# Rorisis/Co-Occ

Measured on AMD Instinct MI355X. Metric: samples/sec (6-cam frame + sweep -> occ+render), 200x200x16 grid, higher is better.
Workload: dtype f32 (split-f16 products, fp32 accumulate)

## Files before the change

co_occ_amd/_lib.py:

```python
import ctypes
import os
import threading
import time

import torch

_HERE = os.path.dirname(os.path.abspath(__file__))
LIB_PATH = os.path.join(_HERE, "libcoocc_hip.so")

c_int, c_float, c_void_p, c_size_t, c_int64 = (ctypes.c_int, ctypes.c_float, ctypes.c_void_p,
                                               ctypes.c_size_t, ctypes.c_int64)


class ConvDesc(ctypes.Structure):
    _fields_ = [(n, c_void_p) for n in ("in_", "w", "out", "scale", "bias", "res", "gather", "out_rows", "ws")] + \
               [("ws_floats", c_int64)] + \
               [(n, c_int) for n in ("M", "Cin", "Cout", "taps", "in_stride", "out_stride", "res_stride",
                                     "B", "Xi", "Yi", "Zi", "Xo", "Yo", "Zo", "ksize", "stride", "pad",
                                     "relu", "res_mode", "splitk", "tile_hint", "kx", "ky", "kz", "px", "py", "pz",
                                     "wgroup_rows", "mfma_dtype")] + [("alpha", ctypes.c_float), ("M_dev", c_void_p), ("gather_stride", c_int), ("out16", c_void_p), ("out16_stride", c_int), ("out_h2", c_int),
                                                                   ("out_h2_twin", c_void_p), ("tile_sem", c_void_p), ("tile_sem_ints", c_int),
                                                                  ("alpha_dev", c_void_p), ("sx", c_int), ("sy", c_int), ("sz", c_int)]


class SearchDesc(ctypes.Structure):
    _fields_ = [("cat4", c_void_p), ("pts", c_void_p), ("pts_rows", c_int), ("pts_stride", c_int)] + \
               [(n, c_int) for n in ("C", "X", "Y", "Z", "K", "fps_num", "max_cluster")] + \
               [("radius", ctypes.c_float), ("dist_thresh", ctypes.c_float), ("offsets", c_void_p), ("noff", c_int)] + \
               [(n, c_void_p) for n in ("lin", "counts", "near_img", "near_pts", "rows", "rows_p", "ws")] + \
               [("ws_bytes", ctypes.c_size_t), ("counts_host", c_void_p)]


P, I, F, Z, L = c_void_p, c_int, c_float, c_size_t, c_int64
SIGNATURES = {
    "coocc_last_error": (ctypes.c_char_p, []),
    "coocc_abi_version": (I, []),
    "coocc_device_cu_count": (I, [P]),
    "coocc_stream_create_cu_mask": (I, [P, I, P]),
    "coocc_stream_destroy": (I, [P]),
    "coocc_event_create": (I, [I, P]),
    "coocc_event_destroy": (I, [P]),
    "coocc_event_record": (I, [P, P]),
    "coocc_stream_wait_event": (I, [P, P]),
    "coocc_event_synchronize": (I, [P]),
    "coocc_event_query": (I, [P]),
    "coocc_event_elapsed_ms": (I, [P, P, P]),
    "coocc_ncdhw_to_ndhwc": (I, [P, P, I, I, I, I, I, P]),
    "coocc_rows_to_bf16": (I, [P, I, L, I, P, P]),
    "coocc_rows_to_h2": (I, [P, I, L, I, F, P, P]),
    "coocc_rows_to_h2_ex": (I, [P, I, L, I, F, P, P, P]),
    "coocc_rows_to_h2_gather": (I, [P, I, P, L, P, I, F, P, P]),
    "coocc_rows_to_f16": (I, [P, I, L, I, P, P]),
    "coocc_wino_input_h2": (I, [P, I, I, I, I, I, I, I, P, I, L, F, P]),
    "coocc_wino_input_h2_ex": (I, [P, I, I, I, I, I, I, I, P, I, L, F, P, P]),
    "coocc_ndhwc_to_ncdhw": (I, [P, P, I, I, I, I, I, P]),
    "coocc_fuser_prepare": (I, [P, P, P, P, P, I, I, I, P]),
    "coocc_fuser_prepare_rows": (I, [P, I, I, P, I, I, P, P, P, I, I, I, P]),
    "coocc_compact_flags": (I, [P, I, P, P, P, Z, P]),
    "coocc_compact_flags_ex": (I, [P, I, P, P, P, P, Z, P]),
    "coocc_lin_to_coords": (I, [P, I, I, I, I, P, P, P]),
    "coocc_furthest_point_sampling": (I, [I, I, I, P, P, P, P]),
    "coocc_fps_voxels_ws": (Z, [I, I, I]),
    "coocc_fps_voxels": (I, [P, I, I, I, I, I, P, P, Z, P]),
    "coocc_fps_voxels_pair": (I, [P, I, P, P, P, I, P, P, Z, I, I, I, I, P]),
    "coocc_ball_query": (I, [I, I, I, F, F, I, P, P, P, P]),
    "coocc_knn_topk": (I, [I, I, I, P, P, P, P, P]),
    "coocc_voxel_index_map": (I, [P, I, I, P, P]),
    "coocc_voxel_index_map_dev": (I, [P, I, P, I, P, P]),
    "coocc_fine_sample_voxel_dev": (I, [P, I, I, I, I, P, I, P, I, P, P, P, I, P]),
    "coocc_fine_sample_img_dev": (I, [P, I, I, I, I, P, P, L, P, P, I, I, P]),
    "coocc_fine_mlp_pre_dev": (I, [P, I, P, I, L, P, I, P, P, P, F, P, P, P, P, F, P, P, I, P, P]),
    "coocc_fine_fused": (I, [P, I, I, I, P, I, I, I, P, P, I, P, I, P, P, P, P, F, P, P, P, P, F, P, P, I, P, P, P]),
    "coocc_fine2_pack": (I, [P, P, I, P, P, P, P, P, P, P, P, P, P]),
    "coocc_fine2_h2": (I, [P, I, I, I, I, P, I, I, I, P, P, I, P, P, P, P, F, F, I, P, P, P, P]),
    "coocc_fine_sample_img_lin": (I, [P, I, I, I, I, P, P, I, I, I, P, P, I, I, P]),
    "coocc_scatter_fine_dev": (I, [P, L, P, I, I, I, P, P, I, I, I, F, P]),
    "coocc_scatter_fine_grouped": (I, [P, I, I, P, I, P, I, I, I, I, P, F, P, P]),
    "coocc_ball_query_voxels": (I, [I, F, F, I, I, I, I, P, P, P, P, P]),
    "coocc_knn_topk_voxels": (I, [I, I, I, I, I, I, P, P, P, P, I, P, P, P, P, P]),
    "coocc_knn_assign": (I, [I, I, I, I, F, P, P, P, P, P, P]),
    "coocc_knn_threshold": (I, [I, F, P, P, P, P]),
    "coocc_index_rows_i32": (I, [P, I, P, I, P, P]),
    "coocc_conv_pack_weights": (L, [P, I, I, I, I, P]),
    "coocc_conv_fwd": (I, [ctypes.POINTER(ConvDesc), P]),
    "coocc_fuser_search_ws": (Z, [ctypes.POINTER(SearchDesc)]),
    "coocc_fuser_search": (I, [ctypes.POINTER(SearchDesc), P, P]),
    "coocc_upsample_add_trilinear": (I, [P, P, I, I, I, I, I, I, I, I, P]),
    "coocc_upsample_add_trilinear_ex": (I, [P, P, I, I, I, I, I, I, I, I, P, P]),
    "coocc_occhead_mix": (I, [P, P, I, P, P, I, I, P]),
    "coocc_occhead_mix_ex": (I, [P, P, I, P, P, I, I, P, P]),
    "coocc_argmax_flags": (I, [P, I, I, I, I, P, P]),
    "coocc_fine_sample_voxel": (I, [P, I, I, I, I, P, I, I, P, P, P, I, P]),
    "coocc_fine_sample_img": (I, [P, I, I, I, I, P, P, L, P, I, I, P]),
    "coocc_fine_mlp_pre": (I, [P, I, P, I, L, P, P, P, F, P, P, P, P, F, P, P, I, P, P]),
    "coocc_fine_mlp": (I, [P, I, P, I, L, P, P, P, P, F, P, P, P, P, F, P, P, I, P, P]),
    "coocc_groupnorm_rows": (I, [P, L, I, I, I, P, P, F, I, P]),
    "coocc_groupnorm_nhwc": (I, [P, I, I, I, I, P, P, F, I, P]),
    "coocc_scatter_fine": (I, [P, L, I, I, P, P, I, I, I, F, P]),
    "coocc_camera_mats": (I, [P, P, P, P, P, P, I, I, I, I, P, P]),
    "coocc_get_geometry": (I, [P, P, P, P, I, I, I, I, P, P]),
    "coocc_bev_pool_forward": (I, [P, P, P, P, I, I, I, I, I, I, I, P, P]),
    "coocc_bev_pool_backward": (I, [P, P, P, P, I, I, I, I, I, I, I, P, P]),
    "coocc_voxel_pool_ws": (Z, [I, I]),
    "coocc_voxel_pool": (I, [P, P, I, I, I, P, I, I, I, I, P, I, P, Z, I, P]),
    "coocc_lift_splat": (I, [P, P, P, I, I, I, I, I, I, P, I, I, I, I, P, I, P, Z, I, P]),
    "coocc_lift_splat_cams": (I, [P, P, P, P, P, P, I, I, I, I, I, I, P, I, I, I, I, P, I, P, Z, I, P]),
    "coocc_lift_splat_reuse": (I, [P, P, I, I, I, I, I, I, I, I, I, P, I, P, Z, P]),
    "coocc_bev_pool_coords": (I, [P, P, I, I, I, I, I, I, P, I, P, Z, I, P]),
    "coocc_render_nearest": (I, [P, I, I, I, P, P, I, I, I, I, P, I, P, P]),
    "coocc_render_nearest_cams": (I, [P, I, I, I, P, P, P, P, P, I, I, I, I, P, I, P, P]),
# ... 275 lines not shown
```

co_occ_amd/backbone.py:

```python
from torch import nn

from .core import PackCache, PackedConv, conv_rows, to_rows
from .registry import BACKBONES

_NORMS = {"BN": nn.BatchNorm3d, "BN3d": nn.BatchNorm3d, "SyncBN": nn.SyncBatchNorm}


def _eval_only(module):
    if module.training:
        raise RuntimeError("%s.forward_rows is the eval-mode (folded-BN, no autograd) path but the module is in training "
                           "mode; call .eval(), or use forward() / co_occ_amd.autograd for training" % type(module).__name__)


def build_bn(norm_cfg, num_features):
    cfg = dict(norm_cfg or dict(type="BN3d"))
    t = cfg.pop("type")
    cfg.pop("requires_grad", None)
    if t not in _NORMS:
        raise NotImplementedError("norm type %r: only BN-family norms are folded into the HIP convs" % t)
    return _NORMS[t](num_features, **cfg)


class BasicBlock(nn.Module):
    expansion = 1

    def __init__(self, in_planes, planes, stride=1, downsample=None, norm_cfg=None):
        super().__init__()
        self.conv1 = nn.Conv3d(in_planes, planes, 3, stride=stride, padding=1, bias=False)
        self.bn1 = build_bn(norm_cfg, planes)
        self.relu = nn.ReLU(inplace=True)
        self.conv2 = nn.Conv3d(planes, planes, 3, padding=1, bias=False)
        self.bn2 = build_bn(norm_cfg, planes)
        self.downsample = downsample
        self.stride = stride

    def packed(self):
        d = dict(c1=PackedConv(self.conv1.weight, bn=self.bn1, ksize=3, stride=self.stride, pad=1),
                 c2=PackedConv(self.conv2.weight, bn=self.bn2, ksize=3, pad=1))
        if self.downsample is not None:
            d["ds"] = PackedConv(self.downsample[0].weight, bn=self.downsample[1], ksize=1, stride=self.stride)
        return d

    def run(self, x, p, readers=()):
        out = conv_rows(x, p["c1"], relu=True, twin_for=(p["c2"],))
        res = conv_rows(x, p["ds"], relu=False) if "ds" in p else x
        return conv_rows(out, p["c2"], relu=True, res=res, twin_for=readers)


@BACKBONES.register_module()
class CustomResNet3D(nn.Module):
    def __init__(self, depth, block_inplanes=[64, 128, 256, 512], block_strides=[1, 2, 2, 2],
                 out_indices=(0, 1, 2, 3), n_input_channels=3, shortcut_type='B',
                 norm_cfg=dict(type='BN3d', requires_grad=True), widen_factor=1.0):
        super().__init__()
        layer_metas = {10: [1, 1, 1, 1], 18: [2, 2, 2, 2], 34: [3, 4, 6, 3]}
        if depth not in layer_metas:
            raise NotImplementedError("CustomResNet3D depth %s: Bottleneck depths are not on the coocc_nusc path" % depth)
        if shortcut_type != 'B':
            raise NotImplementedError("shortcut_type 'A' is not used by any shipped config")
        block_inplanes = [int(x * widen_factor) for x in block_inplanes]
        self.in_planes = block_inplanes[0]
        self.out_indices = out_indices
        self.input_proj = nn.Sequential(
            nn.Conv3d(n_input_channels, self.in_planes, kernel_size=(1, 1, 1), stride=(1, 1, 1), bias=False),
            build_bn(norm_cfg, self.in_planes), nn.ReLU(inplace=True))
        self.layers = nn.ModuleList()
        for i in range(len(block_inplanes)):
            self.layers.append(self._make_layer(block_inplanes[i], layer_metas[depth][i], block_strides[i], norm_cfg))
        for m in self.modules():
            if isinstance(m, nn.Conv3d):
                nn.init.kaiming_normal_(m.weight, mode='fan_out', nonlinearity='relu')
            elif isinstance(m, (nn.BatchNorm3d, nn.SyncBatchNorm)):
                nn.init.constant_(m.weight, 1)
                nn.init.constant_(m.bias, 0)
        self._packs = PackCache(self)

    def _make_layer(self, planes, blocks, stride, norm_cfg):
        downsample = None
        if stride != 1 or self.in_planes != planes:
            downsample = nn.Sequential(nn.Conv3d(self.in_planes, planes, 1, stride=stride, bias=False),
                                       build_bn(norm_cfg, planes))
        layers = [BasicBlock(self.in_planes, planes, stride, downsample, norm_cfg)]
        self.in_planes = planes
        for _ in range(1, blocks):
            layers.append(BasicBlock(self.in_planes, planes, norm_cfg=norm_cfg))
        return nn.Sequential(*layers)

    def _packed(self):
        def build():
            return dict(proj=PackedConv(self.input_proj[0].weight, bn=self.input_proj[1], ksize=1),
                        blocks=[[b.packed() for b in layer] for layer in self.layers])
        return self._packs.get_modules((self,), build)

    def forward_rows(self, x, readers=None):
        _eval_only(self)
        p = self._packed()
        flat = [bp for layer in p["blocks"] for bp in layer]
        x = conv_rows(to_rows(x), p["proj"], relu=True, twin_for=(flat[0]["c1"], flat[0].get("ds")))
        res = []
        n = 0
        for i, layer in enumerate(self.layers):
            for blk, bp in zip(layer, p["blocks"][i]):
                n += 1
                nxt = flat[n] if n < len(flat) else {}
                rd = [nxt.get("c1"), nxt.get("ds")]
                if readers is not None and i in self.out_indices and bp is p["blocks"][i][-1]:
                    rd += list(readers[self.out_indices.index(i)])
                x = blk.run(x, bp, tuple(rd))
            if i in self.out_indices:
                res.append(x)
        return res

    def forward(self, x):
        if self.training:
            from . import autograd as ag
            rows, geom = ag.rows_from_ncdhw(x)
            return [ag.ncdhw_from_rows(r, g) for r, g in ag.backbone_forward_train(self, rows, geom)]
        return [r.as_ncdhw() for r in self.forward_rows(x)]
```

co_occ_amd/core.py:

```python
import ctypes

import torch

from . import _lib
from ._lib import TIMER, ConvDesc, KernelTimer, call, ptr

_F32 = torch.float32


TILE_HINT = int(__import__("os").environ.get("COOCC_CONV_TILE", "0"))
CONV_V2 = int(__import__("os").environ.get("COOCC_CONV_V2", "1"))
WINO = int(__import__("os").environ.get("COOCC_WINO", "1"))
WINO_MIN_ROWS = int(__import__("os").environ.get("COOCC_WINO_MIN_ROWS", "8192"))
CONV_PERSIST = __import__("os").environ.get("COOCC_CONV_PERSIST", "1") != "0"
ZTRIM = __import__("os").environ.get("COOCC_ZTRIM", "1") != "0"
WINO_TILE = int(__import__("os").environ.get("COOCC_WINO_TILE", "4"))
CONV_DTYPE = __import__("os").environ.get("COOCC_CONV_DTYPE", "f32")
CONV_ENGINE = __import__("os").environ.get("COOCC_CONV_ENGINE", "h2")
H2_WINO_SCALE = {2: 0.5, 3: 0.25, 4: 0.125}
H2_DIRECT = __import__("os").environ.get("COOCC_H2_DIRECT", "1") != "0"
INKERNEL_REDUCE = __import__("os").environ.get("COOCC_INKERNEL_REDUCE", "0") != "0"
H2_DIRECT_MIN_FLOPS = float(__import__("os").environ.get("COOCC_H2_MIN_FLOPS", "5e7"))


# ... 22 lines not shown
        return self

    def __exit__(self, *exc):
        if self._ctx is not None:
            self._ctx.__exit__(*exc)
            self._ctx = None
        return False

    def join(self, *tensors):
        if self.on and self.side is not None:
            cur = torch.cuda.current_stream(self.side.device)
            cur.wait_stream(self.side)
            for t in tensors:
                if torch.is_tensor(t) and t.is_cuda:
                    t.record_stream(cur)
            self.side = None


def branch_streams_of(device, stream):
    return [s for (d, h, _), s in _branch_streams.items() if d == device.index and h == stream.cuda_stream]


def conv_kernel_name(M, Cout, table, hint=0, iters=1 << 30, one_by_one=False, grouped=False):
    if (one_by_one and CONV_PERSIST and CONV_V2 and not table and Cout > 64 and M >= 8192 and iters <= 24
            and -(-M // 128) * -(-Cout // 128) > 768):
        return "k_conv2p<1x1>"
    if (grouped and CONV_PERSIST and CONV_V2 and iters <= 24 and (M // 128) * -(-Cout // 128) > 768
            and conv_kernel_name(M, Cout, table, hint, iters) == "k_conv2<128>"):
        return "k_conv2p"
    hint = hint or TILE_HINT
    if Cout <= 32:
        t = "128,32,32,32"
    elif Cout <= 64:
        t = "128,64,32,64"
    elif M < 8192:
        if M >= 512 and not table and CONV_V2:
            return "k_conv2<128>"
        t = "64,128,32,64"
    else:
        def util(bm):
            tiles = -(-M // bm) * (-(-Cout // 128))
            return tiles * bm / float(-(-tiles // 512) * 512)
        big = hint == 160 or (hint == 0 and util(160) > util(128) * 1.02)
        if iters <= 24 and hint != 160:
            big = False
        if not table and CONV_V2:
            return "k_conv2<%d>" % (160 if big else 128)
        t = "160,128,160,32" if big else "128,128,64,64"
    return "k_conv<%s,%s>" % (t, "table" if table else "geom")


class Rows:

    __slots__ = ("t", "B", "X", "Y", "Z", "C", "coff", "h16", "h2", "persistent", "aux")

    def __init__(self, t, B, X, Y, Z, C, coff=0, persistent=False):
        self.t, self.B, self.X, self.Y, self.Z, self.C, self.coff = t, B, X, Y, Z, C, coff
        self.persistent = persistent
        self.aux = None
        self.h16 = None
        self.h2 = None

    @property
    def stride(self):
        return self.t.shape[1]

    @property
    def V(self):
        return self.X * self.Y * self.Z

    def data(self):
        return ptr(self.t, offset=self.coff)

    def as_ncdhw(self):
        v = self.t.view(self.B, self.X, self.Y, self.Z, self.stride)
        if self.coff or self.stride != self.C:
            v = v[..., self.coff:self.coff + self.C]
        v = v.permute(0, 4, 1, 2, 3)
        if not self.persistent:
            v._coocc_rows = (self, v._version)
        return v


def to_rows(x):
    if isinstance(x, Rows):
        return x
    back = getattr(x, "_coocc_rows", None)
    if back is not None:
        r, ver = back
        if ver == x._version and x.dim() == 5 and tuple(x.shape) == (r.B, r.C, r.X, r.Y, r.Z):
            return r
    if x.dim() != 5:
        raise ValueError("expected a [B,C,X,Y,Z] tensor")
    if not x.is_cuda:
        raise _lib.CooccError("co_occ_amd modules run on the GPU only (no CPU fallback)")
    B, C, X, Y, Z = x.shape
    x = x.float()
    cl = x.permute(0, 2, 3, 4, 1)
    if cl.is_contiguous():
        return Rows(cl.reshape(B * X * Y * Z, C), B, X, Y, Z, C)
    x = x.contiguous()
    out = torch.empty(B * X * Y * Z, C, device=x.device, dtype=_F32)
    call("coocc_ncdhw_to_ndhwc", ptr(x), ptr(out), B, C, X * Y * Z, C, 0)
    return Rows(out, B, X, Y, Z, C)


def rows_to_ncdhw_contiguous(r):
    out = torch.empty(r.B, r.C, r.X, r.Y, r.Z, device=r.t.device, dtype=_F32)
    call("coocc_ndhwc_to_ncdhw", ptr(r.t), ptr(out), r.B, r.C, r.V, r.stride, r.coff)
    return out


def fold_bn(bn, conv_bias=None):
    var = bn.running_var.double()
    scale = torch.rsqrt(var + bn.eps)
    if bn.weight is not None:
        scale = scale * bn.weight.double()
    bias = -bn.running_mean.double() * scale
    if bn.bias is not None:
        bias = bias + bn.bias.double()
    if conv_bias is not None:
        bias = bias + conv_bias.double() * scale
    return scale.float(), bias.float()


def zyx_weight(w):
    return w.detach().permute(0, 1, 4, 3, 2).contiguous()
# ... 240 lines not shown


def check_h2_overflow(reset=True):
    fault = _lib.load().coocc_device_fault(1 if reset else 0)
    if fault:
        raise _lib.CooccError("libcoocc_hip: a kernel met an index outside the buffer it addresses and skipped the access (fault code %d: "
                              "%s) -- the outputs of this sample are not trustworthy" % (
                                  fault, {1: "coocc_sparse_tap_sum read a voxel -> ordinal map entry past the rows it was sized for "
                                             "(a stale or corrupted map)"}.get(fault, "unknown")))
    if _lib.load().coocc_h2_overflow(1 if reset else 0):
        raise _lib.CooccRangeError(
            "split-f16 engine: an activation left the f16 operand range (|x| >= 32768, or %g for the F(4x4) Winograd layers whose "
            "transform amplifies by up to 100 at scale 1/8; NaN counts) -- the outputs of this sample are not trustworthy.  "
            "Set COOCC_CONV_ENGINE=f32 (exact-fp32 MFMA kernels, no range limit; ~1.8x slower) or rescale the inputs "
            "(INTEGRATION.md, 'Operand range of the split-f16 engine')." % (32768.0 / (100 * H2_WINO_SCALE[4])))


def ztrim(Zin, Zout, stride, pad):
    ok = [kz for kz in range(3) if any(0 <= zo * stride - pad + kz < Zin for zo in range(Zout))]
    lo, hi = ok[0], ok[-1]
    return (None, None) if hi - lo == 2 else ((lo, hi), (3, 3, hi - lo + 1, pad, pad, pad - lo))


def _route(B, X, Y, Z, pc, rm, splitk):
    Xo, Yo, Zo = out_dims(X, Y, Z, pc)
    M = B * Xo * Yo * Zo
    bf16, f16 = CONV_DTYPE == "bf16", CONV_DTYPE == "f16"
    plan = None if (bf16 or f16) else _wino_plan_geom(B, X, Y, Z, pc, M, rm)
    if plan is not None:
        return "wino", plan, None, None, pc.wino_kz
    trim, kdims = ztrim(Z, Zo, pc.stride, pc.pad) if (ZTRIM and pc._w_cube is not None) else (None, None)
    taps = pc.taps if trim is None else 9 * kdims[2]
    if f16 and pc.Cin % 64 == 0 and pc._w_taps is not None and rm in (0, 1) and splitk in (0, 1):
        return "f16", None, trim, kdims, taps
    if (not bf16 and not f16 and CONV_ENGINE == "h2" and H2_DIRECT and pc.Cin % 32 == 0 and pc._w_taps is not None
            and rm in (0, 1) and 2.0 * M * pc.Cin * pc.Cout * taps >= H2_DIRECT_MIN_FLOPS):
        return "h2", None, trim, kdims, taps
    return "other", None, trim, kdims, taps


def route(B, X, Y, Z, pc, rm=0, splitk=0):
    return _route(B, X, Y, Z, pc, rm, splitk)[0]


def takes_h2(rows, consumers):
    g = (rows.B, rows.X, rows.Y, rows.Z) if isinstance(rows, Rows) else rows
    return any(pc is not None and route(*g, pc) == "h2" for pc in consumers)


def wants_h2_twin(rows, consumers):
    return CONV_ENGINE == "h2" and CONV_DTYPE == "f32" and rows.C % 32 == 0 and takes_h2(rows, consumers)


def conv_rows_wino(x, pc, out, relu, res, plan, in_ranges=None, twin=False):
    dev = x.t.device
    tile, pts, Tx, Ty, rows, G, hint = plan
    V = _wino_buffer(dev, "V", pts * G * pc.Cin)
    Mb = _wino_buffer(dev, "M", pts * G * pc.Cout)
    h2 = h2_capable(pc) and all(c % 32 == 0 for _, c in (in_ranges or []))
    wp = pc.wino_h2_pack(tile) if h2 else pc.wino_pack(tile)
    vscale = H2_WINO_SCALE[tile]
    sdev = getattr(pc, "operand_scale_dev", None) if h2 else None
    with TIMER.region("k_wino_in", 4.0 * x.V * pc.Cin + 4.0 * pts * rows * pc.Cin):
        if in_ranges is None and not h2:
            call("coocc_wino_input", x.data(), x.stride, x.B, x.X, x.Y, x.Z, pc.Cin, tile, ptr(V), G)
        else:
            assert in_ranges is None or sum(c for _, c in in_ranges) == pc.Cin
            voff = 0
            for coff, cr in (in_ranges or [(0, pc.Cin)]):
                src = ptr(x.t, offset=x.coff + coff)
                dst = ptr(V, offset=voff)
                if h2:
                    call("coocc_wino_input_h2_ex", src, x.stride, x.B, x.X, x.Y, x.Z, cr, tile, dst, pc.Cin, G, vscale, ptr(sdev))
                else:
                    call("coocc_wino_input_strided", src, x.stride, x.B, x.X, x.Y, x.Z, cr, tile, dst, pc.Cin, G)
                voff += cr
    kz = pc.wino_kz
    d = conv_desc(dev, in_=ptr(V), w=ptr(wp), out=ptr(Mb), M=pts * G, Cin=pc.Cin, Cout=pc.Cout, taps=kz,
                  in_stride=pc.Cin, out_stride=pc.Cout, B=pts * G // x.Z, Xi=1, Yi=1, Zi=x.Z, Xo=1, Yo=1, Zo=x.Z,
                  ksize=3, stride=1, pad=1, kx=1, ky=1, kz=kz, pz=kz // 2, wgroup_rows=G, splitk=1, tile_hint=hint or TILE_HINT)
    flops = 2.0 * pts * rows * pc.Cin * pc.Cout * kz
    if h2:
        d.mfma_dtype, d.alpha = 3, 1.0 / vscale
        if sdev is not None:
            d.alpha_dev = ptr(sdev, offset=1)
        launch_conv(d, V.device, "k_gemm_h2z wino%d" % tile, flops)
    else:
        launch_conv(d, V.device, lambda: conv_kernel_name(pts * G, pc.Cout, False, hint, kz * -(-pc.Cin // 32), grouped=True)
                    + " wino%d" % tile, flops)
    tw = None
    if twin and h2 and pc.Cout % 32 == 0 and out.coff == 0 and out.stride % 4 == 0:
        tw = out.h2 = torch.empty(out.B * out.V, pc.Cout, device=dev, dtype=_F32)
    with TIMER.region("k_wino_out", 4.0 * pts * rows * pc.Cout + 4.0 * x.V * pc.Cout * (2 if tw is not None else 1)):
        call("coocc_wino_output_ex", ptr(Mb), G, x.B, x.X, x.Y, x.Z, pc.Cout, tile, out.data(), out.stride, ptr(pc.scale),
             ptr(pc.bias), res.data() if res is not None else None, res.stride if res is not None else 0, int(relu), ptr(tw))
    return out


def conv_desc(device, **fields):
    ws = workspace(device)
    return ConvDesc(ws=ptr(ws), ws_floats=ws.numel(), **fields)


def launch_conv(d, device, name, flops):
    if not TIMER.enabled:
        _lib.conv_fwd(d, device)
        return
    with TIMER.region(name() if callable(name) else name, flops):
        _lib.conv_fwd(d, device)


def out_dim(n, k, s, p):
    return (n + 2 * p - k) // s + 1


def out_dims(X, Y, Z, pc):
    return tuple(out_dim(n, k, s, p) for n, k, s, p in zip((X, Y, Z), pc.kernel, pc.strides, pc.pads))


def conv_rows(x, pc, relu=True, res=None, res_mode=0, out=None, splitk=0, twin_for=()):
    Xo, Yo, Zo = out_dims(x.X, x.Y, x.Z, pc)
    M = x.B * Xo * Yo * Zo
    if out is None:
        out = Rows(torch.empty(M, pc.Cout, device=x.t.device, dtype=_F32), x.B, Xo, Yo, Zo, pc.Cout)
    else:
        out.h2 = out.h16 = None
    assert x.C == pc.Cin, "channel mismatch: %d vs %d" % (x.C, pc.Cin)
    rm = res_mode or (1 if res is not None else 0)
    family, plan, trim, kdims, taps = _route(x.B, x.X, x.Y, x.Z, pc, rm, splitk)
    twin = wants_h2_twin(out, twin_for)
    if family == "wino":
        return conv_rows_wino(x, pc, out, relu, res, plan, twin=twin)
    dev = x.t.device
    d = conv_desc(dev, out=out.data(), scale=ptr(pc.scale), bias=ptr(pc.bias), res=res.data() if res is not None else None,
                  M=M, Cin=pc.Cin, Cout=pc.Cout, taps=taps, out_stride=out.stride, res_stride=res.stride if res is not None else 0,
                  B=x.B, Xi=x.X, Yi=x.Y, Zi=x.Z, Xo=Xo, Yo=Yo, Zo=Zo, ksize=pc.ksize, stride=pc.stride, pad=pc.pad,
                  relu=int(relu), res_mode=rm, splitk=splitk, tile_hint=TILE_HINT)
    if trim is not None:
        d.kx, d.ky, d.kz, d.px, d.py, d.pz = kdims
    if pc.aniso:
        (d.kx, d.ky, d.kz), (d.px, d.py, d.pz), (d.sx, d.sy, d.sz) = pc.kernel, pc.pads, pc.strides
    same = pc.is_unit_stride and (Xo, Yo, Zo) == (x.X, x.Y, x.Z)
    flops = 2.0 * M * pc.Cin * pc.Cout * taps
    if family == "f16" and out.coff == 0 and out.stride == pc.Cout:
        xh = x.h16
        if xh is None:
            xh = torch.empty(x.B * x.V, pc.Cin, device=dev, dtype=torch.float16)
            call("coocc_rows_to_f16", x.data(), x.stride, x.B * x.V, pc.Cin, ptr(xh))
        out.h16 = torch.empty(M, pc.Cout, device=dev, dtype=torch.float16) if pc.Cout % 4 == 0 else None
        d.in_, d.in_stride, d.w, d.mfma_dtype, d.alpha, d.splitk = ptr(xh), pc.Cin, ptr(pc.h1_pack(trim)), 4, 1.0, 1
        if out.h16 is not None:
            d.out16, d.out16_stride = ptr(out.h16), pc.Cout
        launch_conv(d, pc.w.device, "k_gemm_h1z" if (same and taps > 1) else "k_gemm_h1w", flops)
        return out
    if family == "h2":
        if x.coff == 0 and x.C == pc.Cin:
            xh = h2_rows(x)
        else:
            xh = scratch(dev, "h2in", x.B * x.V * pc.Cin)
            call("coocc_rows_to_h2", x.data(), x.stride, x.B * x.V, pc.Cin, 1.0, ptr(xh))
        d.in_, d.in_stride, d.w, d.mfma_dtype, d.alpha = ptr(xh), pc.Cin, ptr(pc.h2_pack(trim)), 3, 1.0
        if INKERNEL_REDUCE:
            sem = tile_sem(dev)
            d.tile_sem, d.tile_sem_ints = ptr(sem), sem.numel()
        if twin and out.coff == 0 and out.stride % 4 == 0 and (res is None or res.stride % 4 == 0):
            out.h2 = torch.empty(M, pc.Cout, device=dev, dtype=_F32)
            d.out_h2_twin = ptr(out.h2)
        launch_conv(d, pc.w.device, "k_gemm_h2z direct" if (same and taps > 1) else "k_gemm_h2w", flops)
        return out
    bf16 = CONV_DTYPE == "bf16"
    if bf16 and BF16_PRECONVERT and pc.Cin % 64 == 0 and pc._w_taps is not None and taps > 1:
        xb = stream_buffer(dev, "bf16", x.B * x.V * pc.Cin, torch.bfloat16)
        call("coocc_rows_to_bf16", x.data(), x.stride, x.B * x.V, pc.Cin, ptr(xb))
        d.in_, d.in_stride, d.w, d.mfma_dtype = ptr(xb), pc.Cin, ptr(pc.bf16_pack(trim)), 2
        name = "k_conv_bf16z" if (same and ZSHARE) else "k_conv_bf16w"
    else:
        d.in_, d.in_stride, d.mfma_dtype = x.data(), x.stride, 1 if bf16 else 0
        d.w = ptr(pc.ztrim_pack(*trim) if trim is not None else pc.w)
        name = "k_conv_bf16" if bf16 else lambda: conv_kernel_name(M, pc.Cout, False, 0, taps * -(-pc.Cin // 32),
                                                                   pc.is_pointwise)
    launch_conv(d, pc.w.device, name, flops)
    return out


def linear_rows(x2d, pc, relu=False, out=None, out_coff=0, in_coff=0, in_C=None):
    n = x2d.shape[0]
    Cin = in_C if in_C is not None else pc.Cin
    if out is None:
        out = torch.empty(n, pc.Cout, device=x2d.device, dtype=_F32)
    if n == 0:
        return out
    d = conv_desc(x2d.device, in_=ptr(x2d, offset=in_coff), w=ptr(pc.w), out=ptr(out, offset=out_coff), scale=ptr(pc.scale),
                  bias=ptr(pc.bias), M=n, Cin=Cin, Cout=pc.Cout, taps=1, in_stride=x2d.shape[1], out_stride=out.shape[1],
                  B=1, Xi=n, Yi=1, Zi=1, Xo=n, Yo=1, Zo=1, ksize=1, stride=1, relu=int(relu), tile_hint=TILE_HINT)
    launch_conv(d, x2d.device, lambda: conv_kernel_name(n, pc.Cout, False, 0, -(-Cin // 32), True), 2.0 * n * Cin * pc.Cout)
    return out


def linear_rows_h2(xh, n, Cin, pc, relu=False, out=None, out_coff=0, out_h2=False):
    dev = xh.device
    if out is None:
        out = torch.empty(n, pc.Cout, device=dev, dtype=_F32)
    d = conv_desc(dev, in_=ptr(xh), w=ptr(pc.h2_pack()), out=ptr(out, offset=out_coff), scale=ptr(pc.scale), bias=ptr(pc.bias),
                  M=n, Cin=Cin, Cout=pc.Cout, taps=1, in_stride=Cin, out_stride=out.shape[1], B=1, Xi=n, Yi=1, Zi=1, Xo=n, Yo=1,
                  Zo=1, ksize=1, stride=1, relu=int(relu), splitk=1, mfma_dtype=3, alpha=1.0, out_h2=int(out_h2))
    launch_conv(d, dev, "k_gemm_h2w linear", 2.0 * n * Cin * pc.Cout)
    return out


def rows_to_h2(x2d, C=None, coff=0, name="h2rows"):
    n = x2d.shape[0]
    C = C if C is not None else x2d.shape[1]
    xh = scratch(x2d.device, name, n * C)
    call("coocc_rows_to_h2", ptr(x2d, offset=coff), x2d.shape[1], n, C, 1.0, ptr(xh))
    return xh


def g1_h2_capable(pc, C):
    return bool(CONV_ENGINE == "h2" and H2_DIRECT and C % 32 == 0 and h2_capable(pc) and pc.h2_pack() is not None)


def g1_sources_h2(cat4, C, pc):
    if not g1_h2_capable(pc, C) or cat4.shape[1] < 2 * C:
        return None
    return rows_to_h2(cat4, 2 * C, 0, name="g1rows2")


def gather_conv_rows(src, src_coff, pc, gather, out_rows, dst, dst_coff, gate_coff, C, relu=True, count_dev=None, src_h2=None):
    K, M = gather.shape
    if M == 0:
        return
    d = conv_desc(src.device, in_=ptr(src, offset=src_coff), w=ptr(pc.w), out=ptr(dst, offset=dst_coff), bias=ptr(pc.bias),
                  res=ptr(dst, offset=gate_coff), gather=ptr(gather, torch.int32), out_rows=ptr(out_rows, torch.int32),
                  M=M, Cin=C, Cout=pc.Cout, taps=K, in_stride=src.shape[1], out_stride=dst.shape[1], res_stride=dst.shape[1],
                  B=1, Xi=src.shape[0], Yi=1, Zi=1, Xo=1, Yo=1, Zo=1,
                  ksize=1, stride=1, relu=int(relu), res_mode=2, splitk=1, tile_hint=TILE_HINT)
    if count_dev is not None:
        d.M_dev, d.gather_stride = ptr(count_dev, torch.int32), M
    h2 = g1_h2_capable(pc, C)
    if h2:
        if src_h2 is not None and src_h2[1] <= src_coff and src_coff + C <= src_h2[1] + src_h2[2] and (src_coff - src_h2[1]) % 32 == 0:
            sh, c0, n = src_h2
            d.in_, d.in_stride = ptr(sh, offset=src_coff - c0), n
        else:
            sh = rows_to_h2(src, C, src_coff, name="g1rows")
            d.in_, d.in_stride = ptr(sh), C
        d.w, d.mfma_dtype, d.alpha = ptr(pc.h2_pack()), 3, 1.0
    launch_conv(d, src.device, "k_gemm_h2w" if h2 else lambda: conv_kernel_name(M, pc.Cout, True), 2.0 * M * C * pc.Cout * K)


class PackCache:

    def __init__(self, owner=None):
        self._key = None
        self._val = None
        self._slots = None
        if owner is not None and hasattr(owner, "register_load_state_dict_post_hook"):
            owner.register_load_state_dict_post_hook(self._on_load_state_dict)

    def _on_load_state_dict(self, module, incompatible_keys):
        self.invalidate()

    def __getstate__(self):
        return dict(_key=None, _val=None, _slots=None)

    def invalidate(self):
        self._key = self._val = None
        self._slots = None

    def get_modules(self, modules, build, buffers=True):
        slots = getattr(self, "_slots", None)
        if slots is None:
            slots = []
            for mod in modules:
                for m in mod.modules():
                    slots += [(m._parameters, k) for k in m._parameters]
                    if buffers:
                        slots += [(m._buffers, k) for k in m._buffers]
# ... 58 lines not shown
```

co_occ_amd/csrc/conv3d.hip:

```cpp
#include <stdlib.h>
#include <type_traits>
#include <string.h>

#include "common.h"

typedef float f32x16 __attribute__((ext_vector_type(16)));
typedef float f32x4 __attribute__((ext_vector_type(4)));

#include "conv_k.h"
#include "h2_rows.h"

template <int BM, int BN, int WM, int WN, bool TABLE>
__global__ __launch_bounds__(256, 2) void k_conv(ConvK p) {
  constexpr int WAVES_N = BN / WN;
  constexpr int TM = WM / 32, TN = WN / 32;
  constexpr int PA = BM / 32, PB = BN / 32;
  static_assert((BM / WM) * (BN / WN) == 4, "4 waves per block");
  constexpr int NBUF = (2 * 2 * (BM + BN) * LDS_ST * 4 <= 160 * 1024) ? 2 : 1;
  __shared__ float As[NBUF][BM * LDS_ST];
  __shared__ float Bs[NBUF][BN * LDS_ST];

  const int id = blockIdx.x;
  int mtile, nt, slot = id >> 3;
  if (p.mtiles_per_xcd > 0) {
// ... 960 lines not shown
      }
#pragma unroll
      for (int i = 0; i < TM; ++i)
#pragma unroll
        for (int r = 0; r < 16; ++r) acc[i][r] = 0.f;
    }
    if (!has_next) break;
    id = nid; m0c = m0; n0c = n0;
  }
}

__global__ __launch_bounds__(256) void k_conv_reduce(ConvK p) {
  size_t i = (size_t)blockIdx.x * blockDim.x + threadIdx.x;
  if (i >= (size_t)p.M * p.Cout) return;
  int m = (int)(i / p.Cout), n = (int)(i - (size_t)m * p.Cout);
  float v = 0.f;
  for (int z = 0; z < p.splitk; ++z) v += p.ws[((size_t)z * p.M + m) * p.Npad + n];
  size_t orow = p.out_rows ? (size_t)p.out_rows[m] : (size_t)m;
  p.out[orow * p.out_stride + n] = epilogue(p, v, n, orow);
}

__global__ __launch_bounds__(256) void k_conv_reduce4(ConvK p) {
  const int c4 = p.Cout >> 2;
  const size_t i = (size_t)blockIdx.x * blockDim.x + threadIdx.x;
  if (i >= (size_t)p.M * c4) return;
  const int m = (int)(i / c4), n = (int)(i - (size_t)m * c4) * 4;
  f32x4 v = {0.f, 0.f, 0.f, 0.f};
  const float* src = p.ws + (size_t)m * p.Npad + n;
  const size_t zs = (size_t)p.M * p.Npad;
  const size_t orow = p.out_rows ? (size_t)p.out_rows[m] : (size_t)m;
  const f32x4 zero4 = {0.f, 0.f, 0.f, 0.f}, one4 = {1.f, 1.f, 1.f, 1.f};
  const f32x4 rs = (p.res_mode && p.res) ? *(const f32x4*)(p.res + orow * p.res_stride + n) : zero4;
  const f32x4 sc = p.scale ? *(const f32x4*)(p.scale + n) : one4;
  const f32x4 bi = p.bias ? *(const f32x4*)(p.bias + n) : zero4;
  int z = 0;
  for (; z + 4 <= p.splitk; z += 4) {
    const f32x4 a0 = *(const f32x4*)(src + (size_t)z * zs), a1 = *(const f32x4*)(src + (size_t)(z + 1) * zs);
    const f32x4 a2 = *(const f32x4*)(src + (size_t)(z + 2) * zs), a3 = *(const f32x4*)(src + (size_t)(z + 3) * zs);
    v = v + a0; v = v + a1; v = v + a2; v = v + a3;
  }
  if (z + 2 <= p.splitk) {
    const f32x4 a0 = *(const f32x4*)(src + (size_t)z * zs), a1 = *(const f32x4*)(src + (size_t)(z + 1) * zs);
    v = v + a0; v = v + a1;
    z += 2;
  }
  if (z < p.splitk) v = v + *(const f32x4*)(src + (size_t)z * zs);
  if (p.res_mode == 3) v = v + rs;
  if (p.scale) v = v * sc;
  if (p.bias) v = v + bi;
  if (p.res_mode == 1) v = v + rs;
  if (p.relu && (p.relu == 1 || n < p.relu)) { v[0] = fmaxf(v[0], 0.f); v[1] = fmaxf(v[1], 0.f); v[2] = fmaxf(v[2], 0.f); v[3] = fmaxf(v[3], 0.f); }
  if (p.res_mode == 2) v = v * rs;
  if (p.out_h2) { store_h2(p.out, orow, p.out_stride, n, v); h2_guard(p.h2_flag, v); }
  else *(f32x4*)(p.out + orow * p.out_stride + n) = v;
  if (p.out16) { store_f16(p.out16, orow, p.out16_stride, n, v); h2_guard(p.h2_flag, v); }
  if (p.out_h2t) { store_h2(p.out_h2t, orow, p.Cout, n, v); h2_guard(p.h2_flag, v); }
}

extern "C" int64_t coocc_conv_pack_weights(const float* w_host, int Cout, int Cin, int taps, int tap_major,
                                           float* packed_host) {
  if (Cout <= 0 || Cin <= 0 || taps <= 0) return coocc_set_error(COOCC_EINVAL, "pack_weights: bad dims");
  const int kch = (Cin + KC - 1) / KC;
  const int Npad = (Cout + NPAD_TO - 1) / NPAD_TO * NPAD_TO;
  const int64_t total = (int64_t)taps * kch * Npad * KC;
  if (!packed_host) return total;
  if (!w_host) return coocc_set_error(COOCC_EINVAL, "pack_weights: null weights");
  memset(packed_host, 0, sizeof(float) * (size_t)total);
  for (int t = 0; t < taps; ++t)
    for (int n = 0; n < Cout; ++n)
      for (int c = 0; c < Cin; ++c) {
        float v = tap_major ? w_host[((size_t)n * taps + t) * Cin + c] : w_host[((size_t)n * Cin + c) * taps + t];
        packed_host[wfrag_index((size_t)(c / KC) * taps + t, Npad >> 7, n, c % KC)] = v;
      }
  return total;
}

int coocc_zero_row(const void** out) {
  static void* zero_row[64] = {nullptr};
  int dev = 0;
  COOCC_HIP(hipGetDevice(&dev));
  COOCC_CHECK_ARG(dev >= 0 && dev < 64, "conv_fwd: device index");
  if (!zero_row[dev]) {
    COOCC_HIP(hipMalloc(&zero_row[dev], 256));
    COOCC_HIP(hipMemset(zero_row[dev], 0, 256));
  }
  *out = zero_row[dev];
  return COOCC_OK;
}

template <int BM, int BN, int WM, int WN>
static void launch_cfg(ConvK& k, bool table, hipStream_t s) {
  k.mtiles = (k.M + BM - 1) / BM;
  k.ntiles = (k.Cout + BN - 1) / BN;
  k.mtiles_per_xcd = k.mtiles >= 64 ? (k.mtiles + 7) / 8 : 0;
  dim3 grid(k.mtiles_per_xcd ? 8 * k.mtiles_per_xcd * k.ntiles : k.mtiles * k.ntiles, k.splitk);
  if (table)
    hipLaunchKernelGGL((k_conv<BM, BN, WM, WN, true>), grid, dim3(256), 0, s, k);
  else
    hipLaunchKernelGGL((k_conv<BM, BN, WM, WN, false>), grid, dim3(256), 0, s, k);
}

extern "C" int coocc_conv_fwd(const coocc_conv_desc* d, void* stream) {
  COOCC_CHECK_ARG(d && d->in && d->w && d->out, "conv_fwd: null pointer");
  COOCC_CHECK_ARG(d->M > 0 && d->Cin > 0 && d->Cout > 0 && d->taps > 0, "conv_fwd: bad sizes");
  COOCC_CHECK_ARG(d->Cin % 4 == 0 && d->in_stride % 4 == 0, "conv_fwd: Cin and in_stride must be multiples of 4");
  COOCC_CHECK_ARG(((uintptr_t)d->in & 15) == 0 && ((uintptr_t)d->w & 15) == 0, "conv_fwd: in/w must be 16-byte aligned");
  COOCC_CHECK_ARG(d->res_mode == 0 || d->res, "conv_fwd: res_mode set without res");
  if (!d->gather) {
    if (d->kx > 0) COOCC_CHECK_ARG(d->ky > 0 && d->kz > 0 && d->taps == d->kx * d->ky * d->kz, "conv_fwd: taps != kx*ky*kz");
    else COOCC_CHECK_ARG(d->taps == d->ksize * d->ksize * d->ksize, "conv_fwd: taps != ksize^3");
    COOCC_CHECK_ARG((long long)d->B * d->Xo * d->Yo * d->Zo == d->M, "conv_fwd: M != B*Xo*Yo*Zo");
  }
  ConvK k;
  memset(&k, 0, sizeof(k));
  k.in = d->in; k.w = d->w; k.out = d->out; k.scale = d->scale; k.bias = d->bias; k.res = d->res;
  k.gather = d->gather; k.out_rows = d->out_rows; k.ws = d->ws;
  k.M_dev = (d->gather || d->mfma_dtype >= 3) ? d->M_dev : nullptr;
  k.gstride = d->gather_stride > 0 ? d->gather_stride : d->M;
  COOCC_CHECK_ARG(!d->M_dev || ((d->gather || d->mfma_dtype >= 3) && d->splitk == 1), "conv_fwd: M_dev needs a row table (gather) or mfma_dtype 3, and splitk = 1");
  COOCC_CHECK_ARG(k.gstride >= d->M, "conv_fwd: gather_stride smaller than M");
  k.M = d->M; k.Cin = d->Cin; k.Cout = d->Cout; k.taps = d->taps;
  k.kchunks = (d->Cin + KC - 1) / KC;
  k.Npad = (d->Cout + NPAD_TO - 1) / NPAD_TO * NPAD_TO;
  k.in_stride = d->in_stride; k.out_stride = d->out_stride; k.res_stride = d->res_stride;
  k.Xi = d->Xi; k.Yi = d->Yi; k.Zi = d->Zi; k.Xo = d->Xo; k.Yo = d->Yo; k.Zo = d->Zo;
  k.stride = d->stride;
  COOCC_CHECK_ARG(d->sx >= 0 && d->sy >= 0 && d->sz >= 0, "conv_fwd: negative per-axis stride");
  k.sx = d->sx > 0 ? d->sx : d->stride; k.sy = d->sy > 0 ? d->sy : d->stride; k.sz = d->sz > 0 ? d->sz : d->stride;
  if (d->kx > 0) { k.kx = d->kx; k.ky = d->ky; k.kz = d->kz; k.px = d->px; k.py = d->py; k.pz = d->pz; }
  else { k.kx = k.ky = k.kz = d->ksize; k.px = k.py = k.pz = d->pad; }
  k.wgroup_rows = d->wgroup_rows;
  k.wgroup_floats = (size_t)k.taps * k.kchunks * k.Npad * KC;
  k.relu = d->relu; k.res_mode = d->res_mode;
  k.total_iters = k.taps * k.kchunks;
  if (d->mfma_dtype == 3 || d->mfma_dtype == 4) {
    hipStream_t s3 = as_stream(stream);
    const int rc = coocc_launch_h2(k, d, s3);
    if (rc != COOCC_OK) return rc;
    if (k.splitk > 1 && !k.tile_sem) {
      const bool vec4 = (k.Cout & 3) == 0 && (k.out_stride & 3) == 0 && (!k.res || (k.res_stride & 3) == 0) && (((uintptr_t)k.out) & 15) == 0;
      if (vec4) hipLaunchKernelGGL(k_conv_reduce4, dim3(cdiv((long long)k.M * (k.Cout / 4), 256)), dim3(256), 0, s3, k);
      else hipLaunchKernelGGL(k_conv_reduce, dim3(cdiv((long long)k.M * k.Cout, 256)), dim3(256), 0, s3, k);
      COOCC_LAUNCH_CHECK("k_conv_reduce");
    }
    return COOCC_OK;
  }
  if (d->mfma_dtype == 2) {
    COOCC_CHECK_ARG(d->Cin % 64 == 0 && d->in_stride % 8 == 0, "conv_fwd: bf16 operands need Cin % 64 == 0 and in_stride % 8 == 0");
    k.kchunks = d->Cin / 64;
    k.total_iters = k.taps * k.kchunks;
  }

  int cfg;
  if (d->Cout <= 32) cfg = 3;
  else if (d->Cout <= 64) cfg = 2;
  else cfg = d->M >= 8192 ? 0 : 1;
// ... 164 lines not shown
```

co_occ_amd/csrc/gemm_h2.hip:

```cpp
#include <stdlib.h>
#include <string.h>
#include <type_traits>

#include "conv_k.h"

#include "h2_rows.h"

typedef float f32x16 __attribute__((ext_vector_type(16)));
typedef _Float16 f16x8 __attribute__((ext_vector_type(8)));

__device__ __forceinline__ void glds16_(const void* g, void* l) {
  __builtin_amdgcn_global_load_lds((const __attribute__((address_space(1))) void*)g, (__attribute__((address_space(3))) void*)l,
                                   16, 0, 0);
}

__device__ __forceinline__ void h2_epilogue_vec(const ConvK& p, size_t orow, int n, f32x4 v) {
  if (p.res_mode == 3) v = v + *(const f32x4*)(p.res + orow * p.res_stride + n);
  if (p.scale) v = v * *(const f32x4*)(p.scale + n);
  if (p.bias) v = v + *(const f32x4*)(p.bias + n);
  if (p.res_mode == 1) v = v + *(const f32x4*)(p.res + orow * p.res_stride + n);
  if (p.relu && (p.relu == 1 || n < p.relu)) { v[0] = fmaxf(v[0], 0.f); v[1] = fmaxf(v[1], 0.f); v[2] = fmaxf(v[2], 0.f); v[3] = fmaxf(v[3], 0.f); }
  if (p.res_mode == 2) v = v * *(const f32x4*)(p.res + orow * p.res_stride + n);
  if (p.out_h2) { store_h2(p.out, orow, p.out_stride, n, v); h2_guard(p.h2_flag, v); }
  else *(f32x4*)(p.out + orow * p.out_stride + n) = v;
// ... 826 lines not shown
  const bool zshare = !table && !d->out_rows && !d->M_dev && k.stride == 1 && k.Xo == k.Xi && k.Yo == k.Yi && k.Zo == k.Zi && k.kz >= 1 && k.kz <= 3 &&
                      (k.taps > 1 || d->wgroup_rows > 0);
  COOCC_CHECK_ARG(zshare || d->wgroup_rows == 0, "conv_fwd: weight groups need the stride-1 same geometry");
  k.kchunks = d->Cin / kc;
  k.total_iters = k.taps * k.kchunks;
  k.wgroup_floats = (size_t)k.taps * k.kchunks * k.Npad * 32;
  k.out16 = d->out16;
  k.out16_stride = d->out16_stride;
  COOCC_CHECK_ARG(!d->out16 || (d->Cout % 4 == 0 && d->out16_stride % 4 == 0 && !d->out_rows && ((uintptr_t)d->out16 & 7) == 0),
                  "conv_fwd: out16 needs Cout % 4 == 0, out16_stride % 4 == 0, no row scatter");
  k.alpha = d->alpha != 0.f ? d->alpha : 1.f;
  k.alpha_dev = d->alpha_dev;
  k.M_dev = d->M_dev;
  k.out_h2 = d->out_h2;
  COOCC_CHECK_ARG(!d->out_h2 || (d->Cout % 4 == 0 && d->out_stride % 32 == 0 && !d->out_rows),
                  "conv_fwd: out_h2 needs Cout % 4 == 0, out_stride % 32 == 0, no row scatter");
  k.out_h2t = d->out_h2_twin;
  COOCC_CHECK_ARG(!d->out_h2_twin || (!one && d->Cout % 32 == 0 && !d->out_rows && ((uintptr_t)d->out_h2_twin & 15) == 0 && (d->out_stride & 3) == 0 &&
                                      (!d->res || (d->res_stride & 3) == 0)),
                  "conv_fwd: out_h2_twin needs mfma_dtype 3, Cout % 32 == 0, 16-byte aligned rows, no row scatter");
  k.tile_sem = d->tile_sem;
  int rc = coocc_zero_row(&k.zrow);
  if (rc != COOCC_OK) return rc;
  rc = coocc_h2_flag_ptr(&k.h2_flag);
  if (rc != COOCC_OK) return rc;
  k.ntiles = (k.Cout + 127) / 128;
  k.mtiles = (k.M + 127) / 128;
  k.mtiles_per_xcd = k.mtiles >= 64 ? (k.mtiles + 7) / 8 : 0;
  const int gsz = zshare ? k.kz : 1;
  int splitk = d->splitk;
  const long long blocks = (long long)k.mtiles * k.ntiles;
  const int ngroups = k.total_iters / gsz;
  if (splitk <= 0) {
    splitk = 1;
    const bool vec4 = (d->Cout & 3) == 0 && (d->out_stride & 3) == 0 && (!d->res || (d->res_stride & 3) == 0) && (((uintptr_t)d->out) & 15) == 0;
    const bool second_pass_ok = vec4 || (!d->out_h2 && !d->out16 && !d->out_h2_twin);
    static const int target = getenv("COOCC_SPLITK_TARGET") ? atoi(getenv("COOCC_SPLITK_TARGET")) : 512;
    if (blocks < target / 2 && ngroups >= 8 && d->ws && !d->M_dev && (d->tile_sem ? true : (!d->out_rows && second_pass_ok))) {
      splitk = (int)(target / blocks);
      if (splitk > ngroups / 4) splitk = ngroups / 4;
      if (splitk > 64) splitk = 64;
      while (splitk > 1 && (long long)splitk * d->M * k.Npad > d->ws_floats) --splitk;
      if (splitk < 1) splitk = 1;
    }
  }
  int gps = (ngroups + splitk - 1) / splitk;
  k.iters_per_split = gps * gsz;
  k.splitk = (k.total_iters + k.iters_per_split - 1) / k.iters_per_split;
  COOCC_CHECK_ARG(k.splitk == 1 || (d->ws && !d->M_dev && (long long)k.splitk * d->M * k.Npad <= d->ws_floats),
                  "conv_fwd: split-K workspace too small (or split-K with a device row count)");
  COOCC_CHECK_ARG(k.splitk == 1 || d->tile_sem || (!d->out_h2 && !d->out16 && !d->out_h2_twin) ||
                      ((d->Cout & 3) == 0 && (d->out_stride & 3) == 0 && (!d->res || (d->res_stride & 3) == 0) && (((uintptr_t)d->out) & 15) == 0),
                  "conv_fwd: split-K with an H2 / f16 output needs 16-byte aligned rows (Cout, strides % 4 == 0)");
  COOCC_CHECK_ARG(k.splitk == 1 || !d->tile_sem || (long long)k.mtiles * k.ntiles <= d->tile_sem_ints,
                  "conv_fwd: tile_sem holds fewer counters than the launch has output tiles");
  dim3 grid(k.mtiles_per_xcd ? 8 * k.mtiles_per_xcd * k.ntiles : k.mtiles * k.ntiles, k.splitk);
  static const bool pointwise_on = !(getenv("COOCC_H2_POINTWISE") && atoi(getenv("COOCC_H2_POINTWISE")) == 0);
  if (pointwise_on && !zshare && !table && !one && k.taps == 1 && k.stride == 1 && k.px == 0 && k.py == 0 && k.pz == 0 && k.Xo == k.Xi &&
      k.Yo == k.Yi && k.Zo == k.Zi && k.kchunks <= 4 && k.splitk == 1 && !d->M_dev && !d->out_rows && blocks >= 256 &&
      (d->Cout & 3) == 0 && (d->out_stride & 3) == 0 && (!d->res || (d->res_stride & 3) == 0)) {
    switch (k.kchunks) {
      case 1: hipLaunchKernelGGL(k_gemm_h2p<1>, grid, dim3(256), 0, s, k); break;
      case 2: hipLaunchKernelGGL(k_gemm_h2p<2>, grid, dim3(256), 0, s, k); break;
      case 3: hipLaunchKernelGGL(k_gemm_h2p<3>, grid, dim3(256), 0, s, k); break;
      default: hipLaunchKernelGGL(k_gemm_h2p<4>, grid, dim3(256), 0, s, k); break;
    }
    COOCC_LAUNCH_CHECK("k_gemm_h2p");
    return COOCC_OK;
  }
  if (!zshare) {
    if (one) {
      if (table) hipLaunchKernelGGL((k_gemm_h2w<true, 1>), grid, dim3(256), 0, s, k);
      else hipLaunchKernelGGL((k_gemm_h2w<false, 1>), grid, dim3(256), 0, s, k);
    } else {
      const char* narrow_env = getenv("COOCC_H2_NARROW");
      const bool narrow_on = !(narrow_env && atoi(narrow_env) == 0);
      if (narrow_on && table && k.Cout <= 64 && k.ntiles == 1 && k.splitk == 1 && !d->tile_sem && (long long)k.mtiles >= 512) {
        const dim3 gridn((unsigned)((k.M + 255) / 256), 1);
        if (k.Cout <= 32) hipLaunchKernelGGL(k_gemm_h2n<1>, gridn, dim3(256), 0, s, k);
        else hipLaunchKernelGGL(k_gemm_h2n<2>, gridn, dim3(256), 0, s, k);
        COOCC_LAUNCH_CHECK("k_gemm_h2n");
        return COOCC_OK;
      }
      if (narrow_on && table && k.Cout > 96 && k.ntiles == 1 && k.splitk == 1 && !d->tile_sem && (long long)k.mtiles >= 128 && (long long)k.mtiles < 1024) {
        const dim3 gridn((unsigned)((k.M + 63) / 64), 1);
        hipLaunchKernelGGL(k_gemm_h2n<4>, gridn, dim3(256), 0, s, k);
        COOCC_LAUNCH_CHECK("k_gemm_h2n<4>");
        return COOCC_OK;
      }
      if (table) hipLaunchKernelGGL(k_gemm_h2w<true>, grid, dim3(256), 0, s, k);
      else hipLaunchKernelGGL(k_gemm_h2w<false>, grid, dim3(256), 0, s, k);
    }
    COOCC_LAUNCH_CHECK("k_gemm_h2w");
    return COOCC_OK;
  }
  COOCC_CHECK_ARG((long long)d->M < (1ll << 30) && (136ull + 2ull * ((unsigned long long)k.Yi + 2) * k.Zi) * d->in_stride * 4ull < 0xFFFFFF00ull,
                  "conv_fwd: the split-f16 kernel addresses a tile's window with 32-bit byte offsets");
  const bool xy = !(k.kx == 1 && k.ky == 1 && k.px == 0 && k.py == 0);
  if (one) {
    if (k.kz == 3) { if (xy) hipLaunchKernelGGL((k_gemm_h2z<3, true, 0, 1>), grid, dim3(256), 0, s, k); else hipLaunchKernelGGL((k_gemm_h2z<3, false, 0, 1>), grid, dim3(256), 0, s, k); }
    else if (k.kz == 2) { if (xy) hipLaunchKernelGGL((k_gemm_h2z<2, true, 0, 1>), grid, dim3(256), 0, s, k); else hipLaunchKernelGGL((k_gemm_h2z<2, false, 0, 1>), grid, dim3(256), 0, s, k); }
    else { if (xy) hipLaunchKernelGGL((k_gemm_h2z<1, true, 0, 1>), grid, dim3(256), 0, s, k); else hipLaunchKernelGGL((k_gemm_h2z<1, false, 0, 1>), grid, dim3(256), 0, s, k); }
    COOCC_LAUNCH_CHECK("k_gemm_h2z<f16>");
    return COOCC_OK;
  }
  static const int abl = getenv("COOCC_H2_ABLATE") ? atoi(getenv("COOCC_H2_ABLATE")) : 0;
// ... 31 lines not shown
  if (n_dev) rows = min(rows, (long long)*n_dev);
  if (scale_dev) scale *= *scale_dev;
  const int c8 = C >> 3;
  const long long i = (long long)blockIdx.x * blockDim.x + threadIdx.x;
  if (i >= rows * c8) return;
  const long long r = i / c8;
  const int c = (int)(i - r * c8) * 8;
  const long long sr = row_ids ? (long long)row_ids[r] : r;
  const f32x4 a = *(const f32x4*)(in + sr * in_stride + c), b = *(const f32x4*)(in + sr * in_stride + c + 4);
  f16x8 hi, lo;
#pragma unroll
  for (int e = 0; e < 4; ++e) {
    _Float16 u, v;
    split_h2(a[e] * scale, u, v); hi[e] = u; lo[e] = v;
    split_h2(b[e] * scale, u, v); hi[4 + e] = u; lo[4 + e] = v;
  }
  char* o = out + r * (long long)C * 4 + (c >> 5) * 128 + (c & 31) * 2;
  *(f16x8*)o = hi;
  *(f16x8*)(o + 64) = lo;
  h2_guard(flag, a * scale);
  h2_guard(flag, b * scale);
}

extern "C" int coocc_rows_to_h2_ex(const float* in, int in_stride, int64_t rows, int C, float scale, const float* scale_dev,
                                   void* out_h2, void* stream) {
  COOCC_CHECK_ARG(in && out_h2 && rows >= 0 && C > 0 && C % 32 == 0 && in_stride % 4 == 0 && in_stride >= C, "rows_to_h2: bad args");
  COOCC_CHECK_ARG(((uintptr_t)in & 15) == 0 && ((uintptr_t)out_h2 & 15) == 0, "rows_to_h2: pointers must be 16-byte aligned");
  if (rows == 0) return COOCC_OK;
  int* flag = nullptr;
  if (coocc_h2_flag_ptr(&flag) != COOCC_OK) return COOCC_EHIP;
  hipLaunchKernelGGL(k_rows_to_h2, dim3(cdiv(rows * (C / 8), 256)), dim3(256), 0, as_stream(stream), in, in_stride, (long long)rows, C,
                     scale, (char*)out_h2, (const int32_t*)nullptr, (const int32_t*)nullptr, flag, scale_dev);
  COOCC_LAUNCH_CHECK("k_rows_to_h2");
  return COOCC_OK;
}

extern "C" int coocc_rows_to_h2(const float* in, int in_stride, int64_t rows, int C, float scale, void* out_h2, void* stream) {
  return coocc_rows_to_h2_ex(in, in_stride, rows, C, scale, nullptr, out_h2, stream);
}

extern "C" int coocc_rows_to_h2_gather(const float* in, int in_stride, const int32_t* row_ids, int64_t n_cap, const int32_t* n_dev,
                                       int C, float scale, void* out_h2, void* stream) {
  COOCC_CHECK_ARG(in && out_h2 && row_ids && n_cap >= 0 && C > 0 && C % 32 == 0 && in_stride % 4 == 0, "rows_to_h2_gather: bad args");
  COOCC_CHECK_ARG(((uintptr_t)in & 15) == 0 && ((uintptr_t)out_h2 & 15) == 0, "rows_to_h2_gather: pointers must be 16-byte aligned");
  if (n_cap == 0) return COOCC_OK;
  int* flag = nullptr;
  if (coocc_h2_flag_ptr(&flag) != COOCC_OK) return COOCC_EHIP;
  hipLaunchKernelGGL(k_rows_to_h2, dim3(cdiv(n_cap * (C / 8), 256)), dim3(256), 0, as_stream(stream), in, in_stride, (long long)n_cap, C,
                     scale, (char*)out_h2, row_ids, n_dev, flag, (const float*)nullptr);
  COOCC_LAUNCH_CHECK("k_rows_to_h2");
  return COOCC_OK;
}

__global__ __launch_bounds__(256) void k_rows_to_f16(const float* __restrict__ in, int in_stride, long long rows, int C, _Float16* __restrict__ out) {
  const int c8 = C >> 3;
  const long long i = (long long)blockIdx.x * blockDim.x + threadIdx.x;
  if (i >= rows * c8) return;
  const long long r = i / c8;
  const int c = (int)(i - r * c8) * 8;
  const f32x4 a = *(const f32x4*)(in + r * in_stride + c), b = *(const f32x4*)(in + r * in_stride + c + 4);
  f16x8 o;
#pragma unroll
  for (int e = 0; e < 4; ++e) { o[e] = (_Float16)a[e]; o[4 + e] = (_Float16)b[e]; }
  *(f16x8*)(out + r * C + c) = o;
}

extern "C" int coocc_rows_to_f16(const float* in, int in_stride, int64_t rows, int C, void* out_f16, void* stream) {
  COOCC_CHECK_ARG(in && out_f16 && rows >= 0 && C > 0 && C % 8 == 0 && in_stride % 4 == 0 && in_stride >= C, "rows_to_f16: bad args");
  COOCC_CHECK_ARG(((uintptr_t)in & 15) == 0 && ((uintptr_t)out_f16 & 15) == 0, "rows_to_f16: pointers must be 16-byte aligned");
  if (rows == 0) return COOCC_OK;
  hipLaunchKernelGGL(k_rows_to_f16, dim3(cdiv(rows * (C / 8), 256)), dim3(256), 0, as_stream(stream), in, in_stride, (long long)rows, C,
                     (_Float16*)out_f16);
  COOCC_LAUNCH_CHECK("k_rows_to_f16");
  return COOCC_OK;
}
```

co_occ_amd/csrc/layout.hip:

```cpp
#include <stdarg.h>
#include <stdlib.h>

#include "common.h"

typedef float f32x4 __attribute__((ext_vector_type(4)));

static thread_local char g_err[512] = "";

int coocc_set_error(int code, const char* fmt, ...) {
  va_list ap;
  va_start(ap, fmt);
  vsnprintf(g_err, sizeof(g_err), fmt, ap);
  va_end(ap);
  return code;
}

extern "C" const char* coocc_last_error(void) { return g_err; }
extern "C" int coocc_abi_version(void) { return 1; }

#define TV 64
#define TC 128

__global__ __launch_bounds__(256) void k_ncdhw_to_ndhwc(const float* __restrict__ src,
                                                         float* __restrict__ dst, int C, int V,
// ... 70 lines not shown
  COOCC_LAUNCH_CHECK("k_ndhwc_to_ncdhw");
  return COOCC_OK;
}

__global__ __launch_bounds__(256) void k_fuser_prepare(const float* __restrict__ img,
                                                        const float* __restrict__ pts,
                                                        float* __restrict__ cat4,
                                                        uint8_t* __restrict__ flag_img,
                                                        uint8_t* __restrict__ flag_pts, int C, int V) {
  __shared__ float tile[TV][TC + 1];
  const int b = blockIdx.y;
  const int v0 = blockIdx.x * TV;
  const int t = threadIdx.x;
  const int stride = 4 * C;
  for (int mod = 0; mod < 2; ++mod) {
    const float* src = mod ? pts : img;
    uint8_t* flags = mod ? flag_pts : flag_img;
    float rsum = 0.f;
    for (int c0 = 0; c0 < C; c0 += TC) {
      const int cn = min(TC, C - c0);
      for (int c = t >> 6; c < cn; c += 4) {
        int v = v0 + (t & 63);
        tile[t & 63][c] = v < V ? src[((size_t)b * C + c0 + c) * V + v] : 0.f;
      }
      __syncthreads();
      if (t < TV)
        for (int c = 0; c < cn; ++c) rsum += tile[t][c];
      for (int i = t; i < TV * cn; i += 256) {
        int v = i / cn, c = i - v * cn;
        if (v0 + v < V) cat4[((size_t)b * V + v0 + v) * stride + mod * C + c0 + c] = tile[v][c];
      }
      __syncthreads();
    }
    if (t < TV && v0 + t < V) flags[(size_t)b * V + v0 + t] = rsum != 0.f ? 1 : 0;
  }
  for (int i = t; i < TV * 2 * C; i += 256) {
    int v = i / (2 * C), c = i - v * 2 * C;
    if (v0 + v < V) cat4[((size_t)b * V + v0 + v) * stride + 2 * C + c] = 0.f;
  }
}

extern "C" int coocc_fuser_prepare(const float* img, const float* pts, float* cat4, uint8_t* flag_img,
                                   uint8_t* flag_pts, int B, int C, int V, void* stream) {
  COOCC_CHECK_ARG(img && pts && cat4 && flag_img && flag_pts && B > 0 && C > 0 && V > 0, "fuser_prepare: bad args");
  dim3 grid(cdiv(V, TV), B);
  hipLaunchKernelGGL(k_fuser_prepare, grid, dim3(256), 0, as_stream(stream), img, pts, cat4, flag_img, flag_pts, C, V);
  COOCC_LAUNCH_CHECK("k_fuser_prepare");
  return COOCC_OK;
}

__global__ __launch_bounds__(256) void k_fuser_prepare_rows(const float* __restrict__ img, int img_rows, int img_stride,
                                                             const float* __restrict__ pts, int pts_rows, int pts_stride,
                                                             float* __restrict__ cat4, uint8_t* __restrict__ flag_img,
                                                             uint8_t* __restrict__ flag_pts, int C, int V) {
  __shared__ float tile[TV][TC + 1];
  const int b = blockIdx.y;
  const int v0 = blockIdx.x * TV;
  const int t = threadIdx.x;
  const int stride = 4 * C;
  for (int mod = 0; mod < 2; ++mod) {
    const float* src = mod ? pts : img;
    const int rows = mod ? pts_rows : img_rows, sstride = mod ? pts_stride : img_stride;
    uint8_t* flags = mod ? flag_pts : flag_img;
    const bool in_place = rows && src == cat4 + mod * C && sstride == stride;
    float rsum = 0.f;
    for (int c0 = 0; c0 < C; c0 += TC) {
      const int cn = min(TC, C - c0);
      if (rows) {
        if (cn == TC) {
          for (int i = t; i < TV * (TC / 4); i += 256) {
            const int v = i / (TC / 4), c = (i % (TC / 4)) * 4;
            f32x4 q = {0.f, 0.f, 0.f, 0.f};
            if (v0 + v < V) q = *(const f32x4*)(src + ((size_t)b * V + v0 + v) * sstride + c0 + c);
            tile[v][c] = q[0]; tile[v][c + 1] = q[1]; tile[v][c + 2] = q[2]; tile[v][c + 3] = q[3];
          }
        } else {
          for (int i = t; i < TV * cn; i += 256) {
            int v = i / cn, c = i - v * cn;
            tile[v][c] = v0 + v < V ? src[((size_t)b * V + v0 + v) * sstride + c0 + c] : 0.f;
          }
        }
      } else {
        for (int c = t >> 6; c < cn; c += 4) {
          int v = v0 + (t & 63);
          tile[t & 63][c] = v < V ? src[((size_t)b * C + c0 + c) * V + v] : 0.f;
        }
      }
      __syncthreads();
      if (t < TV)
        for (int c = 0; c < cn; ++c) rsum += tile[t][c];
      if (!in_place)
        for (int i = t; i < TV * cn; i += 256) {
          int v = i / cn, c = i - v * cn;
          if (v0 + v < V) cat4[((size_t)b * V + v0 + v) * stride + mod * C + c0 + c] = tile[v][c];
        }
      __syncthreads();
    }
    if (t < TV && v0 + t < V) flags[(size_t)b * V + v0 + t] = rsum != 0.f ? 1 : 0;
  }
  for (int i = t; i < TV * 2 * C; i += 256) {
    int v = i / (2 * C), c = i - v * 2 * C;
    if (v0 + v < V) cat4[((size_t)b * V + v0 + v) * stride + 2 * C + c] = 0.f;
  }
}

constexpr int FV = 256, FC = 32;
__global__ __launch_bounds__(256) void k_fuser_prepare_rows_fast(const float* __restrict__ img, int img_rows, int img_stride,
                                                                  const float* __restrict__ pts, int pts_rows, int pts_stride,
                                                                  float* __restrict__ cat4, uint8_t* __restrict__ flag_img,
                                                                  uint8_t* __restrict__ flag_pts, int C, int V) {
  __shared__ float tile[FV][FC + 1];
  const int b = blockIdx.y;
  const int v0 = blockIdx.x * FV;
  const int t = threadIdx.x;
  const int stride = 4 * C;
  const int rv = t >> 3, rc = (t & 7) * 4;
  for (int mod = 0; mod < 2; ++mod) {
    const float* src = mod ? pts : img;
    const int rows = mod ? pts_rows : img_rows, sstride = mod ? pts_stride : img_stride;
    uint8_t* flags = mod ? flag_pts : flag_img;
    const bool in_place = rows && src == cat4 + mod * C && sstride == stride;
    float rsum = 0.f;
    for (int c0 = 0; c0 < C; c0 += FC) {
      if (rows) {
#pragma unroll
        for (int ps = 0; ps < FV / 32; ++ps) {
          const int v = ps * 32 + rv;
          f32x4 q = {0.f, 0.f, 0.f, 0.f};
          if (v0 + v < V) q = *(const f32x4*)(src + ((size_t)b * V + v0 + v) * sstride + c0 + rc);
          tile[v][rc] = q[0]; tile[v][rc + 1] = q[1]; tile[v][rc + 2] = q[2]; tile[v][rc + 3] = q[3];
        }
        __syncthreads();
#pragma unroll
        for (int c = 0; c < FC; ++c) rsum += tile[t][c];
      } else {
#pragma unroll 8
        for (int c = 0; c < FC; ++c) {
          const float x = v0 + t < V ? src[((size_t)b * C + c0 + c) * V + v0 + t] : 0.f;
          rsum += x;
          tile[t][c] = x;
        }
        __syncthreads();
      }
      if (!in_place) {
#pragma unroll
        for (int ps = 0; ps < FV / 32; ++ps) {
          const int v = ps * 32 + rv;
          if (v0 + v < V) {
            const f32x4 q = {tile[v][rc], tile[v][rc + 1], tile[v][rc + 2], tile[v][rc + 3]};
            *(f32x4*)(cat4 + ((size_t)b * V + v0 + v) * stride + mod * C + c0 + rc) = q;
          }
        }
      }
      __syncthreads();
    }
    if (v0 + t < V) flags[(size_t)b * V + v0 + t] = rsum != 0.f ? 1 : 0;
  }
  const int vec_per_row = C >> 1;
  const f32x4 z = {0.f, 0.f, 0.f, 0.f};
  if (vec_per_row <= 256 && 256 % vec_per_row == 0) {
    const int vpp = 256 / vec_per_row, tv = t / vec_per_row, c = (t - tv * vec_per_row) * 4;
    for (int v = tv; v < FV; v += vpp)
      if (v0 + v < V) *(f32x4*)(cat4 + ((size_t)b * V + v0 + v) * stride + 2 * C + c) = z;
  } else {
    for (int i = t; i < FV * vec_per_row; i += 256) {
      const int v = i / vec_per_row, c = (i - v * vec_per_row) * 4;
      if (v0 + v < V) *(f32x4*)(cat4 + ((size_t)b * V + v0 + v) * stride + 2 * C + c) = z;
    }
  }
}

extern "C" int coocc_fuser_prepare_rows(const float* img, int img_rows, int img_stride, const float* pts, int pts_rows,
                                        int pts_stride, float* cat4, uint8_t* flag_img, uint8_t* flag_pts, int B, int C, int V,
                                        void* stream) {
  COOCC_CHECK_ARG(img && pts && cat4 && flag_img && flag_pts && B > 0 && C > 0 && V > 0, "fuser_prepare_rows: bad args");
  COOCC_CHECK_ARG((!img_rows || img_stride >= C) && (!pts_rows || pts_stride >= C), "fuser_prepare_rows: row stride < C");
  const bool vec_ok = C % FC == 0 && ((uintptr_t)cat4 & 15) == 0 && (!img_rows || (img_stride % 4 == 0 && ((uintptr_t)img & 15) == 0)) &&
                      (!pts_rows || (pts_stride % 4 == 0 && ((uintptr_t)pts & 15) == 0));
  if (vec_ok) {
    hipLaunchKernelGGL(k_fuser_prepare_rows_fast, dim3(cdiv(V, FV), B), dim3(256), 0, as_stream(stream), img, img_rows, img_stride,
                       pts, pts_rows, pts_stride, cat4, flag_img, flag_pts, C, V);
    COOCC_LAUNCH_CHECK("k_fuser_prepare_rows_fast");
    return COOCC_OK;
  }
  dim3 grid(cdiv(V, TV), B);
  hipLaunchKernelGGL(k_fuser_prepare_rows, grid, dim3(256), 0, as_stream(stream), img, img_rows, img_stride, pts, pts_rows,
                     pts_stride, cat4, flag_img, flag_pts, C, V);
  COOCC_LAUNCH_CHECK("k_fuser_prepare_rows");
  return COOCC_OK;
}

#define CB 1024

__global__ __launch_bounds__(256) void k_flag_count(const uint8_t* __restrict__ flags, int total,
                                                     int32_t* __restrict__ blk) {
  __shared__ int wsum[4];
  int base = blockIdx.x * CB + threadIdx.x * 4;
  int c = 0;
  for (int j = 0; j < 4; ++j)
    if (base + j < total) c += flags[base + j] != 0;
  for (int o = 32; o > 0; o >>= 1) c += __shfl_down(c, o);
  if ((threadIdx.x & 63) == 0) wsum[threadIdx.x >> 6] = c;
  __syncthreads();
  if (threadIdx.x == 0) blk[blockIdx.x] = wsum[0] + wsum[1] + wsum[2] + wsum[3];
}

__global__ __launch_bounds__(1024) void k_scan_blocks(int32_t* __restrict__ blk, int nblk,
                                                       int32_t* __restrict__ count) {
  __shared__ int wsum[16];
  __shared__ int carry_s;
  if (threadIdx.x == 0) carry_s = 0;
  __syncthreads();
  for (int base = 0; base < nblk; base += 1024) {
    int i = base + threadIdx.x;
    int v = i < nblk ? blk[i] : 0;
    int inc = v;
    for (int o = 1; o < 64; o <<= 1) {
      int n = __shfl_up(inc, o);
      if ((threadIdx.x & 63) >= o) inc += n;
    }
    if ((threadIdx.x & 63) == 63) wsum[threadIdx.x >> 6] = inc;
    __syncthreads();
    int woff = 0;
    for (int w = 0; w < (int)(threadIdx.x >> 6); ++w) woff += wsum[w];
    int carry = carry_s;
    if (i < nblk) blk[i] = carry + woff + inc - v;
    __syncthreads();
    if (threadIdx.x == 1023) carry_s = carry + woff + inc;
    __syncthreads();
  }
  if (threadIdx.x == 0) *count = carry_s;
}

__global__ __launch_bounds__(256) void k_flag_write(const uint8_t* __restrict__ flags, int total,
                                                     const int32_t* __restrict__ blk,
                                                     int32_t* __restrict__ lin, int32_t* __restrict__ map) {
  __shared__ int wsum[4];
  int base = blockIdx.x * CB + threadIdx.x * 4;
  int f[4], c = 0;
  for (int j = 0; j < 4; ++j) {
    f[j] = (base + j < total) && flags[base + j] != 0;
    c += f[j];
// ... 189 lines not shown
```

co_occ_amd/csrc/search.hip:

```cpp
#include <stdlib.h>
#include <string.h>

#include "common.h"

__global__ __launch_bounds__(256) void k_gather_xyz(const float* __restrict__ xyz, const int32_t* __restrict__ idx, int m,
                                                     float* __restrict__ out) {
  const int i = blockIdx.x * blockDim.x + threadIdx.x;
  if (i >= m) return;
  const int s = idx[i];
  out[i * 3 + 0] = xyz[s * 3 + 0]; out[i * 3 + 1] = xyz[s * 3 + 1]; out[i * 3 + 2] = xyz[s * 3 + 2];
}

static size_t align256(size_t v) { return (v + 255) & ~(size_t)255; }

struct SearchWs {
  uint8_t* flags;
  int32_t* cws;
  float* xyz;
  int32_t* maps;
  int32_t* rep[2];
  float* rep_xyz[2];
  float* val[2];
  int32_t* nn[2];
  int32_t* group[2];
  int32_t* winner[2];
  void* fps[2];
  size_t fps_bytes;
  size_t total;
};

static SearchWs carve(char* base, int V, int K, int fps_num, int max_cluster, int X, int Y, int Z) {
  SearchWs w;
  size_t o = 0;
  auto take = [&](size_t bytes) { char* p = base ? base + o : nullptr; o += align256(bytes); return p; };
  w.flags = (uint8_t*)take((size_t)2 * V);
  w.cws = (int32_t*)take((size_t)2 * (V / 1024 + 2) * 4);
  w.xyz = (float*)take((size_t)2 * V * 3 * 4);
  w.maps = (int32_t*)take((size_t)2 * V * 4);
  w.fps_bytes = coocc_fps_voxels_ws(X, Y, Z);
  for (int d = 0; d < 2; ++d) {
    w.rep[d] = (int32_t*)take((size_t)fps_num * 4);
    w.rep_xyz[d] = (float*)take((size_t)fps_num * 3 * 4);
    w.val[d] = (float*)take((size_t)fps_num * K * 4);
    w.nn[d] = (int32_t*)take((size_t)fps_num * K * 4);
    w.group[d] = (int32_t*)take((size_t)fps_num * max_cluster * 4);
    w.winner[d] = (int32_t*)take((size_t)K * V * 4);
    w.fps[d] = take(w.fps_bytes);
  }
  w.total = o;
  return w;
}

extern "C" size_t coocc_fuser_search_ws(const coocc_search_desc* d) {
  if (!d || d->X <= 0 || d->Y <= 0 || d->Z <= 0 || d->K <= 0) return 0;
  return carve(nullptr, d->X * d->Y * d->Z, d->K, d->fps_num, d->max_cluster, d->X, d->Y, d->Z).total;
}

#define SRC(call)                    \
  do {                               \
    int rc__ = (call);               \
    if (rc__ != COOCC_OK) return rc__; \
  } while (0)

extern "C" int coocc_fuser_search(coocc_search_desc* d, void* stream, void* side_stream) {
  COOCC_CHECK_ARG(d && d->cat4 && d->pts && d->lin && d->counts && d->rows && d->rows_p && d->near_img && d->near_pts && d->ws &&
                      d->offsets && d->counts_host, "fuser_search: null pointer");
  COOCC_CHECK_ARG(d->C > 0 && d->X > 0 && d->Y > 0 && d->Z > 0 && d->K >= 1 && d->K <= 8 && d->fps_num > 0 && d->max_cluster > 0 &&
                      d->noff > 0, "fuser_search: bad sizes");
  COOCC_CHECK_ARG(stream != side_stream && side_stream, "fuser_search: needs a second stream for the img <- pts direction");
  const int V = d->X * d->Y * d->Z, K = d->K, C = d->C;
  SearchWs w = carve((char*)d->ws, V, K, d->fps_num, d->max_cluster, d->X, d->Y, d->Z);
  COOCC_CHECK_ARG(d->ws_bytes >= w.total, "fuser_search: workspace smaller than coocc_fuser_search_ws()");
  hipStream_t s0 = as_stream(stream), s1 = as_stream(side_stream);
  static const int sdiag = [] { const char* e = getenv("COOCC_SEARCH_DIAG_SKIP"); return e ? atoi(e) : 0; }();
  int32_t* lin_img = d->lin;
  int32_t* lin_pts = d->lin + V;

  SRC(coocc_fuser_prepare_rows(d->cat4, 1, 4 * C, d->pts, d->pts_rows, d->pts_stride, d->cat4, w.flags, w.flags + V, 1, C, V, stream));
  SRC(coocc_compact_flags(w.flags, V, lin_img, d->counts, w.cws, (size_t)(V / 1024 + 2) * 4, stream));
  SRC(coocc_compact_flags(w.flags + V, V, lin_pts, d->counts + 1, w.cws + (V / 1024 + 2), (size_t)(V / 1024 + 2) * 4, stream));
  if (!((sdiag & 4) && d->counts_host[0] > 0)) COOCC_HIP(hipMemcpyAsync(d->counts_host, d->counts, 8, hipMemcpyDeviceToHost, s0));
  if (!((sdiag & 4) && d->counts_host[0] > 0)) {
    static const bool fence = [] { const char* e = getenv("COOCC_SEARCH_COUNT_FENCE"); return e && e[0] == '1'; }();
    hipEvent_t got;
    COOCC_HIP(hipEventCreateWithFlags(&got, hipEventBlockingSync | hipEventDisableTiming | (fence ? 0u : hipEventDisableSystemFence)));
    const hipError_t e1 = hipEventRecord(got, s0);
    const hipError_t e2 = e1 == hipSuccess ? hipEventSynchronize(got) : e1;
    (void)hipEventDestroy(got);
    if (e2 != hipSuccess) return coocc_set_error(COOCC_EHIP, "fuser_search: waiting for the voxel counts failed: %s", hipGetErrorString(e2));
  }
  const int Ni = d->counts_host[0], Np = d->counts_host[1];
  if (Ni <= d->fps_num || Np <= d->fps_num) return COOCC_SEARCH_SMALL;

  float* xyz_img = w.xyz;
  float* xyz_pts = w.xyz + (size_t)V * 3;
  SRC(coocc_lin_to_coords(lin_img, Ni, d->X, d->Y, d->Z, xyz_img, nullptr, stream));
  SRC(coocc_lin_to_coords(lin_pts, Np, d->X, d->Y, d->Z, xyz_pts, nullptr, stream));
  int32_t* map_img = w.maps;
  int32_t* map_pts = w.maps + V;
  SRC(coocc_voxel_index_map(lin_img, Ni, V, map_img, stream));
  SRC(coocc_voxel_index_map(lin_pts, Np, V, map_pts, stream));

  const int pair_rc = (sdiag & 1) ? COOCC_OK
                                  : coocc_fps_voxels_pair(lin_pts, Np, w.rep[0], w.fps[0], lin_img, Ni, w.rep[1], w.fps[1], w.fps_bytes, d->X, d->Y,
                                                          d->Z, d->fps_num, stream);
  if (pair_rc != COOCC_OK && pair_rc != 2) return pair_rc;
  const bool paired = pair_rc == COOCC_OK;
  hipEvent_t fork = nullptr, join = nullptr;
  COOCC_HIP(hipEventCreateWithFlags(&fork, hipEventDisableTiming | hipEventDisableSystemFence));
  if (hipEventCreateWithFlags(&join, hipEventDisableTiming | hipEventDisableSystemFence) != hipSuccess) {
    (void)hipEventDestroy(fork);
    return coocc_set_error(COOCC_EHIP, "fuser_search: hipEventCreate failed");
  }
  bool forked = false;
  auto finish = [&](int rc) -> int {
    if (forked) {
      if (hipEventRecord(join, s1) != hipSuccess || hipStreamWaitEvent(s0, join, 0) != hipSuccess) {
        if (rc == COOCC_OK) rc = coocc_set_error(COOCC_EHIP, "fuser_search: joining the side stream failed");
      }
    }
    (void)hipEventDestroy(fork);
    (void)hipEventDestroy(join);
    return rc;
  };
#define SRF(call)                                \
  do {                                           \
    int rc__ = (call);                           \
    if (rc__ != COOCC_OK) return finish(rc__);   \
  } while (0)
  void* side_q = paired ? stream : side_stream;
  if (!paired) {
// ... 27 lines not shown
```

co_occ_amd/csrc/winograd.hip:

```cpp
#include "conv_k.h"
#include "h2_rows.h"

template <int N> struct Wino;
template <> struct Wino<4> {
  static constexpr int M = 2;
  template <typename T> static __device__ __forceinline__ void bt(const T* d, T* t) {
    t[0] = d[0] - d[2]; t[1] = d[1] + d[2]; t[2] = d[2] - d[1]; t[3] = d[1] - d[3];
  }
  template <typename T> static __device__ __forceinline__ void at(const T* m, T* y) {
    y[0] = m[0] + m[1] + m[2]; y[1] = m[1] - m[2] - m[3];
  }
  template <typename T> static __device__ __forceinline__ void a(const T* y, T* t) {
    t[0] = y[0]; t[1] = y[0] + y[1]; t[2] = y[0] - y[1]; t[3] = -y[1];
  }
};
template <> struct Wino<5> {
  static constexpr int M = 3;
  template <typename T> static __device__ __forceinline__ void bt(const T* d, T* t) {
    t[0] = d[0] - 1.5f * (d[1] + d[2]) + d[3];
    t[1] = d[1] - 2.5f * d[2] + d[3];
    t[2] = 0.5f * (d[2] - d[1]) + d[3];
    t[3] = -2.f * d[1] - d[2] + d[3];
    t[4] = d[1] - 1.5f * (d[2] + d[3]) + d[4];
  }
// ... 24 lines not shown
    y[2] = s12 + 0.25f * m[3] + 4.f * m[4];
    y[3] = d12 + 0.125f * m[3] - 8.f * m[4] + m[5];
  }
  template <typename T> static __device__ __forceinline__ void a(const T* y, T* t) {
    const T s02 = y[0] + y[2], s13 = y[1] + y[3];
    t[0] = y[0]; t[1] = s02 + s13; t[2] = s02 - s13;
    t[3] = y[0] + 0.5f * y[1] + 0.25f * y[2] + 0.125f * y[3];
    t[4] = y[0] - 2.f * y[1] + 4.f * y[2] - 8.f * y[3];
    t[5] = y[3];
  }
};

template <int N>
__global__ __launch_bounds__(256) void k_wino_in(const float* __restrict__ in, int in_stride, int B, int X, int Y, int Z,
                                                  int C, int Tx, int Ty, size_t gstride, int vstride, float* __restrict__ V) {
  constexpr int MO = Wino<N>::M;
  const int c4 = C >> 2;
  const long long i = (long long)blockIdx.x * 256 + threadIdx.x;
  const long long rows = (long long)B * Tx * Ty * Z;
  if (i >= rows * c4) return;
  const int c = (int)(i % c4) * 4;
  const long long row = i / c4;
  long long r = row;
  const int z = (int)(r % Z); r /= Z;
  const int ty = (int)(r % Ty); r /= Ty;
  const int tx = (int)(r % Tx); const int b = (int)(r / Tx);
  f32x4 t[N][N];
#pragma unroll
  for (int e = 0; e < N; ++e) {
    f32x4 d[N], q[N];
    const int y = MO * ty - 1 + e;
#pragma unroll
    for (int a = 0; a < N; ++a) {
      const int x = MO * tx - 1 + a;
      f32x4 v = {0.f, 0.f, 0.f, 0.f};
      if ((unsigned)x < (unsigned)X && (unsigned)y < (unsigned)Y)
        v = *(const f32x4*)(in + ((((size_t)b * X + x) * Y + y) * Z + z) * in_stride + c);
      d[a] = v;
    }
    Wino<N>::bt(d, q);
#pragma unroll
    for (int a = 0; a < N; ++a) t[a][e] = q[a];
  }
  float* o = V + (size_t)row * vstride + c;
#pragma unroll
  for (int a = 0; a < N; ++a) {
    f32x4 q[N];
    Wino<N>::bt(t[a], q);
#pragma unroll
    for (int e = 0; e < N; ++e) *(f32x4*)(o + (size_t)(a * N + e) * gstride) = q[e];
  }
}

template <int N>
__global__ __launch_bounds__(256) void k_wino_in_h2(const float* __restrict__ in, int in_stride, int B, int X, int Y, int Z,
                                                     int C, int Tx, int Ty, size_t gstride_bytes, int vstride, float scale,
                                                     char* __restrict__ V, int* __restrict__ flag, const float* __restrict__ scale_dev) {
  constexpr int MO = Wino<N>::M;
  if (scale_dev) scale *= *scale_dev;
  const int c4 = C >> 2;
  const long long i = (long long)blockIdx.x * 256 + threadIdx.x;
  const long long rows = (long long)B * Tx * Ty * Z;
  if (i >= rows * c4) return;
  const int c = (int)(i % c4) * 4;
  const long long row = i / c4;
  long long r = row;
  const int z = (int)(r % Z); r /= Z;
  const int ty = (int)(r % Ty); r /= Ty;
  const int tx = (int)(r % Tx); const int b = (int)(r / Tx);
  f32x4 t[N][N];
#pragma unroll
  for (int e = 0; e < N; ++e) {
    f32x4 d[N], q[N];
    const int y = MO * ty - 1 + e;
#pragma unroll
    for (int a = 0; a < N; ++a) {
      const int x = MO * tx - 1 + a;
      f32x4 v = {0.f, 0.f, 0.f, 0.f};
      if ((unsigned)x < (unsigned)X && (unsigned)y < (unsigned)Y)
        v = *(const f32x4*)(in + ((((size_t)b * X + x) * Y + y) * Z + z) * in_stride + c);
      d[a] = v;
    }
    Wino<N>::bt(d, q);
#pragma unroll
    for (int a = 0; a < N; ++a) t[a][e] = q[a];
  }
#pragma unroll
  for (int a = 0; a < N; ++a) {
    f32x4 q[N];
    Wino<N>::bt(t[a], q);
#pragma unroll
    for (int e = 0; e < N; ++e) {
      const f32x4 sv = q[e] * scale;
      store_h2_pair(V + (size_t)(a * N + e) * gstride_bytes, (size_t)row, vstride, c, sv);
      h2_guard(flag, sv);
    }
  }
}

extern "C" int coocc_wino_input_h2_ex(const float* in, int in_stride, int B, int X, int Y, int Z, int C, int tile, void* V,
                                      int vstride, int64_t group_rows, float scale, const float* scale_dev, void* stream) {
  COOCC_CHECK_ARG(in && V && B > 0 && X > 0 && Y > 0 && Z > 0 && C > 0 && C % 32 == 0 && in_stride % 4 == 0, "wino_input_h2: bad args");
  COOCC_CHECK_ARG(tile >= 2 && tile <= 4, "wino_input_h2: tile must be 2, 3 or 4");
  COOCC_CHECK_ARG(vstride >= C && vstride % 32 == 0 && ((uintptr_t)V & 127) == 0, "wino_input_h2: V row stride / alignment");
  COOCC_CHECK_ARG(scale > 0.f, "wino_input_h2: scale must be positive");
  const int Tx = (X + tile - 1) / tile, Ty = (Y + tile - 1) / tile;
  const long long rows = (long long)B * Tx * Ty * Z;
  COOCC_CHECK_ARG(group_rows >= rows, "wino_input_h2: group_rows smaller than B*ceil(X/tile)*ceil(Y/tile)*Z");
  const dim3 grid(cdiv(rows * (C / 4), 256));
  const size_t gstride = (size_t)group_rows * vstride * 4;
  hipStream_t s = as_stream(stream);
  int* flag = nullptr;
  if (coocc_h2_flag_ptr(&flag) != COOCC_OK) return COOCC_EHIP;
  if (tile == 2)
    hipLaunchKernelGGL(k_wino_in_h2<4>, grid, dim3(256), 0, s, in, in_stride, B, X, Y, Z, C, Tx, Ty, gstride, vstride, scale, (char*)V, flag, scale_dev);
  else if (tile == 3)
    hipLaunchKernelGGL(k_wino_in_h2<5>, grid, dim3(256), 0, s, in, in_stride, B, X, Y, Z, C, Tx, Ty, gstride, vstride, scale, (char*)V, flag, scale_dev);
  else
    hipLaunchKernelGGL(k_wino_in_h2<6>, grid, dim3(256), 0, s, in, in_stride, B, X, Y, Z, C, Tx, Ty, gstride, vstride, scale, (char*)V, flag, scale_dev);
  COOCC_LAUNCH_CHECK("k_wino_in_h2");
  return COOCC_OK;
}

extern "C" int coocc_wino_input_h2(const float* in, int in_stride, int B, int X, int Y, int Z, int C, int tile, void* V,
                                   int vstride, int64_t group_rows, float scale, void* stream) {
  return coocc_wino_input_h2_ex(in, in_stride, B, X, Y, Z, C, tile, V, vstride, group_rows, scale, nullptr, stream);
}

static int wino_input_impl(const float* in, int in_stride, int B, int X, int Y, int Z, int C, int tile, float* V, int vstride,
                           int64_t group_rows, void* stream) {
  COOCC_CHECK_ARG(in && V && B > 0 && X > 0 && Y > 0 && Z > 0 && C > 0 && C % 4 == 0 && in_stride % 4 == 0, "wino_input: bad args");
  COOCC_CHECK_ARG(tile >= 2 && tile <= 4, "wino_input: tile must be 2, 3 or 4");
  COOCC_CHECK_ARG(vstride >= C && vstride % 4 == 0 && ((uintptr_t)V & 15) == 0, "wino_input: V row stride / alignment");
  const int Tx = (X + tile - 1) / tile, Ty = (Y + tile - 1) / tile;
  const long long rows = (long long)B * Tx * Ty * Z;
  COOCC_CHECK_ARG(group_rows >= rows, "wino_input: group_rows smaller than B*ceil(X/tile)*ceil(Y/tile)*Z");
  const dim3 grid(cdiv(rows * (C / 4), 256));
  const size_t gstride = (size_t)group_rows * vstride;
  if (tile == 2)
    hipLaunchKernelGGL(k_wino_in<4>, grid, dim3(256), 0, as_stream(stream), in, in_stride, B, X, Y, Z, C, Tx, Ty, gstride, vstride, V);
  else if (tile == 3)
    hipLaunchKernelGGL(k_wino_in<5>, grid, dim3(256), 0, as_stream(stream), in, in_stride, B, X, Y, Z, C, Tx, Ty, gstride, vstride, V);
  else
    hipLaunchKernelGGL(k_wino_in<6>, grid, dim3(256), 0, as_stream(stream), in, in_stride, B, X, Y, Z, C, Tx, Ty, gstride, vstride, V);
  COOCC_LAUNCH_CHECK("k_wino_in");
  return COOCC_OK;
}

extern "C" int coocc_wino_input(const float* in, int in_stride, int B, int X, int Y, int Z, int C, int tile, float* V,
                                int64_t group_rows, void* stream) {
// ... 8 lines not shown
template <int N>
__global__ __launch_bounds__(256) void k_wino_out(const float* __restrict__ Mb, size_t gstride, int B, int X, int Y, int Z,
                                                   int C, int Tx, int Ty, float* __restrict__ out, int out_stride,
                                                   const float* __restrict__ scale, const float* __restrict__ bias,
                                                   const float* __restrict__ res, int res_stride, int relu,
                                                   void* __restrict__ twin, int* __restrict__ flag) {
  constexpr int MO = Wino<N>::M;
  const int c4 = (C + 3) >> 2;
  const long long i = (long long)blockIdx.x * 256 + threadIdx.x;
  const long long rows = (long long)B * Tx * Ty * Z;
  if (i >= rows * c4) return;
  const int c = (int)(i % c4) * 4;
  const long long row = i / c4;
  long long r = row;
  const int z = (int)(r % Z); r /= Z;
  const int ty = (int)(r % Ty); r /= Ty;
  const int tx = (int)(r % Tx); const int b = (int)(r / Tx);
  const int nc = min(4, C - c);
  const bool vec = (C & 3) == 0;
  const float* src = Mb + (size_t)row * C + c;
  f32x4 s[MO][N];
#pragma unroll
  for (int e = 0; e < N; ++e) {
    f32x4 m[N], q[MO];
#pragma unroll
    for (int a = 0; a < N; ++a) {
      const float* p = src + (size_t)(a * N + e) * gstride;
      if (vec) m[a] = *(const f32x4*)p;
      else m[a] = f32x4{p[0], nc > 1 ? p[1] : 0.f, nc > 2 ? p[2] : 0.f, nc > 3 ? p[3] : 0.f};
    }
    Wino<N>::at(m, q);
#pragma unroll
    for (int a = 0; a < MO; ++a) s[a][e] = q[a];
  }
  f32x4 sc = {1.f, 1.f, 1.f, 1.f}, bi = {0.f, 0.f, 0.f, 0.f};
#pragma unroll
  for (int e = 0; e < 4; ++e)
    if (e < nc) {
      if (scale) sc[e] = scale[c + e];
      if (bias) bi[e] = bias[c + e];
    }
#pragma unroll
  for (int a = 0; a < MO; ++a) {
    f32x4 y[MO];
    Wino<N>::at(s[a], y);
    const int x = MO * tx + a;
    if (x >= X) continue;
#pragma unroll
    for (int bb = 0; bb < MO; ++bb) {
      const int yy = MO * ty + bb;
      if (yy >= Y) continue;
      const size_t orow = (((size_t)b * X + x) * Y + yy) * Z + z;
      f32x4 v = y[bb] * sc + bi;
      float* o = out + orow * out_stride + c;
      const float* rr = res ? res + orow * res_stride + c : nullptr;
      if (vec && (out_stride & 3) == 0 && (!res || (res_stride & 3) == 0)) {
        if (rr) v = v + *(const f32x4*)rr;
        if (relu) { v[0] = fmaxf(v[0], 0.f); v[1] = fmaxf(v[1], 0.f); v[2] = fmaxf(v[2], 0.f); v[3] = fmaxf(v[3], 0.f); }
        *(f32x4*)o = v;
        if (twin) { store_h2_pair(twin, orow, C, c, v); h2_guard(flag, v); }
      } else {
#pragma unroll
        for (int e = 0; e < 4; ++e)
          if (e < nc) {
            float u = v[e] + (rr ? rr[e] : 0.f);
            o[e] = relu ? fmaxf(u, 0.f) : u;
          }
      }
    }
  }
}

extern "C" int coocc_wino_output_ex(const float* Mb, int64_t group_rows, int B, int X, int Y, int Z, int C, int tile, float* out,
                                    int out_stride, const float* scale, const float* bias, const float* res, int res_stride,
                                    int relu, void* out_h2_twin, void* stream) {
  COOCC_CHECK_ARG(Mb && out && B > 0 && X > 0 && Y > 0 && Z > 0 && C > 0, "wino_output: bad args");
  COOCC_CHECK_ARG(tile >= 2 && tile <= 4, "wino_output: tile must be 2, 3 or 4");
  COOCC_CHECK_ARG(((uintptr_t)out & 15) == 0 && (!res || ((uintptr_t)res & 15) == 0), "wino_output: out/res must be 16-byte aligned");
  COOCC_CHECK_ARG(!out_h2_twin || (C % 32 == 0 && (out_stride & 3) == 0 && (!res || (res_stride & 3) == 0) && ((uintptr_t)out_h2_twin & 15) == 0),
                  "wino_output: the H2 twin needs C % 32 == 0 and 16-byte aligned rows");
  const int Tx = (X + tile - 1) / tile, Ty = (Y + tile - 1) / tile;
  const long long rows = (long long)B * Tx * Ty * Z;
  COOCC_CHECK_ARG(group_rows >= rows, "wino_output: group_rows too small");
  int* flag = nullptr;
  if (out_h2_twin && coocc_h2_flag_ptr(&flag) != COOCC_OK) return COOCC_EHIP;
  const dim3 grid(cdiv(rows * ((C + 3) / 4), 256));
  if (tile == 2)
    hipLaunchKernelGGL(k_wino_out<4>, grid, dim3(256), 0, as_stream(stream), Mb, (size_t)group_rows * C, B, X, Y, Z, C, Tx, Ty,
                       out, out_stride, scale, bias, res, res_stride, relu, out_h2_twin, flag);
  else if (tile == 3)
    hipLaunchKernelGGL(k_wino_out<5>, grid, dim3(256), 0, as_stream(stream), Mb, (size_t)group_rows * C, B, X, Y, Z, C, Tx, Ty,
                       out, out_stride, scale, bias, res, res_stride, relu, out_h2_twin, flag);
  else
    hipLaunchKernelGGL(k_wino_out<6>, grid, dim3(256), 0, as_stream(stream), Mb, (size_t)group_rows * C, B, X, Y, Z, C, Tx, Ty,
                       out, out_stride, scale, bias, res, res_stride, relu, out_h2_twin, flag);
  COOCC_LAUNCH_CHECK("k_wino_out");
  return COOCC_OK;
}

extern "C" int coocc_wino_output(const float* Mb, int64_t group_rows, int B, int X, int Y, int Z, int C, int tile, float* out,
                                 int out_stride, const float* scale, const float* bias, const float* res, int res_stride,
                                 int relu, void* stream) {
  return coocc_wino_output_ex(Mb, group_rows, B, X, Y, Z, C, tile, out, out_stride, scale, bias, res, res_stride, relu, nullptr, stream);
}

template <int N>
__global__ __launch_bounds__(256) void k_wino_gradout(const float* __restrict__ dy, int dy_stride, int B, int X, int Y, int Z,
                                                       int C, int Tx, int Ty, size_t gstride, float* __restrict__ dM) {
  constexpr int MO = Wino<N>::M;
  const int c4 = C >> 2;
  const long long i = (long long)blockIdx.x * 256 + threadIdx.x;
  const long long rows = (long long)B * Tx * Ty * Z;
  if (i >= rows * c4) return;
  const int c = (int)(i % c4) * 4;
  const long long row = i / c4;
  long long r = row;
  const int z = (int)(r % Z); r /= Z;
  const int ty = (int)(r % Ty); r /= Ty;
  const int tx = (int)(r % Tx); const int b = (int)(r / Tx);
  f32x4 t[N][MO];
#pragma unroll
  for (int j = 0; j < MO; ++j) {
    f32x4 d[MO], q[N];
    const int y = MO * ty + j;
#pragma unroll
    for (int a = 0; a < MO; ++a) {
      const int x = MO * tx + a;
      f32x4 v = {0.f, 0.f, 0.f, 0.f};
      if (x < X && y < Y) v = *(const f32x4*)(dy + ((((size_t)b * X + x) * Y + y) * Z + z) * dy_stride + c);
// ... 287 lines not shown
```

co_occ_amd/detector.py:

```python
import numpy as np
import torch
from torch import nn

from . import registry
from .core import to_rows
from .registry import DETECTORS
from .render import MLP, render_block, render_losses
from .view_transformer import get_frustum


def _build_upstream(kind, cfg, external, hip_image=False):
    if cfg is None or isinstance(cfg, nn.Module):
        return cfg
    if hip_image:
        from . import image_encoder
        mine = {"backbone": (image_encoder.IMAGE_BACKBONES, "ResNet"), "neck": (image_encoder.IMAGE_NECKS, "SECONDFPN")}[kind]
        if cfg.get("type") == mine[1]:
            return mine[0].build(cfg)
    ours = {"backbone": registry.BACKBONES, "neck": registry.NECKS}[kind]
    if cfg.get("type") in ours:
        return ours.build(cfg)
    try:
        from mmdet3d.models import builder as m3b
    except Exception as e:
# ... 186 lines not shown

    def extract_feat(self, points, img, img_metas, search=None):
        img_voxel_feats = pts_voxel_feats = pts_feats = depth = img_feats = geom = None
        if img is not None:
            img_voxel_feats, depth, img_feats, geom = self.extract_img_feat(img, img_metas)
        if points is not None:
            pts_voxel_feats, pts_feats = self.extract_pts_feat(points)
        voxel_feats = self.fuse(img_voxel_feats, pts_voxel_feats, search)
        return voxel_feats, img_feats, pts_feats, depth, geom, img_voxel_feats

    def freeze_lidar_encoder(self, frozen=True):
        self._lidar_frozen = bool(frozen)
        if self.pts_middle_encoder is not None:
            for prm in self.pts_middle_encoder.parameters():
                prm.requires_grad_(not frozen)
            if frozen:
                self.pts_middle_encoder.eval()
        return self

    def train(self, mode=True):
        super().train(mode)
        if mode:
            self._pipe1 = None
        if mode and getattr(self, "_lidar_frozen", False) and getattr(self, "pts_middle_encoder", None) is not None:
            self.pts_middle_encoder.eval()
        return self

    def fuse(self, img_voxel_feats, pts_voxel_feats, search=None):
        if self.occ_fuser is not None:
            return self.occ_fuser(img_voxel_feats, pts_voxel_feats, search=search)
        assert (img_voxel_feats is None) or (pts_voxel_feats is None)
        return img_voxel_feats if pts_voxel_feats is None else pts_voxel_feats

    def search(self, img_voxel_feats, pts_voxel_feats):
        return self.occ_fuser.search(img_voxel_feats, pts_voxel_feats)

    def forward_hot_path(self, img_voxel_feats, pts_voxel_feats, gemo=None, img_feats=None, transform=None,
                         render=None, dense_fine=True, search=None):
        voxel_feats = self.fuse(img_voxel_feats, pts_voxel_feats, search)
        return self.decode(voxel_feats, gemo, img_feats, transform, render, dense_fine)

    def decode(self, voxel_feats, gemo=None, img_feats=None, transform=None, render=None, dense_fine=True,
               depth_only=False, fine_size=None, after_encoder=None, static=False, cam_geo=None):
        from . import core
        neck, head = self.semantic_neck, self.pts_bbox_head
        do_render = (self.use_rendering and self.test_rendering) if render is None else render
        rbranch = rendered = None
        if do_render:
            rbranch = core.Fork(0, voxel_feats.t.device if isinstance(voxel_feats, core.Rows) else voxel_feats.device)
            with rbranch:
                rendered = render_block(self.sigma_head, getattr(self, "rgb_head", None), to_rows(voxel_feats), gemo, 16,
                                        depth_only=depth_only or not hasattr(self, "rgb_head"), cam_geo=cam_geo)
        ibranch = head.fork_image_branch(img_feats, transform, to_rows(voxel_feats)) if hasattr(head, "fork_image_branch") else None
        mid = self.semantic_encoder.forward_rows(voxel_feats, readers=neck.lateral_packs() if hasattr(neck, "lateral_packs") else None)
        if after_encoder is not None:
            after_encoder()
        sem = neck.forward_rows(mid, readers=head.level_readers() if hasattr(head, "level_readers") else None)
        kw = dict(image_branch=ibranch) if ibranch is not None else {}
        output = self.pts_bbox_head(voxel_feats=sem, img_feats=img_feats, transform=transform, static=static, **kw)
        res = dict(voxel_feats=voxel_feats, pred_c=output['output_voxels'][0], pred_f=None,
                   output_voxels_fine=output['output_voxels_fine'], output_coords_fine=output['output_coords_fine'])
        if output['output_voxels_fine'] is not None and dense_fine:
            cf = self.pts_bbox_head.cascade_ratio
            pc = res['pred_c']
            size = fine_size or [pc.shape[2] * cf, pc.shape[3] * cf, pc.shape[4] * cf]
            res['pred_f'] = self.pts_bbox_head.scatter_fine(output['output_voxels_fine'][0],
                                                            output['output_coords_fine'][0], list(size),
                                                            count_dev=output.get('fine_count'))
            res['fine_count'] = output.get('fine_count')
        if do_render:
            rgbs, depths, maps = rendered
            rbranch.join(rgbs, depths, maps)
            res.update(rgbs=rgbs, depths=depths, render_maps=maps)
        return res

    def forward_train_hot_path(self, img_voxel_feats, pts_voxel_feats, gemo=None, img_feats=None, transform=None,
                               coarse_lin=None, render=True, generator=None, depth_only=False, search=None):
        from . import autograd as ag
        one = img_voxel_feats if img_voxel_feats is not None else pts_voxel_feats
        B, C, X, Y, Z = one.shape
        assert B == 1, "batch size 1 per GPU (coocc_ray.py:365)"
        V = X * Y * Z
        rows = lambda t: t.float().permute(0, 2, 3, 4, 1).reshape(V, t.shape[1])
        if self.occ_fuser is not None:
            sr = search
            if sr is None:
                with torch.no_grad():
                    sr = self.occ_fuser.search(img_voxel_feats.detach(), pts_voxel_feats.detach())
            self.occ_fuser.finish_bookkeeping(sr)
            cat4 = ag.fuser_fuse_train(self.occ_fuser, rows(img_voxel_feats).contiguous(), rows(pts_voxel_feats).contiguous(), sr)
            vf, geom = ag.con_enc_train(self.occ_fuser.con_enc, cat4, (1, X, Y, Z))
        else:
            assert (img_voxel_feats is None) or (pts_voxel_feats is None)
            vf, geom = rows(one).contiguous(), (1, X, Y, Z)
        levels = ag.trunk_forward_train(None, self.semantic_encoder, self.semantic_neck, vf, geom)
        head = self.pts_bbox_head
        out_rows, logit_rows = ag.occhead_coarse_train(head, levels)
        res = dict(voxel_rows=vf, levels=levels, out_voxel_rows=out_rows, logit_rows=logit_rows)
        if head.cascade_ratio != 1 and (head.sample_from_img or head.sample_from_voxel):
            if coarse_lin is None:
                coarse_lin = head.draw_fine_voxels(logit_rows.detach(), generator)
            if coarse_lin.numel():
                res["fine_logits"], res["fine_xyz"] = ag.fine_branch_train(head, out_rows, (1, X, Y, Z), coarse_lin.contiguous(),
                                                                           img_feats, transform)
        if render and self.use_rendering:
            rgb_head = None if (depth_only or not hasattr(self, "rgb_head")) else self.rgb_head
            res["rgbs"], res["depths"] = ag.render_block_train(self.sigma_head, rgb_head, vf, (X, Y, Z), gemo)
# ... 339 lines not shown
```

co_occ_amd/fuser.py:

```python
import torch
from torch import nn

from . import _lib, streams
from ._lib import call, ptr
from . import core as _core_mod
from .core import PackCache, PackedConv, Rows, conv_rows, gather_conv_rows
from .registry import FUSION_LAYERS

_I32, _F32, _I64 = torch.int32, torch.float32, torch.int64


_side = {}


def _side_stream(dev, cur, which=0):
    key = (dev.index, cur.cuda_stream, which)
    if key not in _side:
        _side[key] = streams.side_stream_for(cur, which) or torch.cuda.Stream(device=dev, priority=getattr(cur, "priority", 0))
    return _side[key]


FPS_HIGH_PRIORITY = __import__("os").environ.get("COOCC_FPS_HIGH_PRIORITY", "0") != "0"
_fps_hi = {}
FPS_MAX_BUCKETS = 8 * 1024
# ... 95 lines not shown
    winner = torch.empty(num, Q, device=dev, dtype=_I32)
    out = torch.empty(num, Q, device=dev, dtype=_I32)
    call("coocc_knn_assign", fps_num, num, max_cluster_samples, Q, float(dist_thresh), ptr(val), ptr(nn_), ptr(group),
         ptr(winner), ptr(out))
    return out


def _as_rows_view(x):
    if isinstance(x, Rows):
        return x
    if x.dim() != 5 or not x.is_cuda or x.dtype != _F32:
        return None
    B, C, X, Y, Z = x.shape
    sb, sc, sx, sy, sz = x.stride()
    S = sz
    if sc != 1 or S < C or S % 4 or sy != Z * S or sx != Y * Z * S or (B > 1 and sb != X * Y * Z * S):
        return None
    off = x.storage_offset()
    coff = off % S
    if coff + C > S or (x.data_ptr() - 4 * coff) % 16:
        return None
    base = torch.as_strided(x, (B * X * Y * Z, S), (S, 1), off - coff)
    return Rows(base, B, X, Y, Z, C, coff)


_concat_buffers = {}


def _register_concat(t):
    import weakref
    for k in [k for k, r in _concat_buffers.items() if r() is None]:
        del _concat_buffers[k]
    _concat_buffers[t.data_ptr()] = weakref.ref(t)


def _is_concat(t):
    r = _concat_buffers.get(t.data_ptr())
    base = r() if r is not None else None
    return base is not None and base.data_ptr() == t.data_ptr() and base.numel() == t.numel()


class SearchSlot:

    def __init__(self, C, knum, grid, device):
        X, Y, Z = grid
        V = X * Y * Z
        self.grid, self.C, self.V = (X, Y, Z), C, V
        self.cat4 = torch.empty(V, 4 * C, device=device, dtype=_F32)
        _register_concat(self.cat4)
        self.lin = torch.zeros(2, V, device=device, dtype=_I32)
        self.counts = torch.zeros(2, device=device, dtype=_I32)
        self.rows = torch.zeros(knum, V, device=device, dtype=_I32)
        self.rows_p = torch.zeros(knum, V, device=device, dtype=_I32)

        self.knum = knum
        self.near = torch.zeros(2, knum * V, device=device, dtype=_I32)
        self._native = None

    def img_rows(self):
        X, Y, Z = self.grid
        return Rows(self.cat4, 1, X, Y, Z, self.C, 0, persistent=True)

    def native_desc(self):
        if self._native is None:
            import ctypes
            X, Y, Z = self.grid
            d = _lib.SearchDesc()
            d.cat4 = self.cat4.data_ptr()
            d.C, d.X, d.Y, d.Z, d.K = self.C, X, Y, Z, self.knum
            d.fps_num, d.max_cluster, d.radius, d.dist_thresh = 2048, 200, 6.0, 13.3
            off = offset_table(Z, self.cat4.device)
            d.offsets, d.noff = off.data_ptr(), off.numel()
            d.lin, d.counts = self.lin.data_ptr(), self.counts.data_ptr()
            d.near_img, d.near_pts = self.near[0].data_ptr(), self.near[1].data_ptr()
            d.rows, d.rows_p = self.rows.data_ptr(), self.rows_p.data_ptr()
            need = int(_lib.load().coocc_fuser_search_ws(ctypes.byref(d)))
            ws = torch.empty(need, device=self.cat4.device, dtype=torch.uint8)
            d.ws, d.ws_bytes = ws.data_ptr(), need
            host = (ctypes.c_int32 * 2)()
            d.counts_host = ctypes.addressof(host)
            self._native = (d, ws, host, off)
        return self._native


class SearchResult:

    def __init__(self, cat4, lin_img, lin_pts):
        self.cat4, self.lin_img, self.lin_pts = cat4, lin_img, lin_pts
        self.rows = self.rows_p = self.near_img = self.near_pts = None
        self.done_main = self.done_side = None
        self.keep = ()
        self.slot = None
        self.counts = (lin_img.numel(), lin_pts.numel())

    def tensors(self):
        out = [self.cat4.t, self.lin_img, self.lin_pts]
        out += [t for t in (self.rows, self.rows_p, self.near_img, self.near_pts) if t is not None]
        return out + [t for t in self.keep if torch.is_tensor(t)]


@FUSION_LAYERS.register_module()
class BiFuser_N(nn.Module):
    def __init__(self, in_channels, out_channels, knum=1, norm_cfg=None):
        super().__init__()
        self.in_channels, self.out_channels, self.knum = in_channels, out_channels, knum
        self.con_enc = nn.Sequential(
            nn.Conv3d(in_channels * 4, out_channels * 2, 3, padding=1, bias=False),
            nn.BatchNorm3d(out_channels * 2), nn.ReLU(True),
            nn.Conv3d(in_channels * 2, out_channels, 3, padding=1, bias=False),
            nn.BatchNorm3d(out_channels), nn.ReLU(True))
        self.knn_enc = nn.Sequential(nn.Linear(in_channels * knum, out_channels), nn.ReLU())
        self._packs = PackCache(self)
        self.last_counts = None
        self.output_readers = None

    def set_conenc_tiles(self, tiles):
        self.conenc_tiles = None if tiles is None else (int(tiles[0]), int(tiles[1]))
        _core_mod.invalidate_packs(self)

    def _packed(self):
        def build():
            d = build_packs()
            import os
            from . import core as _core
            default = "4,4" if _core.CONV_ENGINE == "h2" else "2,2"
            forced = getattr(self, "conenc_tiles", None)
            t0, t3 = forced if forced is not None else [int(v) for v in os.environ.get("COOCC_CONENC_TILES", default).split(",")]
            d["c0"].wino_tile, d["c3"].wino_tile = t0, t3
            d["c0_dense"].wino_tile = t0
            d["conenc_tiles"] = (t0, t3)
            d["conenc_tiles_large"] = (t0, t3) if ("COOCC_CONENC_TILES" in os.environ or forced is not None) else (2, 2)
            return d

        def build_packs():
            C, W0 = self.in_channels, self.con_enc[0].weight
            Co = W0.shape[0]
            dense_idx = list(range(0, C)) + list(range(3 * C, 4 * C))
            w_cols = W0[:, C:3 * C].reshape(Co, 2 * C, 27).permute(2, 0, 1).reshape(27 * Co, 2 * C).contiguous()
            return dict(
                c0_dense=PackedConv(W0[:, dense_idx].contiguous(), bn=self.con_enc[1], ksize=3, pad=1),
                c0_sparse=PackedConv(w_cols),
                c0=PackedConv(self.con_enc[0].weight, bn=self.con_enc[1], ksize=3, pad=1),
                c3=PackedConv(self.con_enc[3].weight, bn=self.con_enc[4], ksize=3, pad=1),
                knn=PackedConv(self.knn_enc[0].weight, bias=self.knn_enc[0].bias, tap_major=True, taps=self.knum))
        return self._packs.get_modules((self.con_enc, self.knn_enc), build)

    def fps_NN_fast(self, query, key, fps_num, radius, max_cluster_samples, dist_thresh, num):
        q = query[:, 1:].float().contiguous()
        k = key[:, 1:].float().contiguous()
        out = _fps_nn_xyz(q, k, fps_num, radius, max_cluster_samples, dist_thresh, num).long()
        return out[0] if num == 1 else out

    def concat_buffer(self, B, X, Y, Z, device):
        C = self.in_channels
        cat4 = torch.empty(B * X * Y * Z, 4 * C, device=device, dtype=_F32)
        _register_concat(cat4)
        return Rows(cat4, B, X, Y, Z, C, 0)

    def search(self, img_voxel_feats, pts_voxel_feats, slot=None):
        img_r, pts_r = _as_rows_view(img_voxel_feats), _as_rows_view(pts_voxel_feats)
        one = img_r if img_r is not None else img_voxel_feats
        if isinstance(one, Rows):
            B, C, X, Y, Z = one.B, one.C, one.X, one.Y, one.Z
            dev = one.t.device
        else:
            B, C, X, Y, Z = one.shape
            dev = one.device
        V = X * Y * Z
        if dev.type != "cuda":
            raise _lib.CooccError("BiFuser_N runs on the GPU only (no CPU fallback)")
        flags = torch.empty(2, B * V, device=dev, dtype=torch.uint8)
        if img_r is None and pts_r is None:
            img = img_voxel_feats.float().contiguous()
            pts = pts_voxel_feats.float().contiguous()
            cat4 = torch.empty(B * V, 4 * C, device=dev, dtype=_F32)
            call("coocc_fuser_prepare", ptr(img), ptr(pts), ptr(cat4), ptr(flags[0]), ptr(flags[1]), B, C, V)
        else:
            in_place = (img_r is not None and img_r.t.shape[1] == 4 * C and img_r.coff == 0 and img_r.t.is_contiguous()
                        and (_is_concat(img_r.t) or (slot is not None and img_r.t.data_ptr() == slot.cat4.data_ptr())))
            if slot is not None:
                assert in_place and img_r.t.data_ptr() == slot.cat4.data_ptr() and B == 1, \
                    "search(slot=...): the camera rows must already sit in slot 0 of the slot's concat buffer"
            cat4 = img_r.t if in_place else torch.empty(B * V, 4 * C, device=dev, dtype=_F32)
            img = img_r if img_r is not None else img_voxel_feats.float().contiguous()
            pts = pts_r if pts_r is not None else pts_voxel_feats.float().contiguous()
            src = lambda r: (r.data(), 1, r.stride) if isinstance(r, Rows) else (ptr(r), 0, 0)
            call("coocc_fuser_prepare_rows", *src(img), *src(pts), ptr(cat4), ptr(flags[0]), ptr(flags[1]), B, C, V)
        assert slot is None or (img_r is not None or pts_r is not None), "search(slot=...) takes channels-last producers"
        lin = slot.lin if slot is not None else torch.empty(2, B * V, device=dev, dtype=_I32)
        counts = slot.counts if slot is not None else torch.empty(2, device=dev, dtype=_I32)
        ws = torch.empty(2, B * V // 1024 + 2, device=dev, dtype=_I32)
        for i in range(2):
            call("coocc_compact_flags", ptr(flags[i]), B * V, ptr(lin[i]), ptr(counts[i:i + 1]), ptr(ws[i]),
                 ws[i].numel() * 4)
        Ni, Np = (int(v) for v in _lib.host_read(counts))
        self.last_counts = (Ni, Np)
        lin_img, lin_pts = lin[0, :Ni], lin[1, :Np]
        xyz = torch.empty(Ni + Np, 3, device=dev, dtype=_F32)
        if Ni:
            call("coocc_lin_to_coords", ptr(lin_img), Ni, X, Y, Z, ptr(xyz[:Ni]), None)
        if Np:
            call("coocc_lin_to_coords", ptr(lin_pts), Np, X, Y, Z, ptr(xyz[Ni:]), None)
        xyz_img, xyz_pts = xyz[:Ni], xyz[Ni:]
        K = self.knum
        kw = dict(fps_num=2048, radius=6, max_cluster_samples=200, dist_thresh=13.3, num=K)
        sr = SearchResult(Rows(cat4, B, X, Y, Z, 4 * C), lin_img, lin_pts)
        sr.slot = slot
        cur = torch.cuda.current_stream(dev)
        if Np and Ni:
            vox = (X, Y, Z) if B == 1 else None
            side = _side_stream(dev, cur)
            side.wait_stream(cur)
            with torch.cuda.stream(side):
                sr.near_pts = _fps_nn_xyz(xyz_img, xyz_pts, q_lin=lin_img if vox else None, k_lin=lin_pts if vox else None, grid=vox,
                                          which=1, home=cur, **kw)
                sr.rows_p = slot.rows_p[:, :Ni] if slot is not None else torch.empty(K, Ni, device=dev, dtype=_I32)
                base, nbase = (lin_pts, Np) if K == 1 else (lin_img, Ni)
                for k in range(K):
                    call("coocc_index_rows_i32", ptr(base), nbase, ptr(sr.near_pts[k]), Ni, ptr(sr.rows_p[k]))
                sr.done_side = streams.new_event()
                sr.done_side.record()
            sr.near_img = _fps_nn_xyz(xyz_pts, xyz_img, q_lin=lin_pts if vox else None, k_lin=lin_img if vox else None, grid=vox,
                                      which=0, home=cur, **kw)
            sr.rows = slot.rows[:, :Np] if slot is not None else torch.empty(K, Np, device=dev, dtype=_I32)
            for k in range(K):
                call("coocc_index_rows_i32", ptr(lin_img), Ni, ptr(sr.near_img[k]), Np, ptr(sr.rows[k]))
            sr.keep = (xyz, lin, img, pts)
        elif Np or Ni:
            raise IndexError("BiFuser_N: one modality has no non-empty voxel (the reference fails on empty keys)")
        sr.done_main = streams.new_event()
        sr.done_main.record()
        return sr

    def search_native(self, pts_voxel_feats, slot):
        import ctypes
        X, Y, Z = slot.grid
        dev = slot.cat4.device
        pts_r = _as_rows_view(pts_voxel_feats)
        B = pts_r.B if pts_r is not None else pts_voxel_feats.shape[0]
        if B != 1 or (X + 3) // 4 * ((Y + 3) // 4) * ((Z + 7) // 8) > FPS_MAX_BUCKETS:
            return self.search(slot.img_rows().as_ncdhw(), pts_voxel_feats, slot=slot)
        d, _, host, _ = slot.native_desc()
        if pts_r is not None:
            d.pts, d.pts_rows, d.pts_stride = pts_r.t.data_ptr() + 4 * pts_r.coff, 1, pts_r.stride
            keep = pts_r.t
        else:
            keep = pts_voxel_feats.float().contiguous()
            d.pts, d.pts_rows, d.pts_stride = keep.data_ptr(), 0, 0
        cur = torch.cuda.current_stream(dev)
        side = _side_stream(dev, cur)
        rc = _lib.load().coocc_fuser_search(ctypes.byref(d), ctypes.c_void_p(cur.cuda_stream), ctypes.c_void_p(side.cuda_stream))
        if rc == 1:
            return self.search(slot.img_rows().as_ncdhw(), pts_voxel_feats, slot=slot)
        _lib.check(rc)
        Ni, Np = int(host[0]), int(host[1])
        self.last_counts = (Ni, Np)
        K, V = self.knum, slot.V
        sr = SearchResult(Rows(slot.cat4, 1, X, Y, Z, 4 * self.in_channels), slot.lin[0, :Ni], slot.lin[1, :Np])
        sr.slot = slot
        sr.near_img = slot.near[0, :K * Np].view(K, Np)
        sr.near_pts = slot.near[1, :K * Ni].view(K, Ni)
        sr.rows, sr.rows_p = slot.rows[:, :Np], slot.rows_p[:, :Ni]
        sr.keep = (keep,)
        sr.done_main = streams.new_event()
        sr.done_main.record()
        sr.done_side = sr.done_main
        return sr

    def finish(self, sr):
        cat4 = sr.cat4.t
        dev = cat4.device
        C = self.in_channels
        cur = torch.cuda.current_stream(dev)
        packs = self._packed()
        sr.done_main.wait(cur)
        for t in sr.tensors():
            t.record_stream(cur)
        if sr.rows is not None and sr.slot is not None:
            sr.done_side.wait(cur)
            self.finish_static(sr.slot)
            self.last_near = (sr.near_img, sr.near_pts)
        elif sr.rows is not None:
            sr.done_side.wait(cur)
            h2 = self._g1_h2(cat4, packs)
            gather_conv_rows(cat4, 0, packs["knn"], sr.rows, sr.lin_pts, cat4, 2 * C, C, C, src_h2=h2)
            gather_conv_rows(cat4, C, packs["knn"], sr.rows_p, sr.lin_img, cat4, 3 * C, 0, C, src_h2=h2)
            self.last_near = (sr.near_img, sr.near_pts)
        return sr.cat4, (sr.lin_img, sr.lin_pts)

    def _g1_h2(self, cat4, packs):
        import os
        from . import core
        if os.environ.get("COOCC_G1_H2_ONCE", "1") == "0":
            return None
        sh = core.g1_sources_h2(cat4, self.in_channels, packs["knn"])
        return None if sh is None else (sh, 0, 2 * self.in_channels)

    def finish_static(self, slot):
        C = self.in_channels
        packs = self._packed()
        cat4 = slot.cat4
        h2 = self._g1_h2(cat4, packs)
        gather_conv_rows(cat4, 0, packs["knn"], slot.rows, slot.lin[1], cat4, 2 * C, C, C, count_dev=slot.counts[1:2], src_h2=h2)
        gather_conv_rows(cat4, C, packs["knn"], slot.rows_p, slot.lin[0], cat4, 3 * C, 0, C, count_dev=slot.counts[0:1], src_h2=h2)
        X, Y, Z = slot.grid
        return Rows(cat4, 1, X, Y, Z, 4 * C)

    def forward_static(self, slot):
        packs = self._packed()
        cat4 = self.finish_static(slot)
        x = self.con_enc0(cat4, slot.lin[1], packs, count_dev=slot.counts[1:2])
        return conv_rows(x, packs["c3"], relu=True, twin_for=self._readers())

    def finish_bookkeeping(self, sr):
        cur = torch.cuda.current_stream(sr.cat4.t.device)
        sr.done_main.wait(cur)
        if sr.done_side is not None:
            sr.done_side.wait(cur)
        for t in sr.tensors():
            t.record_stream(cur)
        if sr.rows is not None:
            self.last_near = (sr.near_img, sr.near_pts)

    def fuse(self, img_voxel_feats, pts_voxel_feats, search=None):
        return self.finish(search if search is not None else self.search(img_voxel_feats, pts_voxel_feats))

    def forward(self, img_voxel_feats, pts_voxel_feats, search=None):
        if not (img_voxel_feats.t if isinstance(img_voxel_feats, Rows) else img_voxel_feats).is_cuda:
            raise _lib.CooccError("BiFuser_N runs on the GPU only (no CPU fallback)")
        if self.training:
            from . import autograd as ag
            assert img_voxel_feats.shape[0] == 1, "BiFuser_N training path: batch size 1 per GPU (samples_per_gpu=1 upstream)"
            with torch.no_grad():
                sr = search if search is not None else self.search(img_voxel_feats.detach(), pts_voxel_feats.detach())
            (ri, geom), (rp, _) = ag.rows_from_ncdhw(img_voxel_feats), ag.rows_from_ncdhw(pts_voxel_feats)
            self.finish_bookkeeping(sr)
            x, g = ag.con_enc_train(self.con_enc, ag.fuser_fuse_train(self, ri, rp, sr), geom)
            return ag.ncdhw_from_rows(x, g)
        packs = self._packed()
        cat4, (_, lin_pts) = self.fuse(img_voxel_feats, pts_voxel_feats, search)
        x = self.con_enc0(cat4, lin_pts, packs)
        x = conv_rows(x, packs["c3"], relu=True, twin_for=self._readers())
        return x.as_ncdhw()

    def _readers(self):
        return tuple(self.output_readers()) if self.output_readers is not None else ()

    @staticmethod
    def c0_capacity(V):
        return int(SPLIT_C0_MAX_DENSITY * V)

    def con_enc0(self, cat4, lin_pts, packs, count_dev=None):
        from . import core
        C, V, dev = self.in_channels, cat4.V * cat4.B, cat4.t.device
        Np = int(lin_pts.numel())
        pd = packs["c0_dense"]
        if "conenc_tiles" in packs:
            t0, t3 = packs["conenc_tiles_large"] if cat4.V > DENSE_C0_MAX_VOXELS else packs["conenc_tiles"]
            packs["c0"].wino_tile = pd.wino_tile = t0
            packs["c3"].wino_tile = t3
        split = SPLIT_C0 or (core.CONV_ENGINE == "h2" and V > DENSE_C0_MAX_VOXELS and "COOCC_SPLIT_C0" not in __import__("os").environ)
        plan = core.wino_plan(cat4, pd, V, 1) if (split and core.CONV_DTYPE == "f32") else None
        if count_dev is not None:
            if plan is None or cat4.B != 1:
                return conv_rows(cat4, packs["c0"], relu=True)
            Np = self.c0_capacity(V)
        elif plan is None or Np == 0 or Np > SPLIT_C0_MAX_DENSITY * V or cat4.B != 1:
            return conv_rows(cat4, packs["c0"], relu=True)
        ps = packs["c0_sparse"]
        Co = pd.Cout
        P = core.scratch(dev, "c0P", Np * 27 * Co)
        src = ptr(cat4.t, offset=cat4.coff + C)
        d = core.conv_desc(dev, in_=src, w=ptr(ps.w), out=ptr(P), gather=ptr(lin_pts), M=Np, Cin=2 * C, Cout=27 * Co, taps=1,
                           in_stride=cat4.stride, out_stride=27 * Co, B=1, Yi=1, Zi=1, Xo=1, Yo=1, Zo=1,
                           Xi=V,
                           ksize=1, stride=1, splitk=1, tile_hint=core.TILE_HINT)
        if count_dev is not None:
            d.M_dev, d.gather_stride = ptr(count_dev, _I32), lin_pts.numel()
        h2 = core.CONV_ENGINE == "h2" and core.H2_DIRECT and (2 * C) % 32 == 0
        if h2:
            rh = core.scratch(dev, "c0rows", Np * 2 * C)
            call("coocc_rows_to_h2_gather", src, cat4.stride, ptr(lin_pts), Np, ptr(count_dev, _I32) if count_dev is not None else None,
                 2 * C, 1.0, ptr(rh))
            d.in_, d.in_stride, d.w, d.gather, d.gather_stride = ptr(rh), 2 * C, ptr(ps.h2_pack()), None, 0
            d.Xi, d.Xo = Np, Np
            d.mfma_dtype, d.alpha = 3, 1.0
        core.launch_conv(d, dev, "k_gemm_h2w c0-sparse" if h2 else lambda: core.conv_kernel_name(Np, 27 * Co, True) + " c0-sparse",
                         2.0 * Np * 2 * C * 27 * Co)
        vmap = torch.empty(V, device=dev, dtype=_I32)
        if count_dev is not None:
            call("coocc_voxel_index_map_dev", ptr(lin_pts), int(lin_pts.numel()), ptr(count_dev, _I32), V, ptr(vmap))
        else:
            call("coocc_voxel_index_map", ptr(lin_pts), Np, V, ptr(vmap))
        S = core.Rows(torch.empty(V, Co, device=dev, dtype=_F32), cat4.B, cat4.X, cat4.Y, cat4.Z, Co)
        call("coocc_sparse_tap_sum", ptr(P), ptr(vmap), cat4.B, cat4.X, cat4.Y, cat4.Z, Co, ptr(pd.scale), ptr(S.t), Co, int(Np))
        out = core.Rows(torch.empty(V, Co, device=dev, dtype=_F32), cat4.B, cat4.X, cat4.Y, cat4.Z, Co)
        return core.conv_rows_wino(cat4, pd, out, True, S, plan, in_ranges=[(0, C), (3 * C, C)])
```

co_occ_amd/lidar_trunk.py:

```python
import ctypes

import torch
from torch import nn

from . import _lib, core
from .backbone import build_bn
from .core import PackCache, PackedConv, Rows, conv_rows, fold_bn
from ._lib import call, ptr
from .registry import BACKBONES, NECKS

_F32 = torch.float32


class _Cfg(dict):
    __getattr__ = dict.get


def rows_as_bczyx(r):
    v = r.t.view(r.B, r.X, r.Y, r.Z, r.stride)
    if r.coff or r.stride != r.C:
        v = v[..., r.coff:r.coff + r.C]
    v = v.permute(0, 4, 3, 2, 1)
    if not r.persistent:
        v._coocc_rows_zyx = (r, v._version)
# ... 79 lines not shown
                 init_cfg=None, pretrained=None):
        super().__init__()
        assert len(layer_strides) == len(layer_nums)
        assert len(out_channels) == len(layer_nums)
        assert not (init_cfg and pretrained), 'init_cfg and pretrained cannot be setting at the same time'
        in_filters = list(in_channels) if isinstance(in_channels, (list, tuple)) else [in_channels, *out_channels[:-1]]
        conv_cfg = _Cfg(conv_cfg)
        self.is_cascade = is_cascade
        self.kernel_type = conv_cfg.get("type", "Conv3d")
        _conv_type(conv_cfg, "SECOND3D")
        kernel = _kernel_zyx(conv_cfg.pop("kernel", (1, 3, 3)), "SECOND3D")
        bias = bool(conv_cfg.get("bias", True))
        padding = tuple((k - 1) // 2 for k in kernel)
        self.kernel, self.layer_strides = kernel, [int(s) for s in layer_strides]
        blocks = []
        for i, n in enumerate(layer_nums):
            s = self.layer_strides[i]
            block = [nn.Conv3d(in_filters[i], out_channels[i], kernel, stride=(1, s, s), padding=padding, bias=bias),
                     build_bn(norm_cfg, out_channels[i]), nn.ReLU(inplace=True)]
            for _ in range(n):
                block += [nn.Conv3d(out_channels[i], out_channels[i], kernel, padding=padding, bias=bias),
                          build_bn(norm_cfg, out_channels[i]), nn.ReLU(inplace=True)]
            blocks.append(nn.Sequential(*block))
        self.blocks = nn.ModuleList(blocks)
        self.init_cfg = dict(type='Pretrained', checkpoint=pretrained) if isinstance(pretrained, str) else \
            dict(type='Kaiming', layer=self.kernel_type)
        self._packs = PackCache(self)

    def init_weights(self):
        if self.init_cfg.get("type") == "Pretrained":
            raise NotImplementedError("SECOND3D.init_weights: loading init_cfg checkpoint %r is the caller's (load_state_dict)"
                                      % self.init_cfg.get("checkpoint"))
        for m in self.modules():
            if isinstance(m, nn.Conv3d):
                nn.init.kaiming_normal_(m.weight, mode='fan_out', nonlinearity='relu')
                if m.bias is not None:
                    nn.init.constant_(m.bias, 0)

    def _packed(self):
        kz, ky, kx = self.kernel

        def build():
            out = []
            for i, blk in enumerate(self.blocks):
                s, packs = self.layer_strides[i], []
                for j in range(0, len(blk), 3):
                    st = (s, s, 1) if j == 0 else (1, 1, 1)
                    packs.append(PackedConv(core.zyx_weight(blk[j].weight), bn=blk[j + 1], bias=blk[j].bias, kernel=(kx, ky, kz),
                                            strides=st))
                out.append(packs)
            return out
        return self._packs.get_modules((self,), build)

    def forward_rows(self, x, readers=None):
        _eval_only(self)
        p = self._packed()
        outs = []
        for i, packs in enumerate(p):
            h = x
            for j, pc in enumerate(packs):
                if j + 1 < len(packs):
                    nxt = (packs[j + 1],)
                else:
                    nxt = tuple(readers[i]) if readers is not None else ()
                    if self.is_cascade and i + 1 < len(p):
                        nxt += (p[i + 1][0],)
                h = conv_rows(h, pc, relu=True, twin_for=nxt)
            outs.append(h)
            if self.is_cascade:
                x = h
        return outs

    def forward(self, x):
        _eval_only(self)
        return tuple(rows_as_bczyx(r) for r in self.forward_rows(bczyx_to_rows(x)))


@NECKS.register_module()
class SECOND3DFPN(nn.Module):
    def __init__(self, in_channels=[128, 128, 256], out_channels=[256, 256, 256], upsample_strides=[1, 2, 4],
                 norm_cfg=dict(type='BN3d', eps=1e-3, momentum=0.01), upsample_cfg=dict(type='deconv3d', bias=False),
                 conv_cfg=dict(type='Conv3d', bias=False), extra_conv=None, use_conv_for_no_stride=False, use_for_distill=False,
                 init_cfg=None):
        super().__init__()
        assert len(out_channels) == len(upsample_strides) == len(in_channels)
        if use_for_distill:
            raise NotImplementedError("SECOND3DFPN: use_for_distill (the before-ReLU taps of cross-modality distillation) is not built")
        if upsample_cfg.get("type") != "deconv3d":
            raise NotImplementedError("SECOND3DFPN: upsample type %r is not built; only 'deconv3d'" % upsample_cfg.get("type"))
        _conv_type(conv_cfg, "SECOND3DFPN")
        if not 1 <= len(out_channels) <= 4:
            raise NotImplementedError("SECOND3DFPN: %d levels; the sum kernel takes 1-4" % len(out_channels))
        if len(set(out_channels)) != 1:
            raise ValueError("SECOND3DFPN: sum(ups) needs equal out_channels, got %r" % (out_channels,))
        self.in_channels, self.out_channels = list(in_channels), list(out_channels)
        self.extra_conv = dict(extra_conv) if extra_conv is not None else None
        self.fp16_enabled = False
        self.use_for_distill = False
        self.upsample_strides = []
        deblocks = []
        for i, oc in enumerate(out_channels):
            s = upsample_strides[i]
            if s != int(s) or int(s) not in (1, 2, 4, 8):
                raise NotImplementedError("SECOND3DFPN: upsample stride %r; deconvs whose kernel = stride = (1,s,s), s in 1, 2, 4, 8 "
                                          "only (fractional strides are strided convs)" % (s,))
            s = int(s)
            self.upsample_strides.append(s)
# ... 103 lines not shown
```

include/coocc_hip.h:

```cpp
#ifndef COOCC_HIP_H
#define COOCC_HIP_H

#include <stddef.h>
#include <stdint.h>

#ifdef __cplusplus
extern "C" {
#endif

#define COOCC_OK 0
#define COOCC_EINVAL (-1)
#define COOCC_EHIP (-2)
#define COOCC_ENOMEM (-3)

const char* coocc_last_error(void);
int coocc_abi_version(void);

int coocc_device_cu_count(int* n);
int coocc_stream_create_cu_mask(const uint32_t* mask_host, int nwords, void** stream_out);
int coocc_stream_destroy(void* stream);

int coocc_event_create(int flags, void** event_out);
int coocc_event_destroy(void* event);
int coocc_event_record(void* event, void* stream);
int coocc_stream_wait_event(void* stream, void* event);
int coocc_event_synchronize(void* event);
int coocc_event_query(void* event);
int coocc_event_elapsed_ms(void* start, void* stop, float* ms);


int coocc_ncdhw_to_ndhwc(const float* src, float* dst, int B, int C, int V, int dst_stride,
                         int dst_coff, void* stream);
int coocc_ndhwc_to_ncdhw(const float* src, float* dst, int B, int C, int V, int src_stride,
                         int src_coff, void* stream);

int coocc_fuser_prepare(const float* img, const float* pts, float* cat4, uint8_t* flag_img,
                        uint8_t* flag_pts, int B, int C, int V, void* stream);
int coocc_fuser_prepare_rows(const float* img, int img_rows, int img_stride, const float* pts, int pts_rows,
                             int pts_stride, float* cat4, uint8_t* flag_img, uint8_t* flag_pts, int B, int C, int V,
                             void* stream);

int coocc_compact_flags(const uint8_t* flags, int total, int32_t* lin, int32_t* count, void* ws,
                        size_t ws_bytes, void* stream);
int coocc_compact_flags_ex(const uint8_t* flags, int total, int32_t* lin, int32_t* count, int32_t* map, void* ws,
                           size_t ws_bytes, void* stream);
int coocc_lin_to_coords(const int32_t* lin, int n, int X, int Y, int Z, float* xyz, int64_t* bxyz,
                        void* stream);


int coocc_furthest_point_sampling(int b, int n, int m, const float* points, float* temp,
                                  int32_t* idx, void* stream);

size_t coocc_fps_voxels_ws(int X, int Y, int Z);
int coocc_fps_voxels(const int32_t* lin, int n, int X, int Y, int Z, int m, int32_t* idx, void* ws,
                     size_t ws_bytes, void* stream);
int coocc_fps_voxels_pair(const int32_t* lin0, int n0, int32_t* idx0, void* ws0, const int32_t* lin1, int n1, int32_t* idx1,
                          void* ws1, size_t ws_bytes_each, int X, int Y, int Z, int m, void* stream);

int coocc_ball_query(int b, int n, int m, float min_radius, float max_radius, int nsample,
                     const float* new_xyz, const float* xyz, int32_t* idx, void* stream);

#define COOCC_SEARCH_SMALL 1
typedef struct coocc_search_desc {
  float* cat4;
  const float* pts;
  int pts_rows, pts_stride;
  int C, X, Y, Z, K;
  int fps_num, max_cluster;
  float radius, dist_thresh;
  const uint32_t* offsets;
  int noff;
  int32_t* lin;
  int32_t* counts;
  int32_t* near_img;
  int32_t* near_pts;
  int32_t* rows;
  int32_t* rows_p;
  void* ws;
  size_t ws_bytes;
  int32_t* counts_host;
} coocc_search_desc;
size_t coocc_fuser_search_ws(const coocc_search_desc* d);
int coocc_fuser_search(coocc_search_desc* d, void* stream, void* side_stream);

int coocc_voxel_index_map(const int32_t* lin, int n, int nvox, int32_t* map, void* stream);
int coocc_voxel_index_map_dev(const int32_t* lin, int n_cap, const int32_t* n_dev, int nvox, int32_t* map, void* stream);
int coocc_ball_query_voxels(int m, float min_radius, float max_radius, int nsample, int X, int Y, int Z,
                            const int32_t* centre_ord, const int32_t* lin_q, const int32_t* map_q, int32_t* idx,
                            void* stream);
int coocc_knn_topk_voxels(int nq, int nk, int K, int X, int Y, int Z, const int32_t* rep_ord, const int32_t* lin_q,
                          const int32_t* map_k, const uint32_t* offsets, int noff, const float* q, const float* key,
                          float* val, int32_t* idx, void* stream);

int coocc_knn_topk(int nq, int nk, int K, const float* q, const float* key, float* val,
                   int32_t* idx, void* stream);

int coocc_knn_assign(int nc, int K, int ns, int nq, float dist_thresh, const float* val,
                     const int32_t* nn, const int32_t* group, int32_t* winner, int32_t* out,
                     void* stream);
int coocc_knn_threshold(int nq, float dist_thresh, const float* val, const int32_t* nn,
                        int32_t* out, void* stream);
int coocc_index_rows_i32(const int32_t* base, int nbase, const int32_t* sel, int n, int32_t* rows,
                         void* stream);


int64_t coocc_conv_pack_weights(const float* w_host, int Cout, int Cin, int taps, int tap_major,
                                float* packed_host);

typedef struct coocc_conv_desc {
  const float* in;
  const float* w;
  float* out;
  const float* scale;
  const float* bias;
  const float* res;
  const int32_t* gather;
  const int32_t* out_rows;
  float* ws;
  int64_t ws_floats;
  int M, Cin, Cout, taps;
  int in_stride, out_stride, res_stride;
  int B, Xi, Yi, Zi, Xo, Yo, Zo, ksize, stride, pad;
  int relu, res_mode;
  int splitk;
  int tile_hint;
  int kx, ky, kz;
  int px, py, pz;
  int wgroup_rows;
  int mfma_dtype;
  float alpha;
  const int32_t* M_dev;
  int gather_stride;
  void* out16;
  int out16_stride;
  int out_h2;
  void* out_h2_twin;
  int32_t* tile_sem;
  int tile_sem_ints;
  const float* alpha_dev;
  int sx, sy, sz;
} coocc_conv_desc;

int coocc_conv_fwd(const coocc_conv_desc* d, void* stream);

int coocc_rows_to_bf16(const float* in, int in_stride, int64_t rows, int C, void* out_bf16, void* stream);

int coocc_rows_to_h2(const float* in, int in_stride, int64_t rows, int C, float scale, void* out_h2, void* stream);
int coocc_rows_to_h2_ex(const float* in, int in_stride, int64_t rows, int C, float scale, const float* scale_dev, void* out_h2,
                        void* stream);
int coocc_rows_to_f16(const float* in, int in_stride, int64_t rows, int C, void* out_f16, void* stream);
int coocc_rows_to_h2_gather(const float* in, int in_stride, const int32_t* row_ids, int64_t n_cap, const int32_t* n_dev,
                            int C, float scale, void* out_h2, void* stream);

int coocc_wino_input(const float* in, int in_stride, int B, int X, int Y, int Z, int C, int tile, float* V,
                     int64_t group_rows, void* stream);
int coocc_wino_input_strided(const float* in, int in_stride, int B, int X, int Y, int Z, int C, int tile, float* V,
                             int vstride, int64_t group_rows, void* stream);
int coocc_wino_input_h2(const float* in, int in_stride, int B, int X, int Y, int Z, int C, int tile, void* V,
                        int vstride, int64_t group_rows, float scale, void* stream);
int coocc_wino_input_h2_ex(const float* in, int in_stride, int B, int X, int Y, int Z, int C, int tile, void* V,
                           int vstride, int64_t group_rows, float scale, const float* scale_dev, void* stream);
int coocc_sparse_tap_sum(const float* P, const int32_t* map, int B, int X, int Y, int Z, int Cout, const float* scale,
                         float* S, int s_stride, int p_rows, void* stream);
int coocc_wino_output(const float* Mb, int64_t group_rows, int B, int X, int Y, int Z, int C, int tile, float* out,
                      int out_stride, const float* scale, const float* bias, const float* res, int res_stride,
                      int relu, void* stream);
int coocc_wino_output_ex(const float* Mb, int64_t group_rows, int B, int X, int Y, int Z, int C, int tile, float* out,
                         int out_stride, const float* scale, const float* bias, const float* res, int res_stride,
                         int relu, void* out_h2_twin, void* stream);
int coocc_render_heads_h2(const void* x_h2, int V, int Cin, int width, const void* ws0_pack, const float* bs0,
                          const float* ws1, const float* bs1, const void* const* wr_packs_host,
                          const float* const* br_host, int n_rgb_hidden, const float* wr_out, const float* br_out,
                          float* table, int activate, void* stream);
int64_t coocc_wino_pack_weights_h2_dev(const float* w, int Cout, int Cin, int tile, int dgrad, void* packed, void* stream);
int64_t coocc_conv_pack_weights_h2_dev(const float* w, int Cout, int Cin, int taps, int mode, void* packed, void* stream);
int coocc_h2_overflow(int reset);
#define COOCC_FAULT_SPARSE_ORDINAL 1
int coocc_device_fault(int reset);
int64_t coocc_wino_pack_weights_dev(const float* w, int Cout, int Cin, int tile, int dgrad, float* packed, void* stream);
int coocc_wino_gradout(const float* dy, int dy_stride, int B, int X, int Y, int Z, int C, int tile, float* dM,
                       int64_t group_rows, void* stream);
int coocc_wino_ztap_table(int64_t rows_total, int Z, int32_t* table, void* stream);
int coocc_wino_wgrad(const float* V, const float* dM, int64_t group_rows, int Z, int Cin, int Cout, int tile,
                     const int32_t* ztap_table, float* dw, int accumulate, float* ws, int64_t ws_floats,
                     void* stream);
int coocc_rows_to_kh2(const float* x, int stride, int64_t rows, int64_t rows_pad, int C, float scale, const float* scale_dev,
                      void* out_kh2, void* stream);
int coocc_wino_operand_kh2(int which, const float* x, int x_stride, int B, int X, int Y, int Z, int C, int tile, void* out_kh2,
                           int64_t group_rows, float scale, const float* scale_dev, void* stream);
int coocc_conv_wgrad_h2(const void* x_kh2, const void* dy_kh2, int64_t rows_pad, int Cin, int Cout, float alpha,
                        const float* alpha_dev, float* dw, int accumulate, float* ws, int64_t ws_floats, void* stream);
int coocc_wino_wgrad_h2(const void* V_kh2, const void* dM_kh2, int64_t group_rows, int Z, int Cin, int Cout, int tile,
                        float alpha, const float* alpha_dev, float* dw, int accumulate, float* ws, int64_t ws_floats,
                        void* stream);

int64_t coocc_conv_pack_weights_dev(const float* w, int Cout, int Cin, int taps, int mode, float* packed,
                                    void* stream);
int coocc_conv_tap_table(int B, int Xi, int Yi, int Zi, int Xo, int Yo, int Zo, int ksize, int stride, int pad,
                         int dgrad, int32_t* table, void* stream);
int coocc_conv_epilogue_bwd(const float* dout, int dout_stride, const float* out, int out_stride,
                            const float* scale, int M, int C, int relu, float* dacc, int dacc_stride,
                            float* dres, int dres_stride, int dres_accumulate, float* dbias,
                            int dbias_accumulate, float* ws, int64_t ws_floats, void* stream);
#define COOCC_AMAX_WORDS 2048
int coocc_conv_epilogue_bwd_ex(const float* dout, int dout_stride, const float* out, int out_stride,
                               const float* scale, int M, int C, int relu, float* dacc, int dacc_stride,
                               float* dres, int dres_stride, int dres_accumulate, float* dbias,
                               int dbias_accumulate, float* ws, int64_t ws_floats, uint32_t* amax_word, float* scale2,
                               float target, void* stream);
int coocc_conv_wgrad(const float* in, int in_rows, int in_stride, const float* dacc, int dacc_stride,
                     const int32_t* table, int M, int Cin, int Cout, int taps, float* dw, int accumulate,
                     float* ws, int64_t ws_floats, void* stream);
int coocc_conv_wgrad_h2t(const float* in, int in_rows, int in_stride, const float* dacc, int dacc_stride,
                         const int32_t* table, int M, int Cin, int Cout, int taps, const float* scale2,
// ... 284 lines not shown
```

Measured before the change: 259.6.

## Skip unread fp32 rows and zero-fill via occupancy masks in fuser and backbone

The fuser prepare step now records a per-voxel occupancy byte and can leave the fused concat columns unfilled. The masked Winograd input transform for con_enc.0 then treats those columns as zero from the occupancy bits. The H2 conversion of the g1 sources is limited to the listed occupied rows, and backbone block outputs whose only readers take the H2 twin skip the fp32 store. Together these cut memory writes and traffic, at the cost of rows that are twin-only and raise errors if any fp32 reader appears, plus stricter preconditions on routing.

```diff
diff --git a/co_occ_amd/_lib.py b/co_occ_amd/_lib.py
--- a/co_occ_amd/_lib.py
+++ b/co_occ_amd/_lib.py
@@ -28,7 +28,7 @@
                [(n, c_int) for n in ("C", "X", "Y", "Z", "K", "fps_num", "max_cluster")] + \
                [("radius", ctypes.c_float), ("dist_thresh", ctypes.c_float), ("offsets", c_void_p), ("noff", c_int)] + \
                [(n, c_void_p) for n in ("lin", "counts", "near_img", "near_pts", "rows", "rows_p", "ws")] + \
-               [("ws_bytes", ctypes.c_size_t), ("counts_host", c_void_p)]
+               [("ws_bytes", ctypes.c_size_t), ("counts_host", c_void_p), ("occ", c_void_p), ("no_zero_fused", c_int)]
 
 
 P, I, F, Z, L = c_void_p, c_int, c_float, c_size_t, c_int64
@@ -50,12 +50,15 @@
     "coocc_rows_to_h2": (I, [P, I, L, I, F, P, P]),
     "coocc_rows_to_h2_ex": (I, [P, I, L, I, F, P, P, P]),
     "coocc_rows_to_h2_gather": (I, [P, I, P, L, P, I, F, P, P]),
+    "coocc_rows_to_h2_lists": (I, [P, I, L, I, P, P, P, P, P, P]),
     "coocc_rows_to_f16": (I, [P, I, L, I, P, P]),
     "coocc_wino_input_h2": (I, [P, I, I, I, I, I, I, I, P, I, L, F, P]),
     "coocc_wino_input_h2_ex": (I, [P, I, I, I, I, I, I, I, P, I, L, F, P, P]),
+    "coocc_wino_input_h2_masked": (I, [P, I, I, I, I, I, I, I, P, I, L, F, P, P, P, P, I, P]),
     "coocc_ndhwc_to_ncdhw": (I, [P, P, I, I, I, I, I, P]),
     "coocc_fuser_prepare": (I, [P, P, P, P, P, I, I, I, P]),
     "coocc_fuser_prepare_rows": (I, [P, I, I, P, I, I, P, P, P, I, I, I, P]),
+    "coocc_fuser_prepare_rows_occ": (I, [P, I, I, P, I, I, P, P, P, I, I, I, P, I, P]),
     "coocc_compact_flags": (I, [P, I, P, P, P, Z, P]),
     "coocc_compact_flags_ex": (I, [P, I, P, P, P, P, Z, P]),
     "coocc_lin_to_coords": (I, [P, I, I, I, I, P, P, P]),
diff --git a/co_occ_amd/backbone.py b/co_occ_amd/backbone.py
--- a/co_occ_amd/backbone.py
+++ b/co_occ_amd/backbone.py
@@ -41,10 +41,10 @@
             d["ds"] = PackedConv(self.downsample[0].weight, bn=self.downsample[1], ksize=1, stride=self.stride)
         return d
 
-    def run(self, x, p, readers=()):
+    def run(self, x, p, readers=(), fp32_unread=False):
         out = conv_rows(x, p["c1"], relu=True, twin_for=(p["c2"],))
         res = conv_rows(x, p["ds"], relu=False) if "ds" in p else x
-        return conv_rows(out, p["c2"], relu=True, res=res, twin_for=readers)
+        return conv_rows(out, p["c2"], relu=True, res=res, twin_for=readers, fp32_unread=fp32_unread)
 
 
 @BACKBONES.register_module()
@@ -92,7 +92,8 @@
                         blocks=[[b.packed() for b in layer] for layer in self.layers])
         return self._packs.get_modules((self,), build)
 
-    def forward_rows(self, x, readers=None):
+    def forward_rows(self, x, readers=None, internal=False):
+        from . import core
         _eval_only(self)
         p = self._packed()
         flat = [bp for layer in p["blocks"] for bp in layer]
@@ -104,9 +105,13 @@
                 n += 1
                 nxt = flat[n] if n < len(flat) else {}
                 rd = [nxt.get("c1"), nxt.get("ds")]
-                if readers is not None and i in self.out_indices and bp is p["blocks"][i][-1]:
+                last = bp is p["blocks"][i][-1]
+                if readers is not None and i in self.out_indices and last:
                     rd += list(readers[self.out_indices.index(i)])
-                x = blk.run(x, bp, tuple(rd))
+                known = last and internal and (i not in self.out_indices or readers is not None)
+                grid = (x.B,) + core.out_dims(x.X, x.Y, x.Z, bp["c1"])
+                drop = bool(known and (not nxt or "ds" in nxt) and core.fp32_unread_by(grid, rd))
+                x = blk.run(x, bp, tuple(rd), fp32_unread=drop)
             if i in self.out_indices:
                 res.append(x)
         return res
diff --git a/co_occ_amd/core.py b/co_occ_amd/core.py
--- a/co_occ_amd/core.py
+++ b/co_occ_amd/core.py
@@ -98,10 +98,11 @@
 
 class Rows:
 
-    __slots__ = ("t", "B", "X", "Y", "Z", "C", "coff", "h16", "h2", "persistent", "aux")
+    __slots__ = ("t", "B", "X", "Y", "Z", "C", "coff", "h16", "h2", "persistent", "aux", "twin_only")
 
     def __init__(self, t, B, X, Y, Z, C, coff=0, persistent=False):
         self.t, self.B, self.X, self.Y, self.Z, self.C, self.coff = t, B, X, Y, Z, C, coff
+        self.twin_only = False
         self.persistent = persistent
         self.aux = None
         self.h16 = None
@@ -116,9 +117,13 @@
         return self.X * self.Y * self.Z
 
     def data(self):
+        if self.twin_only:
+            raise _lib.CooccError("these rows were written as their H2 twin only (conv_rows(fp32_unread=True)): no fp32 rows to read")
         return ptr(self.t, offset=self.coff)
 
     def as_ncdhw(self):
+        if self.twin_only:
+            raise _lib.CooccError("these rows were written as their H2 twin only (conv_rows(fp32_unread=True)): no fp32 rows to view")
         v = self.t.view(self.B, self.X, self.Y, self.Z, self.stride)
         if self.coff or self.stride != self.C:
             v = v[..., self.coff:self.coff + self.C]
@@ -465,18 +470,31 @@
     return CONV_ENGINE == "h2" and CONV_DTYPE == "f32" and rows.C % 32 == 0 and takes_h2(rows, consumers)
 
 
-def conv_rows_wino(x, pc, out, relu, res, plan, in_ranges=None, twin=False):
+def fp32_unread_by(rows, consumers):
+    g = (rows.B, rows.X, rows.Y, rows.Z) if isinstance(rows, Rows) else rows
+    real = [pc for pc in consumers if pc is not None]
+    return bool(real) and CONV_ENGINE == "h2" and CONV_DTYPE == "f32" and all(route(*g, pc) == "h2" for pc in real)
+
+
+def conv_rows_wino(x, pc, out, relu, res, plan, in_ranges=None, twin=False, in_mask=None, fp32_unread=False):
     dev = x.t.device
     tile, pts, Tx, Ty, rows, G, hint = plan
     V = _wino_buffer(dev, "V", pts * G * pc.Cin)
     Mb = _wino_buffer(dev, "M", pts * G * pc.Cout)
     h2 = h2_capable(pc) and all(c % 32 == 0 for _, c in (in_ranges or []))
+    if in_mask is not None and (not h2 or in_ranges is not None):
+        raise _lib.CooccError("conv_rows(in_mask=...) needs the split-f16 Winograd path over whole rows")
     wp = pc.wino_h2_pack(tile) if h2 else pc.wino_pack(tile)
     vscale = H2_WINO_SCALE[tile]
     sdev = getattr(pc, "operand_scale_dev", None) if h2 else None
     with TIMER.region("k_wino_in", 4.0 * x.V * pc.Cin + 4.0 * pts * rows * pc.Cin):
         if in_ranges is None and not h2:
             call("coocc_wino_input", x.data(), x.stride, x.B, x.X, x.Y, x.Z, pc.Cin, tile, ptr(V), G)
+        elif in_mask is not None:
+            occ, ends, bits = in_mask
+            assert occ.dtype == torch.uint8 and occ.numel() == x.B * x.V and ends[-1] == pc.Cin and len(ends) == len(bits)
+            call("coocc_wino_input_h2_masked", x.data(), x.stride, x.B, x.X, x.Y, x.Z, pc.Cin, tile, ptr(V), pc.Cin, G, vscale,
+                 ptr(sdev), ptr(occ), _lib.host_i32(ends), _lib.host_i32(bits), len(ends))
         else:
             assert in_ranges is None or sum(c for _, c in in_ranges) == pc.Cin
             voff = 0
@@ -504,8 +522,11 @@
     tw = None
     if twin and h2 and pc.Cout % 32 == 0 and out.coff == 0 and out.stride % 4 == 0:
         tw = out.h2 = torch.empty(out.B * out.V, pc.Cout, device=dev, dtype=_F32)
-    with TIMER.region("k_wino_out", 4.0 * pts * rows * pc.Cout + 4.0 * x.V * pc.Cout * (2 if tw is not None else 1)):
-        call("coocc_wino_output_ex", ptr(Mb), G, x.B, x.X, x.Y, x.Z, pc.Cout, tile, out.data(), out.stride, ptr(pc.scale),
+    optr, ostride = out.data(), out.stride
+    if fp32_unread and tw is not None:
+        out.t, out.twin_only, optr = torch.empty(0, ostride, device=dev, dtype=_F32), True, None
+    with TIMER.region("k_wino_out", 4.0 * pts * rows * pc.Cout + 4.0 * x.V * pc.Cout * ((1 if tw is not None else 0) + (1 if optr is not None else 0))):
+        call("coocc_wino_output_ex", ptr(Mb), G, x.B, x.X, x.Y, x.Z, pc.Cout, tile, optr, ostride, ptr(pc.scale),
              ptr(pc.bias), res.data() if res is not None else None, res.stride if res is not None else 0, int(relu), ptr(tw))
     return out
 
@@ -531,7 +552,7 @@
     return tuple(out_dim(n, k, s, p) for n, k, s, p in zip((X, Y, Z), pc.kernel, pc.strides, pc.pads))
 
 
-def conv_rows(x, pc, relu=True, res=None, res_mode=0, out=None, splitk=0, twin_for=()):
+def conv_rows(x, pc, relu=True, res=None, res_mode=0, out=None, splitk=0, twin_for=(), in_mask=None, fp32_unread=False):
     Xo, Yo, Zo = out_dims(x.X, x.Y, x.Z, pc)
     M = x.B * Xo * Yo * Zo
     if out is None:
@@ -543,7 +564,9 @@
     family, plan, trim, kdims, taps = _route(x.B, x.X, x.Y, x.Z, pc, rm, splitk)
     twin = wants_h2_twin(out, twin_for)
     if family == "wino":
-        return conv_rows_wino(x, pc, out, relu, res, plan, twin=twin)
+        return conv_rows_wino(x, pc, out, relu, res, plan, twin=twin, in_mask=in_mask, fp32_unread=fp32_unread)
+    if in_mask is not None:
+        raise _lib.CooccError("conv_rows(in_mask=...) needs the split-f16 Winograd path, this layer takes %r" % family)
     dev = x.t.device
     d = conv_desc(dev, out=out.data(), scale=ptr(pc.scale), bias=ptr(pc.bias), res=res.data() if res is not None else None,
                   M=M, Cin=pc.Cin, Cout=pc.Cout, taps=taps, out_stride=out.stride, res_stride=res.stride if res is not None else 0,
@@ -633,10 +656,18 @@
     return bool(CONV_ENGINE == "h2" and H2_DIRECT and C % 32 == 0 and h2_capable(pc) and pc.h2_pack() is not None)
 
 
-def g1_sources_h2(cat4, C, pc):
+def g1_sources_h2(cat4, C, pc, lists=None):
     if not g1_h2_capable(pc, C) or cat4.shape[1] < 2 * C:
         return None
-    return rows_to_h2(cat4, 2 * C, 0, name="g1rows2")
+    if lists is None:
+        return rows_to_h2(cat4, 2 * C, 0, name="g1rows2")
+    n = cat4.shape[0]
+    xh = scratch(cat4.device, "g1rows2", n * 2 * C)
+    l0, c0, l1, c1 = lists
+    assert l0.numel() >= n and l1.numel() >= n, "g1_sources_h2: the row lists hold fewer than rows(cat4) entries"
+    call("coocc_rows_to_h2_lists", ptr(cat4), cat4.shape[1], n, C, ptr(l0, torch.int32), ptr(c0, torch.int32), ptr(l1, torch.int32),
+         ptr(c1, torch.int32), ptr(xh))
+    return xh
 
 
 def gather_conv_rows(src, src_coff, pc, gather, out_rows, dst, dst_coff, gate_coff, C, relu=True, count_dev=None, src_h2=None):
diff --git a/co_occ_amd/csrc/conv3d.hip b/co_occ_amd/csrc/conv3d.hip
--- a/co_occ_amd/csrc/conv3d.hip
+++ b/co_occ_amd/csrc/conv3d.hip
@@ -1036,7 +1036,7 @@
   if (p.relu && (p.relu == 1 || n < p.relu)) { v[0] = fmaxf(v[0], 0.f); v[1] = fmaxf(v[1], 0.f); v[2] = fmaxf(v[2], 0.f); v[3] = fmaxf(v[3], 0.f); }
   if (p.res_mode == 2) v = v * rs;
   if (p.out_h2) { store_h2(p.out, orow, p.out_stride, n, v); h2_guard(p.h2_flag, v); }
-  else *(f32x4*)(p.out + orow * p.out_stride + n) = v;
+  else if (p.out) *(f32x4*)(p.out + orow * p.out_stride + n) = v;
   if (p.out16) { store_f16(p.out16, orow, p.out16_stride, n, v); h2_guard(p.h2_flag, v); }
   if (p.out_h2t) { store_h2(p.out_h2t, orow, p.Cout, n, v); h2_guard(p.h2_flag, v); }
 }
@@ -1085,7 +1085,7 @@
 }
 
 extern "C" int coocc_conv_fwd(const coocc_conv_desc* d, void* stream) {
-  COOCC_CHECK_ARG(d && d->in && d->w && d->out, "conv_fwd: null pointer");
+  COOCC_CHECK_ARG(d && d->in && d->w && (d->out || ((d->mfma_dtype == 3) && d->out_h2_twin)), "conv_fwd: null pointer");
   COOCC_CHECK_ARG(d->M > 0 && d->Cin > 0 && d->Cout > 0 && d->taps > 0, "conv_fwd: bad sizes");
   COOCC_CHECK_ARG(d->Cin % 4 == 0 && d->in_stride % 4 == 0, "conv_fwd: Cin and in_stride must be multiples of 4");
   COOCC_CHECK_ARG(((uintptr_t)d->in & 15) == 0 && ((uintptr_t)d->w & 15) == 0, "conv_fwd: in/w must be 16-byte aligned");
diff --git a/co_occ_amd/csrc/gemm_h2.hip b/co_occ_amd/csrc/gemm_h2.hip
--- a/co_occ_amd/csrc/gemm_h2.hip
+++ b/co_occ_amd/csrc/gemm_h2.hip
@@ -902,6 +902,9 @@
   COOCC_CHECK_ARG(k.splitk == 1 || d->tile_sem || (!d->out_h2 && !d->out16 && !d->out_h2_twin) ||
                       ((d->Cout & 3) == 0 && (d->out_stride & 3) == 0 && (!d->res || (d->res_stride & 3) == 0) && (((uintptr_t)d->out) & 15) == 0),
                   "conv_fwd: split-K with an H2 / f16 output needs 16-byte aligned rows (Cout, strides % 4 == 0)");
+  COOCC_CHECK_ARG(d->out || (k.splitk > 1 && !d->tile_sem && d->out_h2_twin && !d->out_h2 && !d->out16 && (d->Cout & 3) == 0 &&
+                             (d->out_stride & 3) == 0 && (!d->res || (d->res_stride & 3) == 0)),
+                  "conv_fwd: a null fp32 output needs out_h2_twin and the split-K second pass (splitk > 1, no tile_sem, no out_h2 / out16)");
   COOCC_CHECK_ARG(k.splitk == 1 || !d->tile_sem || (long long)k.mtiles * k.ntiles <= d->tile_sem_ints,
                   "conv_fwd: tile_sem holds fewer counters than the launch has output tiles");
   dim3 grid(k.mtiles_per_xcd ? 8 * k.mtiles_per_xcd * k.ntiles : k.mtiles * k.ntiles, k.splitk);
@@ -1039,6 +1042,53 @@
   return COOCC_OK;
 }
 
+__global__ __launch_bounds__(256) void k_rows_to_h2_lists(const float* __restrict__ in, int in_stride, int rows, int C,
+                                                           char* __restrict__ out, const int32_t* __restrict__ list0,
+                                                           const int32_t* __restrict__ n0, const int32_t* __restrict__ list1,
+                                                           const int32_t* __restrict__ n1, int* __restrict__ flag) {
+  const int half = blockIdx.y;
+  const int32_t* __restrict__ list = half ? list1 : list0;
+  const int n = min(rows, max(0, half ? *n1 : *n0));
+  const int c8 = C >> 3;
+  const long long i = (long long)blockIdx.x * blockDim.x + threadIdx.x;
+  if (i >= (long long)n * c8) return;
+  const int r = (int)(i / c8);
+  const int c = (int)(i - (long long)r * c8) * 8 + half * C;
+  const int sr = list[r];
+  if ((unsigned)sr >= (unsigned)rows) return;
+  const float* src = in + (long long)sr * in_stride + c;
+  const f32x4 a = *(const f32x4*)src, b = *(const f32x4*)(src + 4);
+  f16x8 hi, lo;
+#pragma unroll
+  for (int e = 0; e < 4; ++e) {
+    _Float16 u, v;
+    split_h2(a[e], u, v); hi[e] = u; lo[e] = v;
+    split_h2(b[e], u, v); hi[4 + e] = u; lo[4 + e] = v;
+  }
+  char* o = out + (long long)sr * (2 * C) * 4 + (c >> 5) * 128 + (c & 31) * 2;
+  *(f16x8*)o = hi;
+  *(f16x8*)(o + 64) = lo;
+  h2_guard(flag, a);
+  h2_guard(flag, b);
+}
+
+extern "C" int coocc_rows_to_h2_lists(const float* in, int in_stride, int64_t rows, int C, const int32_t* list0, const int32_t* count0,
+                                      const int32_t* list1, const int32_t* count1, void* out_h2, void* stream) {
+  COOCC_CHECK_ARG(in && out_h2 && list0 && count0 && list1 && count1, "rows_to_h2_lists: null pointer");
+  COOCC_CHECK_ARG(rows >= 0 && rows < (1ll << 31) && C > 0 && C % 32 == 0 && in_stride % 4 == 0 && in_stride >= 2 * C,
+                  "rows_to_h2_lists: bad sizes (C % 32 == 0, in_stride % 4 == 0, in_stride >= 2 C)");
+  COOCC_CHECK_ARG(((uintptr_t)in & 15) == 0 && ((uintptr_t)out_h2 & 15) == 0 && ((uintptr_t)list0 & 3) == 0 && ((uintptr_t)list1 & 3) == 0 &&
+                      ((uintptr_t)count0 & 3) == 0 && ((uintptr_t)count1 & 3) == 0,
+                  "rows_to_h2_lists: rows must be 16-byte aligned, lists and counts 4-byte aligned");
+  if (rows == 0) return COOCC_OK;
+  int* flag = nullptr;
+  if (coocc_h2_flag_ptr(&flag) != COOCC_OK) return COOCC_EHIP;
+  hipLaunchKernelGGL(k_rows_to_h2_lists, dim3(cdiv(rows * (C / 8), 256), 2), dim3(256), 0, as_stream(stream), in, in_stride, (int)rows, C,
+                     (char*)out_h2, list0, count0, list1, count1, flag);
+  COOCC_LAUNCH_CHECK("k_rows_to_h2_lists");
+  return COOCC_OK;
+}
+
 __global__ __launch_bounds__(256) void k_rows_to_f16(const float* __restrict__ in, int in_stride, long long rows, int C, _Float16* __restrict__ out) {
   const int c8 = C >> 3;
   const long long i = (long long)blockIdx.x * blockDim.x + threadIdx.x;
diff --git a/co_occ_amd/csrc/layout.hip b/co_occ_amd/csrc/layout.hip
--- a/co_occ_amd/csrc/layout.hip
+++ b/co_occ_amd/csrc/layout.hip
@@ -146,18 +146,21 @@
 __global__ __launch_bounds__(256) void k_fuser_prepare_rows(const float* __restrict__ img, int img_rows, int img_stride,
                                                              const float* __restrict__ pts, int pts_rows, int pts_stride,
                                                              float* __restrict__ cat4, uint8_t* __restrict__ flag_img,
-                                                             uint8_t* __restrict__ flag_pts, int C, int V) {
+                                                             uint8_t* __restrict__ flag_pts, int C, int V, uint8_t* __restrict__ occ,
+                                                             int zero_fused) {
   __shared__ float tile[TV][TC + 1];
   const int b = blockIdx.y;
   const int v0 = blockIdx.x * TV;
   const int t = threadIdx.x;
   const int stride = 4 * C;
+  unsigned ob = 0;
   for (int mod = 0; mod < 2; ++mod) {
     const float* src = mod ? pts : img;
     const int rows = mod ? pts_rows : img_rows, sstride = mod ? pts_stride : img_stride;
     uint8_t* flags = mod ? flag_pts : flag_img;
     const bool in_place = rows && src == cat4 + mod * C && sstride == stride;
     float rsum = 0.f;
+    bool any = false;
     for (int c0 = 0; c0 < C; c0 += TC) {
       const int cn = min(TC, C - c0);
       if (rows) {
@@ -182,7 +185,7 @@
       }
       __syncthreads();
       if (t < TV)
-        for (int c = 0; c < cn; ++c) rsum += tile[t][c];
+        for (int c = 0; c < cn; ++c) { rsum += tile[t][c]; any |= tile[t][c] != 0.f; }
       if (!in_place)
         for (int i = t; i < TV * cn; i += 256) {
           int v = i / cn, c = i - v * cn;
@@ -191,7 +194,10 @@
       __syncthreads();
     }
     if (t < TV && v0 + t < V) flags[(size_t)b * V + v0 + t] = rsum != 0.f ? 1 : 0;
-  }
+    ob |= ((rsum != 0.f ? 1u : 0u) | (any ? 4u : 0u)) << mod;
+  }
+  if (occ && t < TV && v0 + t < V) occ[(size_t)b * V + v0 + t] = (uint8_t)ob;
+  if (!zero_fused) return;
   for (int i = t; i < TV * 2 * C; i += 256) {
     int v = i / (2 * C), c = i - v * 2 * C;
     if (v0 + v < V) cat4[((size_t)b * V + v0 + v) * stride + 2 * C + c] = 0.f;
@@ -202,19 +208,22 @@
 __global__ __launch_bounds__(256) void k_fuser_prepare_rows_fast(const float* __restrict__ img, int img_rows, int img_stride,
                                                                   const float* __restrict__ pts, int pts_rows, int pts_stride,
                                                                   float* __restrict__ cat4, uint8_t* __restrict__ flag_img,
-                                                                  uint8_t* __restrict__ flag_pts, int C, int V) {
+                                                                  uint8_t* __restrict__ flag_pts, int C, int V,
+                                                                  uint8_t* __restrict__ occ, int zero_fused) {
   __shared__ float tile[FV][FC + 1];
   const int b = blockIdx.y;
   const int v0 = blockIdx.x * FV;
   const int t = threadIdx.x;
   const int stride = 4 * C;
   const int rv = t >> 3, rc = (t & 7) * 4;
+  unsigned ob = 0;
   for (int mod = 0; mod < 2; ++mod) {
     const float* src = mod ? pts : img;
     const int rows = mod ? pts_rows : img_rows, sstride = mod ? pts_stride : img_stride;
     uint8_t* flags = mod ? flag_pts : flag_img;
     const bool in_place = rows && src == cat4 + mod * C && sstride == stride;
     float rsum = 0.f;
+    bool any = false;
     for (int c0 = 0; c0 < C; c0 += FC) {
       if (rows) {
 #pragma unroll
@@ -226,12 +235,13 @@
         }
         __syncthreads();
 #pragma unroll
-        for (int c = 0; c < FC; ++c) rsum += tile[t][c];
+        for (int c = 0; c < FC; ++c) { rsum += tile[t][c]; any |= tile[t][c] != 0.f; }
       } else {
 #pragma unroll 8
         for (int c = 0; c < FC; ++c) {
           const float x = v0 + t < V ? src[((size_t)b * C + c0 + c) * V + v0 + t] : 0.f;
           rsum += x;
+          any |= x != 0.f;
           tile[t][c] = x;
         }
         __syncthreads();
@@ -249,7 +259,10 @@
       __syncthreads();
     }
     if (v0 + t < V) flags[(size_t)b * V + v0 + t] = rsum != 0.f ? 1 : 0;
-  }
+    ob |= ((rsum != 0.f ? 1u : 0u) | (any ? 4u : 0u)) << mod;
+  }
+  if (occ && v0 + t < V) occ[(size_t)b * V + v0 + t] = (uint8_t)ob;
+  if (!zero_fused) return;
   const int vec_per_row = C >> 1;
   const f32x4 z = {0.f, 0.f, 0.f, 0.f};
   if (vec_per_row <= 256 && 256 % vec_per_row == 0) {
@@ -264,24 +277,32 @@
   }
 }
 
-extern "C" int coocc_fuser_prepare_rows(const float* img, int img_rows, int img_stride, const float* pts, int pts_rows,
-                                        int pts_stride, float* cat4, uint8_t* flag_img, uint8_t* flag_pts, int B, int C, int V,
-                                        void* stream) {
+extern "C" int coocc_fuser_prepare_rows_occ(const float* img, int img_rows, int img_stride, const float* pts, int pts_rows,
+                                            int pts_stride, float* cat4, uint8_t* flag_img, uint8_t* flag_pts, int B, int C, int V,
+                                            uint8_t* occ, int zero_fused, void* stream) {
   COOCC_CHECK_ARG(img && pts && cat4 && flag_img && flag_pts && B > 0 && C > 0 && V > 0, "fuser_prepare_rows: bad args");
+  COOCC_CHECK_ARG(occ || zero_fused, "fuser_prepare_rows: leaving the fused slots unfilled needs the occupancy map");
   COOCC_CHECK_ARG((!img_rows || img_stride >= C) && (!pts_rows || pts_stride >= C), "fuser_prepare_rows: row stride < C");
   const bool vec_ok = C % FC == 0 && ((uintptr_t)cat4 & 15) == 0 && (!img_rows || (img_stride % 4 == 0 && ((uintptr_t)img & 15) == 0)) &&
                       (!pts_rows || (pts_stride % 4 == 0 && ((uintptr_t)pts & 15) == 0));
   if (vec_ok) {
     hipLaunchKernelGGL(k_fuser_prepare_rows_fast, dim3(cdiv(V, FV), B), dim3(256), 0, as_stream(stream), img, img_rows, img_stride,
-                       pts, pts_rows, pts_stride, cat4, flag_img, flag_pts, C, V);
+                       pts, pts_rows, pts_stride, cat4, flag_img, flag_pts, C, V, occ, zero_fused);
     COOCC_LAUNCH_CHECK("k_fuser_prepare_rows_fast");
     return COOCC_OK;
   }
   dim3 grid(cdiv(V, TV), B);
   hipLaunchKernelGGL(k_fuser_prepare_rows, grid, dim3(256), 0, as_stream(stream), img, img_rows, img_stride, pts, pts_rows,
-                     pts_stride, cat4, flag_img, flag_pts, C, V);
+                     pts_stride, cat4, flag_img, flag_pts, C, V, occ, zero_fused);
   COOCC_LAUNCH_CHECK("k_fuser_prepare_rows");
   return COOCC_OK;
+}
+
+extern "C" int coocc_fuser_prepare_rows(const float* img, int img_rows, int img_stride, const float* pts, int pts_rows,
+                                        int pts_stride, float* cat4, uint8_t* flag_img, uint8_t* flag_pts, int B, int C, int V,
+                                        void* stream) {
+  return coocc_fuser_prepare_rows_occ(img, img_rows, img_stride, pts, pts_rows, pts_stride, cat4, flag_img, flag_pts, B, C, V, nullptr, 1,
+                                      stream);
 }
 
 #define CB 1024
diff --git a/co_occ_amd/csrc/search.hip b/co_occ_amd/csrc/search.hip
--- a/co_occ_amd/csrc/search.hip
+++ b/co_occ_amd/csrc/search.hip
@@ -76,7 +76,9 @@
   int32_t* lin_img = d->lin;
   int32_t* lin_pts = d->lin + V;
 
-  SRC(coocc_fuser_prepare_rows(d->cat4, 1, 4 * C, d->pts, d->pts_rows, d->pts_stride, d->cat4, w.flags, w.flags + V, 1, C, V, stream));
+  COOCC_CHECK_ARG(d->occ || !d->no_zero_fused, "fuser_search: leaving the fused slots unfilled needs the occupancy map");
+  SRC(coocc_fuser_prepare_rows_occ(d->cat4, 1, 4 * C, d->pts, d->pts_rows, d->pts_stride, d->cat4, w.flags, w.flags + V, 1, C, V, d->occ,
+                                   d->no_zero_fused ? 0 : 1, stream));
   SRC(coocc_compact_flags(w.flags, V, lin_img, d->counts, w.cws, (size_t)(V / 1024 + 2) * 4, stream));
   SRC(coocc_compact_flags(w.flags + V, V, lin_pts, d->counts + 1, w.cws + (V / 1024 + 2), (size_t)(V / 1024 + 2) * 4, stream));
   if (!((sdiag & 4) && d->counts_host[0] > 0)) COOCC_HIP(hipMemcpyAsync(d->counts_host, d->counts, 8, hipMemcpyDeviceToHost, s0));
diff --git a/co_occ_amd/csrc/winograd.hip b/co_occ_amd/csrc/winograd.hip
--- a/co_occ_amd/csrc/winograd.hip
+++ b/co_occ_amd/csrc/winograd.hip
@@ -100,10 +100,18 @@
   }
 }
 
-template <int N>
-__global__ __launch_bounds__(256) void k_wino_in_h2(const float* __restrict__ in, int in_stride, int B, int X, int Y, int Z,
-                                                     int C, int Tx, int Ty, size_t gstride_bytes, int vstride, float scale,
-                                                     char* __restrict__ V, int* __restrict__ flag, const float* __restrict__ scale_dev) {
+#define WINO_MASK_RANGES 8
+struct WinoMask {
+  const uint8_t* occ;
+  int n;
+  int end[WINO_MASK_RANGES];
+  int bits[WINO_MASK_RANGES];
+};
+
+template <int N, bool MASKED>
+__device__ __forceinline__ void wino_in_h2_body(const float* __restrict__ in, int in_stride, int B, int X, int Y, int Z, int C, int Tx,
+                                                int Ty, size_t gstride_bytes, int vstride, float scale, char* __restrict__ V,
+                                                int* __restrict__ flag, const float* __restrict__ scale_dev, const WinoMask& mk) {
   constexpr int MO = Wino<N>::M;
   if (scale_dev) scale *= *scale_dev;
   const int c4 = C >> 2;
@@ -116,6 +124,13 @@
   const int z = (int)(r % Z); r /= Z;
   const int ty = (int)(r % Ty); r /= Ty;
   const int tx = (int)(r % Tx); const int b = (int)(r / Tx);
+  int need = 0;
+  if (MASKED) {
+    need = mk.bits[0];
+#pragma unroll
+    for (int j = 1; j < WINO_MASK_RANGES; ++j)
+      if (j < mk.n && c >= mk.end[j - 1]) need = mk.bits[j];
+  }
   f32x4 t[N][N];
 #pragma unroll
   for (int e = 0; e < N; ++e) {
@@ -125,8 +140,10 @@
     for (int a = 0; a < N; ++a) {
       const int x = MO * tx - 1 + a;
       f32x4 v = {0.f, 0.f, 0.f, 0.f};
-      if ((unsigned)x < (unsigned)X && (unsigned)y < (unsigned)Y)
-        v = *(const f32x4*)(in + ((((size_t)b * X + x) * Y + y) * Z + z) * in_stride + c);
+      if ((unsigned)x < (unsigned)X && (unsigned)y < (unsigned)Y) {
+        const size_t vox = (((size_t)b * X + x) * Y + y) * Z + z;
+        if (!MASKED || need == 0 || (mk.occ[vox] & need)) v = *(const f32x4*)(in + vox * in_stride + c);
+      }
       d[a] = v;
     }
     Wino<N>::bt(d, q);
@@ -144,6 +161,59 @@
       h2_guard(flag, sv);
     }
   }
+}
+
+template <int N>
+__global__ __launch_bounds__(256) void k_wino_in_h2(const float* __restrict__ in, int in_stride, int B, int X, int Y, int Z,
+                                                     int C, int Tx, int Ty, size_t gstride_bytes, int vstride, float scale,
+                                                     char* __restrict__ V, int* __restrict__ flag, const float* __restrict__ scale_dev) {
+  wino_in_h2_body<N, false>(in, in_stride, B, X, Y, Z, C, Tx, Ty, gstride_bytes, vstride, scale, V, flag, scale_dev, WinoMask{});
+}
+
+template <int N>
+__global__ __launch_bounds__(256) void k_wino_in_h2m(const float* __restrict__ in, int in_stride, int B, int X, int Y, int Z,
+                                                      int C, int Tx, int Ty, size_t gstride_bytes, int vstride, float scale,
+                                                      char* __restrict__ V, int* __restrict__ flag, const float* __restrict__ scale_dev,
+                                                      WinoMask mk) {
+  wino_in_h2_body<N, true>(in, in_stride, B, X, Y, Z, C, Tx, Ty, gstride_bytes, vstride, scale, V, flag, scale_dev, mk);
+}
+
+extern "C" int coocc_wino_input_h2_masked(const float* in, int in_stride, int B, int X, int Y, int Z, int C, int tile, void* V,
+                                          int vstride, int64_t group_rows, float scale, const float* scale_dev, const uint8_t* occ,
+                                          const int32_t* range_end, const int32_t* range_bits, int nranges, void* stream) {
+  COOCC_CHECK_ARG(in && V && B > 0 && X > 0 && Y > 0 && Z > 0 && C > 0 && C % 32 == 0 && in_stride % 4 == 0, "wino_input_h2_masked: bad args");
+  COOCC_CHECK_ARG(((uintptr_t)in & 15) == 0, "wino_input_h2_masked: rows must be 16-byte aligned");
+  COOCC_CHECK_ARG(tile >= 2 && tile <= 4, "wino_input_h2_masked: tile must be 2, 3 or 4");
+  COOCC_CHECK_ARG(vstride >= C && vstride % 32 == 0 && ((uintptr_t)V & 127) == 0, "wino_input_h2_masked: V row stride / alignment");
+  COOCC_CHECK_ARG(scale > 0.f, "wino_input_h2_masked: scale must be positive");
+  COOCC_CHECK_ARG(occ && range_end && range_bits && nranges >= 1 && nranges <= WINO_MASK_RANGES,
+                  "wino_input_h2_masked: needs the occupancy map and 1..8 channel ranges");
+  WinoMask mk = {};
+  mk.occ = occ;
+  mk.n = nranges;
+  for (int j = 0; j < nranges; ++j) {
+    COOCC_CHECK_ARG(range_end[j] > (j ? range_end[j - 1] : 0) && range_end[j] % 4 == 0 && range_bits[j] >= 0 && range_bits[j] <= 255,
+                    "wino_input_h2_masked: range ends must ascend in multiples of 4, bits must fit a byte");
+    mk.end[j] = range_end[j];
+    mk.bits[j] = range_bits[j];
+  }
+  COOCC_CHECK_ARG(range_end[nranges - 1] == C, "wino_input_h2_masked: the last range must end at C");
+  const int Tx = (X + tile - 1) / tile, Ty = (Y + tile - 1) / tile;
+  const long long rows = (long long)B * Tx * Ty * Z;
+  COOCC_CHECK_ARG(group_rows >= rows, "wino_input_h2_masked: group_rows smaller than B*ceil(X/tile)*ceil(Y/tile)*Z");
+  const dim3 grid(cdiv(rows * (C / 4), 256));
+  const size_t gstride = (size_t)group_rows * vstride * 4;
+  hipStream_t s = as_stream(stream);
+  int* flag = nullptr;
+  if (coocc_h2_flag_ptr(&flag) != COOCC_OK) return COOCC_EHIP;
+  if (tile == 2)
+    hipLaunchKernelGGL(k_wino_in_h2m<4>, grid, dim3(256), 0, s, in, in_stride, B, X, Y, Z, C, Tx, Ty, gstride, vstride, scale, (char*)V, flag, scale_dev, mk);
+  else if (tile == 3)
+    hipLaunchKernelGGL(k_wino_in_h2m<5>, grid, dim3(256), 0, s, in, in_stride, B, X, Y, Z, C, Tx, Ty, gstride, vstride, scale, (char*)V, flag, scale_dev, mk);
+  else
+    hipLaunchKernelGGL(k_wino_in_h2m<6>, grid, dim3(256), 0, s, in, in_stride, B, X, Y, Z, C, Tx, Ty, gstride, vstride, scale, (char*)V, flag, scale_dev, mk);
+  COOCC_LAUNCH_CHECK("k_wino_in_h2m");
+  return COOCC_OK;
 }
 
 extern "C" int coocc_wino_input_h2_ex(const float* in, int in_stride, int B, int X, int Y, int Z, int C, int tile, void* V,
@@ -258,17 +328,17 @@
       if (yy >= Y) continue;
       const size_t orow = (((size_t)b * X + x) * Y + yy) * Z + z;
       f32x4 v = y[bb] * sc + bi;
-      float* o = out + orow * out_stride + c;
+      float* o = out ? out + orow * out_stride + c : nullptr;
       const float* rr = res ? res + orow * res_stride + c : nullptr;
       if (vec && (out_stride & 3) == 0 && (!res || (res_stride & 3) == 0)) {
         if (rr) v = v + *(const f32x4*)rr;
         if (relu) { v[0] = fmaxf(v[0], 0.f); v[1] = fmaxf(v[1], 0.f); v[2] = fmaxf(v[2], 0.f); v[3] = fmaxf(v[3], 0.f); }
-        *(f32x4*)o = v;
+        if (o) *(f32x4*)o = v;
         if (twin) { store_h2_pair(twin, orow, C, c, v); h2_guard(flag, v); }
       } else {
 #pragma unroll
         for (int e = 0; e < 4; ++e)
-          if (e < nc) {
+          if (e < nc && o) {
             float u = v[e] + (rr ? rr[e] : 0.f);
             o[e] = relu ? fmaxf(u, 0.f) : u;
           }
@@ -280,7 +350,7 @@
 extern "C" int coocc_wino_output_ex(const float* Mb, int64_t group_rows, int B, int X, int Y, int Z, int C, int tile, float* out,
                                     int out_stride, const float* scale, const float* bias, const float* res, int res_stride,
                                     int relu, void* out_h2_twin, void* stream) {
-  COOCC_CHECK_ARG(Mb && out && B > 0 && X > 0 && Y > 0 && Z > 0 && C > 0, "wino_output: bad args");
+  COOCC_CHECK_ARG(Mb && (out || out_h2_twin) && B > 0 && X > 0 && Y > 0 && Z > 0 && C > 0, "wino_output: bad args");
   COOCC_CHECK_ARG(tile >= 2 && tile <= 4, "wino_output: tile must be 2, 3 or 4");
   COOCC_CHECK_ARG(((uintptr_t)out & 15) == 0 && (!res || ((uintptr_t)res & 15) == 0), "wino_output: out/res must be 16-byte aligned");
   COOCC_CHECK_ARG(!out_h2_twin || (C % 32 == 0 && (out_stride & 3) == 0 && (!res || (res_stride & 3) == 0) && ((uintptr_t)out_h2_twin & 15) == 0),
diff --git a/co_occ_amd/detector.py b/co_occ_amd/detector.py
--- a/co_occ_amd/detector.py
+++ b/co_occ_amd/detector.py
@@ -262,7 +262,8 @@
                 rendered = render_block(self.sigma_head, getattr(self, "rgb_head", None), to_rows(voxel_feats), gemo, 16,
                                         depth_only=depth_only or not hasattr(self, "rgb_head"), cam_geo=cam_geo)
         ibranch = head.fork_image_branch(img_feats, transform, to_rows(voxel_feats)) if hasattr(head, "fork_image_branch") else None
-        mid = self.semantic_encoder.forward_rows(voxel_feats, readers=neck.lateral_packs() if hasattr(neck, "lateral_packs") else None)
+        mid = self.semantic_encoder.forward_rows(voxel_feats, readers=neck.lateral_packs() if hasattr(neck, "lateral_packs") else None,
+                                                 internal=bool(static))
         if after_encoder is not None:
             after_encoder()
         sem = neck.forward_rows(mid, readers=head.level_readers() if hasattr(head, "level_readers") else None)
diff --git a/co_occ_amd/fuser.py b/co_occ_amd/fuser.py
--- a/co_occ_amd/fuser.py
+++ b/co_occ_amd/fuser.py
@@ -171,7 +171,8 @@
         self.counts = torch.zeros(2, device=device, dtype=_I32)
         self.rows = torch.zeros(knum, V, device=device, dtype=_I32)
         self.rows_p = torch.zeros(knum, V, device=device, dtype=_I32)
-
+        self.occ = torch.zeros(V, device=device, dtype=torch.uint8)
+        self.fused_unfilled = False
         self.knum = knum
         self.near = torch.zeros(2, knum * V, device=device, dtype=_I32)
         self._native = None
@@ -193,7 +194,8 @@
             d.lin, d.counts = self.lin.data_ptr(), self.counts.data_ptr()
             d.near_img, d.near_pts = self.near[0].data_ptr(), self.near[1].data_ptr()
             d.rows, d.rows_p = self.rows.data_ptr(), self.rows_p.data_ptr()
-            need = int(_lib.load().coocc_fuser_search_ws(ctypes.byref(d)))
+            d.occ = self.occ.data_ptr()
+            need =int(_lib.load().coocc_fuser_search_ws(ctypes.byref(d)))
             ws = torch.empty(need, device=self.cat4.device, dtype=torch.uint8)
             d.ws, d.ws_bytes = ws.data_ptr(), need
             host = (ctypes.c_int32 * 2)()
@@ -211,6 +213,7 @@
         self.keep = ()
         self.slot = None
         self.counts = (lin_img.numel(), lin_pts.numel())
+        self.lin = self.counts_dev = None
 
     def tensors(self):
         out = [self.cat4.t, self.lin_img, self.lin_pts]
@@ -289,6 +292,7 @@
         if dev.type != "cuda":
             raise _lib.CooccError("BiFuser_N runs on the GPU only (no CPU fallback)")
         flags = torch.empty(2, B * V, device=dev, dtype=torch.uint8)
+        occ, unfilled = None, False
         if img_r is None and pts_r is None:
             img = img_voxel_feats.float().contiguous()
             pts = pts_voxel_feats.float().contiguous()
@@ -304,7 +308,12 @@
             img = img_r if img_r is not None else img_voxel_feats.float().contiguous()
             pts = pts_r if pts_r is not None else pts_voxel_feats.float().contiguous()
             src = lambda r: (r.data(), 1, r.stride) if isinstance(r, Rows) else (ptr(r), 0, 0)
-            call("coocc_fuser_prepare_rows", *src(img), *src(pts), ptr(cat4), ptr(flags[0]), ptr(flags[1]), B, C, V)
+            occ = slot.occ if slot is not None else torch.empty(B * V, device=dev, dtype=torch.uint8)
+            unfilled = slot is not None and self.c0_reads_masked(B, X, Y, Z)
+            call("coocc_fuser_prepare_rows_occ", *src(img), *src(pts), ptr(cat4), ptr(flags[0]), ptr(flags[1]), B, C, V, ptr(occ),
+                 0 if unfilled else 1)
+        if slot is not None:
+            slot.fused_unfilled = unfilled
         assert slot is None or (img_r is not None or pts_r is not None), "search(slot=...) takes channels-last producers"
         lin = slot.lin if slot is not None else torch.empty(2, B * V, device=dev, dtype=_I32)
         counts = slot.counts if slot is not None else torch.empty(2, device=dev, dtype=_I32)
@@ -325,6 +334,8 @@
         kw = dict(fps_num=2048, radius=6, max_cluster_samples=200, dist_thresh=13.3, num=K)
         sr = SearchResult(Rows(cat4, B, X, Y, Z, 4 * C), lin_img, lin_pts)
         sr.slot = slot
+        sr.lin, sr.counts_dev = lin, counts
+        sr.cat4.aux = dict(occ=occ, fused_unfilled=unfilled)
         cur = torch.cuda.current_stream(dev)
         if Np and Ni:
             vox = (X, Y, Z) if B == 1 else None
@@ -344,7 +355,7 @@
             sr.rows = slot.rows[:, :Np] if slot is not None else torch.empty(K, Np, device=dev, dtype=_I32)
             for k in range(K):
                 call("coocc_index_rows_i32", ptr(lin_img), Ni, ptr(sr.near_img[k]), Np, ptr(sr.rows[k]))
-            sr.keep = (xyz, lin, img, pts)
+            sr.keep = (xyz, lin, img, pts, counts, occ)
         elif Np or Ni:
             raise IndexError("BiFuser_N: one modality has no non-empty voxel (the reference fails on empty keys)")
         sr.done_main = streams.new_event()
@@ -366,6 +377,9 @@
         else:
             keep = pts_voxel_feats.float().contiguous()
             d.pts, d.pts_rows, d.pts_stride = keep.data_ptr(), 0, 0
+        unfilled = self.c0_reads_masked(1, X, Y, Z)
+        d.no_zero_fused = int(unfilled)
+        slot.fused_unfilled = unfilled
         cur = torch.cuda.current_stream(dev)
         side = _side_stream(dev, cur)
         rc = _lib.load().coocc_fuser_search(ctypes.byref(d), ctypes.c_void_p(cur.cuda_stream), ctypes.c_void_p(side.cuda_stream))
@@ -377,6 +391,8 @@
         K, V = self.knum, slot.V
         sr = SearchResult(Rows(slot.cat4, 1, X, Y, Z, 4 * self.in_channels), slot.lin[0, :Ni], slot.lin[1, :Np])
         sr.slot = slot
+        sr.lin, sr.counts_dev = slot.lin, slot.counts
+        sr.cat4.aux = dict(occ=slot.occ, fused_unfilled=unfilled)
         sr.near_img = slot.near[0, :K * Np].view(K, Np)
         sr.near_pts = slot.near[1, :K * Ni].view(K, Ni)
         sr.rows, sr.rows_p = slot.rows[:, :Np], slot.rows_p[:, :Ni]
@@ -401,29 +417,35 @@
             self.last_near = (sr.near_img, sr.near_pts)
         elif sr.rows is not None:
             sr.done_side.wait(cur)
-            h2 = self._g1_h2(cat4, packs)
+            h2 = self._g1_h2(cat4, packs, sr.lin, sr.counts_dev)
             gather_conv_rows(cat4, 0, packs["knn"], sr.rows, sr.lin_pts, cat4, 2 * C, C, C, src_h2=h2)
             gather_conv_rows(cat4, C, packs["knn"], sr.rows_p, sr.lin_img, cat4, 3 * C, 0, C, src_h2=h2)
             self.last_near = (sr.near_img, sr.near_pts)
         return sr.cat4, (sr.lin_img, sr.lin_pts)
 
-    def _g1_h2(self, cat4, packs):
+    def _g1_h2(self, cat4, packs, lin=None, counts_dev=None):
         import os
         from . import core
         if os.environ.get("COOCC_G1_H2_ONCE", "1") == "0":
             return None
-        sh = core.g1_sources_h2(cat4, self.in_channels, packs["knn"])
+        lists = None
+        if lin is not None and counts_dev is not None:
+            j = 1 if self.knum == 1 else 0
+            lists = (lin[0], counts_dev[0:1], lin[j], counts_dev[j:j + 1])
+        sh = core.g1_sources_h2(cat4, self.in_channels, packs["knn"], lists)
         return None if sh is None else (sh, 0, 2 * self.in_channels)
 
     def finish_static(self, slot):
         C = self.in_channels
         packs = self._packed()
         cat4 = slot.cat4
-        h2 = self._g1_h2(cat4, packs)
+        h2 = self._g1_h2(cat4, packs, slot.lin, slot.counts)
         gather_conv_rows(cat4, 0, packs["knn"], slot.rows, slot.lin[1], cat4, 2 * C, C, C, count_dev=slot.counts[1:2], src_h2=h2)
         gather_conv_rows(cat4, C, packs["knn"], slot.rows_p, slot.lin[0], cat4, 3 * C, 0, C, count_dev=slot.counts[0:1], src_h2=h2)
         X, Y, Z = slot.grid
-        return Rows(cat4, 1, X, Y, Z, 4 * C)
+        out = Rows(cat4, 1, X, Y, Z, 4 * C)
+        out.aux = dict(occ=slot.occ, fused_unfilled=slot.fused_unfilled)
+        return out
 
     def forward_static(self, slot):
         packs = self._packed()
@@ -469,6 +491,30 @@
     def c0_capacity(V):
         return int(SPLIT_C0_MAX_DENSITY * V)
 
+    def _c0_split_possible(self, B, X, Y, Z):
+        from . import core
+        V = B * X * Y * Z
+        split = SPLIT_C0 or (core.CONV_ENGINE == "h2" and V > DENSE_C0_MAX_VOXELS and "COOCC_SPLIT_C0" not in __import__("os").environ)
+        return bool(split and core.CONV_DTYPE == "f32" and B == 1
+                    and core._wino_plan_geom(B, X, Y, Z, self._packed()["c0_dense"], V, 1) is not None)
+
+    def c0_reads_masked(self, B, X, Y, Z):
+        from . import core
+        pc = self._packed()["c0"]
+        return bool(core.CONV_DTYPE == "f32" and core.h2_capable(pc) and core.route(B, X, Y, Z, pc) == "wino"
+                    and not self._c0_split_possible(B, X, Y, Z))
+
+    def _c0_dense(self, cat4, packs):
+        aux = cat4.aux or {}
+        occ = aux.get("occ")
+        C = self.in_channels
+        if occ is not None and cat4.coff == 0 and self.c0_reads_masked(cat4.B, cat4.X, cat4.Y, cat4.Z):
+            return conv_rows(cat4, packs["c0"], relu=True, in_mask=(occ, (C, 2 * C, 3 * C, 4 * C), (4, 8, 2, 1)))
+        if aux.get("fused_unfilled"):
+            raise _lib.CooccError("BiFuser_N: the fused columns of these concat rows were left unfilled for the masked form of "
+                                  "con_enc.0, which the current settings do not take: search again")
+        return conv_rows(cat4, packs["c0"], relu=True)
+
     def con_enc0(self, cat4, lin_pts, packs, count_dev=None):
         from . import core
         C, V, dev = self.in_channels, cat4.V * cat4.B, cat4.t.device
@@ -482,10 +528,13 @@
         plan = core.wino_plan(cat4, pd, V, 1) if (split and core.CONV_DTYPE == "f32") else None
         if count_dev is not None:
             if plan is None or cat4.B != 1:
-                return conv_rows(cat4, packs["c0"], relu=True)
+                return self._c0_dense(cat4, packs)
             Np = self.c0_capacity(V)
         elif plan is None or Np == 0 or Np > SPLIT_C0_MAX_DENSITY * V or cat4.B != 1:
-            return conv_rows(cat4, packs["c0"], relu=True)
+            return self._c0_dense(cat4, packs)
+        if (cat4.aux or {}).get("fused_unfilled"):
+            raise _lib.CooccError("BiFuser_N: the fused columns of these concat rows were left unfilled for the masked form of "
+                                  "con_enc.0, which the current settings do not take: search again")
         ps = packs["c0_sparse"]
         Co = pd.Cout
         P = core.scratch(dev, "c0P", Np * 27 * Co)
diff --git a/co_occ_amd/lidar_trunk.py b/co_occ_amd/lidar_trunk.py
--- a/co_occ_amd/lidar_trunk.py
+++ b/co_occ_amd/lidar_trunk.py
@@ -155,7 +155,7 @@
             return out
         return self._packs.get_modules((self,), build)
 
-    def forward_rows(self, x, readers=None):
+    def forward_rows(self, x, readers=None, internal=False):
         _eval_only(self)
         p = self._packed()
         outs = []
diff --git a/include/coocc_hip.h b/include/coocc_hip.h
--- a/include/coocc_hip.h
+++ b/include/coocc_hip.h
@@ -39,6 +39,9 @@
 int coocc_fuser_prepare_rows(const float* img, int img_rows, int img_stride, const float* pts, int pts_rows,
                              int pts_stride, float* cat4, uint8_t* flag_img, uint8_t* flag_pts, int B, int C, int V,
                              void* stream);
+int coocc_fuser_prepare_rows_occ(const float* img, int img_rows, int img_stride, const float* pts, int pts_rows,
+                                 int pts_stride, float* cat4, uint8_t* flag_img, uint8_t* flag_pts, int B, int C, int V,
+                                 uint8_t* occ, int zero_fused, void* stream);
 
 int coocc_compact_flags(const uint8_t* flags, int total, int32_t* lin, int32_t* count, void* ws,
                         size_t ws_bytes, void* stream);
@@ -79,6 +82,8 @@
   void* ws;
   size_t ws_bytes;
   int32_t* counts_host;
+  uint8_t* occ;
+  int no_zero_fused;
 } coocc_search_desc;
 size_t coocc_fuser_search_ws(const coocc_search_desc* d);
 int coocc_fuser_search(coocc_search_desc* d, void* stream, void* side_stream);
@@ -151,6 +156,8 @@
 int coocc_rows_to_f16(const float* in, int in_stride, int64_t rows, int C, void* out_f16, void* stream);
 int coocc_rows_to_h2_gather(const float* in, int in_stride, const int32_t* row_ids, int64_t n_cap, const int32_t* n_dev,
                             int C, float scale, void* out_h2, void* stream);
+int coocc_rows_to_h2_lists(const float* in, int in_stride, int64_t rows, int C, const int32_t* list0, const int32_t* count0,
+                           const int32_t* list1, const int32_t* count1, void* out_h2, void* stream);
 
 int coocc_wino_input(const float* in, int in_stride, int B, int X, int Y, int Z, int C, int tile, float* V,
                      int64_t group_rows, void* stream);
@@ -160,6 +167,9 @@
                         int vstride, int64_t group_rows, float scale, void* stream);
 int coocc_wino_input_h2_ex(const float* in, int in_stride, int B, int X, int Y, int Z, int C, int tile, void* V,
                            int vstride, int64_t group_rows, float scale, const float* scale_dev, void* stream);
+int coocc_wino_input_h2_masked(const float* in, int in_stride, int B, int X, int Y, int Z, int C, int tile, void* V,
+                               int vstride, int64_t group_rows, float scale, const float* scale_dev, const uint8_t* occ,
+                               const int32_t* range_end, const int32_t* range_bits, int nranges, void* stream);
 int coocc_sparse_tap_sum(const float* P, const int32_t* map, int B, int X, int Y, int Z, int Cout, const float* scale,
                          float* S, int s_stride, int p_rows, void* stream);
 int coocc_wino_output(const float* Mb, int64_t group_rows, int B, int X, int Y, int Z, int C, int tile, float* out,
```

New measurement: 261.3, median of 2. No clear change (+0.7%).
